# mindazhao/PWStableNet

Hardware: AMD Instinct MI355X
Metric: stabilized frames/sec at 256x256 (netG fp32 + grid_sample), whole job (higher is better)
Workload: dtype f32

## Files before the change

### pwstablenet_amd/csrc/abi.cpp

```cpp
#include <vector>

#include "common.h"

namespace pws {
bool g_two_queues = true;
int g_math = PWS_MATH_FP32;
int g_store = PWS_STORE_FP32;
int g_experiment = 0;
bool g_prof_on = false;
thread_local int g_prof_tag = -1;
thread_local bool t_deterministic = false;
namespace {
struct ProfEntry {
    hipEvent_t a, b;
    int kernel_id, tag;
    double flops, bytes;
};
std::vector<ProfEntry> g_prof_log;
std::vector<hipEvent_t> g_prof_pool;
hipEvent_t prof_event() {
    if (!g_prof_pool.empty()) {
        hipEvent_t e = g_prof_pool.back();
        g_prof_pool.pop_back();
        return e;
    }
    hipEvent_t e = nullptr;
    (void)hipEventCreate(&e);
    return e;
}
const char *const kKernelNames[KID_COUNT] = {
    "conv_mfma_kernel<k3s1,16x16>", "conv_mfma_kernel<k3s1,small>", "conv_mfma_kernel<k3s2,16x16>",
    "conv_mfma_kernel<k3s2,small>", "conv_mfma_kernel<k5s1,16x16>", "conv_mfma_kernel<convT4,16x16>",
    "conv_mfma_kernel<convT4,small>", "theta_head_kernel", "field_head_kernel", "grid_sample_fwd_kernel",
    "grid_sample_bwd_kernel", "upsample_grid_sample_fwd_kernel", "upsample_bilinear_ac_kernel", "affine_grid_kernel",
    "adam_kernel", "pack_weight_kernel", "conv_mfma_kernel<dgrad k4s2>", "conv_mfma_kernel<dgrad subpix k3s2>",
    "wgrad_mfma_kernel", "act_bwd_bias_kernel", "field_head_bwd_kernels", "theta_head_bwd_kernels",
    "wino_k3s1_kernel<F(2x2,3x3)>", "conv_bf16_kernel", "wgrad_bf16_kernel",
    "wino_ct4_kernel<F(3x3,2x2)>", "upsample_grid_sample_u8_kernel", "objective_kernels", "conv_ring_kernel", "conv_ringf_kernel",
    "wino_ring_kernel<F(2x2,3x3)>", "wino_ring_kernel<convT4,F(2x2,2x2)>", "conv_skinny_kernel", "wgrad_ring_kernel", "conv_skinny16_kernel", "conv_first_kernel", "wino5_first_kernel",
    "field_homography_kernel"};
}

bool prof_begin(int kernel_id, double flops, double bytes, hipStream_t st) {
    hipStreamCaptureStatus cs = hipStreamCaptureStatusNone;
    if (hipStreamIsCapturing(st, &cs) != hipSuccess || cs != hipStreamCaptureStatusNone) return false;
    ProfEntry e{prof_event(), prof_event(), kernel_id, g_prof_tag, flops, bytes};
    (void)hipEventRecord(e.a, st);
    g_prof_log.push_back(e);
    return true;
}
void prof_end(hipStream_t st) {
    if (!g_prof_log.empty()) (void)hipEventRecord(g_prof_log.back().b, st);
}
}

namespace pws {
static thread_local char g_err[512] = "";

void set_error(const char *fmt, ...) {
    va_list ap;
    va_start(ap, fmt);
    vsnprintf(g_err, sizeof(g_err), fmt, ap);
    va_end(ap);
}
}

extern "C" int pws_version(void) { return PWS_VERSION; }

extern "C" const char *pws_last_error(void) { return pws::g_err; }

extern "C" int pws_device_info(int *compute_units, int *arch_is_gfx950) {
    int dev = 0;
    hipError_t e = hipGetDevice(&dev);
    hipDeviceProp_t prop;
    if (e == hipSuccess) e = hipGetDeviceProperties(&prop, dev);
    if (e != hipSuccess) {
        pws::set_error("pws_device_info: %s", hipGetErrorString(e));
        return PWS_EHIP;
    }
    if (compute_units) *compute_units = prop.multiProcessorCount;
    if (arch_is_gfx950) {
        const char *a = prop.gcnArchName;
        *arch_is_gfx950 = (a[0] == 'g' && a[1] == 'f' && a[2] == 'x' && a[3] == '9' && a[4] == '5' && a[5] == '0') ? 1 : 0;
    }
    return PWS_OK;
}

extern "C" int pws_prof_enable(int on) {
    pws::g_prof_on = on != 0;
    return PWS_OK;
}

extern "C" int pws_prof_collect(pws_prof_record *out, int max_records) {
    const int n = (int)pws::g_prof_log.size();
    hipError_t bad = hipSuccess;
    for (int i = 0; i < n; ++i) {
        pws::ProfEntry &e = pws::g_prof_log[i];
        float ms = 0.f;
        hipError_t err = hipEventSynchronize(e.b);
        if (err == hipSuccess) err = hipEventElapsedTime(&ms, e.a, e.b);
        if (err != hipSuccess && bad == hipSuccess) bad = err;
        if (err == hipSuccess && out && i < max_records) out[i] = pws_prof_record{e.kernel_id, e.tag, e.flops, e.bytes, ms};
        pws::g_prof_pool.push_back(e.a);
        pws::g_prof_pool.push_back(e.b);
    }
    pws::g_prof_log.clear();
    if (bad != hipSuccess) {
        pws::set_error("pws_prof_collect: %s", hipGetErrorString(bad));
        return PWS_EHIP;
    }
    return n;
}

extern "C" const char *pws_prof_kernel_name(int kernel_id) {
    return (kernel_id >= 0 && kernel_id < pws::KID_COUNT) ? pws::kKernelNames[kernel_id] : "?";
}

extern "C" int pws_set_option(int key, int value) {
    if (key == PWS_OPT_TWO_QUEUES) {
        pws::g_two_queues = value != 0;
        return PWS_OK;
    }
    if (key == PWS_OPT_MATH) {
        if (value != PWS_MATH_FP32 && value != PWS_MATH_BF16) {
            pws::set_error("pws_set_option: PWS_OPT_MATH value %d is not PWS_MATH_FP32 / PWS_MATH_BF16", value);
            return PWS_EINVAL;
        }
        pws::g_math = value;
        return PWS_OK;
    }
    if (key == PWS_OPT_STORE) {
        if (value != PWS_STORE_FP32 && value != PWS_STORE_BF16) {
            pws::set_error("pws_set_option: PWS_OPT_STORE value %d is not PWS_STORE_FP32 / PWS_STORE_BF16", value);
            return PWS_EINVAL;
        }
        pws::g_store = value;
        return PWS_OK;
    }
    if (key == PWS_OPT_EXPERIMENT) {
        pws::g_experiment = value;
        return PWS_OK;
    }
    pws::set_error("pws_set_option: unknown key %d", key);
    return PWS_EINVAL;
}

extern "C" int pws_get_option(int key) {
    if (key == PWS_OPT_TWO_QUEUES) return pws::g_two_queues ? 1 : 0;
    if (key == PWS_OPT_MATH) return pws::g_math;
    if (key == PWS_OPT_STORE) return pws::g_store;
    if (key == PWS_OPT_EXPERIMENT) return pws::g_experiment;
    pws::set_error("pws_get_option: unknown key %d", key);
    return PWS_EINVAL;
}
```

### pwstablenet_amd/csrc/common.h

```cpp
#pragma once
#include <hip/hip_runtime.h>

#include <cstdarg>
#include <cstdio>

#include "../../include/pwstable.h"
#include "experiments.h"

namespace pws {

void set_error(const char *fmt, ...);

inline int check_launch(const char *what) {
    hipError_t e = hipGetLastError();
    if (e != hipSuccess) {
        set_error("%s: %s", what, hipGetErrorString(e));
        return PWS_EHIP;
    }
    return PWS_OK;
}

#define PWS_REQUIRE(cond, ...)          \
    do {                                \
        if (!(cond)) {                  \
            pws::set_error(__VA_ARGS__); \
            return PWS_EINVAL;          \
        }                               \
    } while (0)

inline hipStream_t as_stream(pws_stream_t s) { return reinterpret_cast<hipStream_t>(s); }

constexpr int kWave = 64;
constexpr int kXcds = 8;

__device__ __forceinline__ unsigned xcd_remap(unsigned bid, unsigned nblocks) {
    const unsigned q = nblocks / kXcds, r = nblocks % kXcds;
    const unsigned xcd = bid % kXcds, slot = bid / kXcds;
    const unsigned base = xcd < r ? xcd * (q + 1) : r * (q + 1) + (xcd - r) * q;
    return base + slot;
}

constexpr int kMaxDevices = 32;
inline int current_device_slot() {
    int d = 0;
    (void)hipGetDevice(&d);
    return (int)((unsigned)d % kMaxDevices);
}
struct PerDeviceFlag {
    bool v[kMaxDevices] = {};
    bool &cur() { return v[current_device_slot()]; }
};
struct PerDeviceInt {
    int v[kMaxDevices] = {};
    int &cur() { return v[current_device_slot()]; }
};

#if defined(__HIPCC__)
__device__ __forceinline__ float mul_rounded(float a, float b) {
    float p = a * b;
    asm volatile("" : "+v"(p));
    return p;
}
#endif

enum KernelId {
    KID_CONV_K3S1_BIG = 0, KID_CONV_K3S1_SMALL, KID_CONV_K3S2_BIG, KID_CONV_K3S2_SMALL, KID_CONV_K5S1, KID_CONVT4_BIG,
    KID_CONVT4_SMALL, KID_THETA_HEAD, KID_FIELD_HEAD, KID_GRID_SAMPLE_FWD, KID_GRID_SAMPLE_BWD, KID_UPSAMPLE_GRID_SAMPLE_FWD,
    KID_UPSAMPLE, KID_AFFINE_GRID, KID_ADAM, KID_PACK, KID_DGRAD_K4S2, KID_DGRAD_SP3, KID_WGRAD, KID_ACT_BWD, KID_FIELD_HEAD_BWD,
    KID_THETA_HEAD_BWD, KID_CONV_WINO, KID_CONV_BF16, KID_WGRAD_BF16, KID_CONV_WINO_CT4, KID_UPSAMPLE_GRID_SAMPLE_U8, KID_OBJECTIVE, KID_CONV_RING, KID_CONV_RINGF, KID_CONV_WRING, KID_CONV_WRING_CT4, KID_CONV_SKINNY, KID_WGRAD_RING, KID_CONV_SKINNY16, KID_CONV_FIRST, KID_CONV_FIRST_WINO, KID_FIELD_HOMOGRAPHY, KID_COUNT
};
extern thread_local bool t_deterministic;
struct DeterministicScope {
    bool prev;
    explicit DeterministicScope(bool on) : prev(t_deterministic) { t_deterministic = on || prev; }
    ~DeterministicScope() { t_deterministic = prev; }
};
extern bool g_two_queues;
extern int g_math;
extern int g_store;
extern bool g_prof_on;
extern thread_local int g_prof_tag;
bool prof_begin(int kernel_id, double flops, double bytes, hipStream_t st);
void prof_end(hipStream_t st);
struct ProfScope {
    hipStream_t st;
    bool on;
    ProfScope(int kernel_id, double flops, double bytes, hipStream_t s) : st(s), on(g_prof_on) {
        if (on) on = prof_begin(kernel_id, flops, bytes, st);
    }
    ~ProfScope() {
        if (on) prof_end(st);
    }
};

int nchw_to_nhwc_pad_strided(const float *x, size_t sample_stride, float *out, int n, int c, int h, int w, int cpad, int store, hipStream_t st);

struct ProfHint {
    double flops, bytes;
};
int theta_z1(const float *x, int n, int c, int hidden, const float *w_flat, const float *b_flat, float *ws, float *z1, hipStream_t st);
int theta_z2(const float *h, int n, int hidden, const float *w_lin, const float *b_lin, float *z2, hipStream_t st);
int field_head_raw(const float *x, int ld, int n, int h, int w, int c, const float *w_out, const float *b_out, float *z, hipStream_t st);
int field_bn_finish(const float *yhat, const float *theta, int n, int h, int w, int ac, float *resid, float *grid, hipStream_t st);
int field_bwd_gz(const float *resid, const float *g_grid, const float *g_resid, int n, int h, int w, int ac, float *gz, float *db_out,
                 float *dtheta, hipStream_t st);
int field_bwd_dx_dw(const float *x, int ld, const float *gz, int n, int h, int w, int c, const float *w_out, float *dx, int dx_ld,
                    int dx_accumulate, float *dw_out, int store, hipStream_t st, int dx_act = 0);
int theta_bwd_bn_lin(const float *dz2, const float *h, int n, int hidden, const float *w_lin, float *dw_lin, float *dh, hipStream_t st);
int theta_bwd_flat(const float *x, int n, int c, int hidden, const float *w_flat, const float *dz1, float *dw_flat, float *dx,
                   int dx_accumulate, hipStream_t st);
int wino_k3s1_launch(const pws_conv_args *a, const ProfHint &ph, hipStream_t st);
int wring_try(const pws_conv_args *a, const ProfHint &ph, hipStream_t st);
int wring_pack(const float *pk, float *ur, int cin_pad, int cout, int ct4, hipStream_t st);
__host__ __device__ inline size_t wring_index(int nc, int xi, int ci, int co, int nchunks) {
    const int cob = co >> 5, c32 = co & 31, co16 = c32 >> 1, nt = c32 & 1;
    const int chunk = ci >> 4, kq = (ci >> 2) & 3, st = ci & 3;
    return ((((((size_t)cob * nchunks + chunk) * nc + xi) * 2 + nt) * 4 + kq) * 16 + co16) * 4 + st;
}
#ifdef __HIPCC__
__device__ inline void wring_pack_element(const float *__restrict__ pk, float *__restrict__ ur, size_t plane, size_t i, int cin_pad, int cout,
                                          int ct4) {
    const int co = (int)(i % cout), ci = (int)(i / cout), nch = cin_pad / 16;
    if (!ct4) {
        float g[3][3];
#pragma unroll
        for (int r = 0; r < 3; ++r)
#pragma unroll
            for (int s = 0; s < 3; ++s) g[r][s] = pk[(size_t)(r * 3 + s) * plane + i];
        float u[4][3];
#pragma unroll
        for (int s = 0; s < 3; ++s) {
            u[0][s] = g[0][s], u[1][s] = 0.5f * (g[0][s] + g[1][s] + g[2][s]), u[2][s] = 0.5f * (g[0][s] - g[1][s] + g[2][s]);
            u[3][s] = g[2][s];
        }
#pragma unroll
        for (int r = 0; r < 4; ++r) {
            ur[wring_index(16, r * 4 + 0, ci, co, nch)] = u[r][0];
            ur[wring_index(16, r * 4 + 1, ci, co, nch)] = 0.5f * (u[r][0] + u[r][1] + u[r][2]);
            ur[wring_index(16, r * 4 + 2, ci, co, nch)] = 0.5f * (u[r][0] - u[r][1] + u[r][2]);
            ur[wring_index(16, r * 4 + 3, ci, co, nch)] = u[r][2];
        }
    } else if (ct4 == 2) {
        const double G[6][5] = {{1, 0, 0, 0, 0},
                                {-1.0 / 3, -1.0 / 3, -1.0 / 3, -1.0 / 3, -1.0 / 3},
                                {1.0 / 3, -1.0 / 3, 1.0 / 3, -1.0 / 3, 1.0 / 3},
                                {1.0 / 15, 2.0 / 15, 4.0 / 15, 8.0 / 15, 16.0 / 15},
                                {-16.0 / 15, 8.0 / 15, -4.0 / 15, 2.0 / 15, -1.0 / 15},
                                {0, 0, 0, 0, 1}};
        double t[6][5];
        for (int r = 0; r < 6; ++r)
            for (int v = 0; v < 5; ++v) {
                double a = 0;
                for (int q = 0; q < 5; ++q) a += G[r][q] * (double)pk[(size_t)(q * 5 + v) * plane + i];
                t[r][v] = a;
            }
        for (int r = 0; r < 6; ++r)
            for (int c = 0; c < 6; ++c) {
                double a = 0;
                for (int v = 0; v < 5; ++v) a += t[r][v] * G[c][v];
                ur[((((size_t)((ci >> 2) * 9 + ((r * 6 + c) >> 2)) * (cout / 16) + (co >> 4)) * 4 + (ci & 3)) * 16 + (co & 15)) * 4 + ((r * 6 + c) & 3)] = (float)a;
            }
    } else {
#pragma unroll
        for (int py = 0; py < 2; ++py)
#pragma unroll
            for (int px = 0; px < 2; ++px) {
                float g[2][2];
#pragma unroll
                for (int r = 0; r < 2; ++r)
#pragma unroll
                    for (int s = 0; s < 2; ++s) g[r][s] = pk[(size_t)((py * 2 + px) * 4 + r * 2 + s) * plane + i];
                float u[3][2];
#pragma unroll
                for (int s = 0; s < 2; ++s) u[0][s] = g[0][s], u[1][s] = g[0][s] + g[1][s], u[2][s] = g[1][s];
                float *o = ur + (size_t)py * 18 * plane;
#pragma unroll
                for (int r = 0; r < 3; ++r) {
                    o[wring_index(18, px * 9 + r * 3 + 0, ci, co, nch)] = u[r][0];
                    o[wring_index(18, px * 9 + r * 3 + 1, ci, co, nch)] = u[r][0] + u[r][1];
                    o[wring_index(18, px * 9 + r * 3 + 2, ci, co, nch)] = u[r][1];
                }
            }
    }
}
#endif

typedef __bf16 bf16x8 __attribute__((ext_vector_type(8)));
typedef __bf16 bf16x2 __attribute__((ext_vector_type(2)));
typedef float f32x2 __attribute__((ext_vector_type(2)));
typedef float f32x4 __attribute__((ext_vector_type(4)));
typedef unsigned u32x4 __attribute__((ext_vector_type(4)));
__device__ __forceinline__ unsigned cvt_pk_bf16(float a, float b) {
    return __builtin_bit_cast(unsigned, __builtin_convertvector((f32x2){a, b}, bf16x2));
}

template <bool IO16>
__device__ __forceinline__ float4 ld4(const float *base, size_t idx) {
    if constexpr (IO16) {
        const uint2 u = *reinterpret_cast<const uint2 *>(reinterpret_cast<const __bf16 *>(base) + idx);
        return make_float4(__builtin_bit_cast(float, u.x << 16), __builtin_bit_cast(float, u.x & 0xffff0000u),
                           __builtin_bit_cast(float, u.y << 16), __builtin_bit_cast(float, u.y & 0xffff0000u));
    } else {
        return *reinterpret_cast<const float4 *>(base + idx);
    }
}
template <bool IO16>
__device__ __forceinline__ void st4(float *base, size_t idx, const float4 &v) {
    if constexpr (IO16) {
        *reinterpret_cast<uint2 *>(reinterpret_cast<__bf16 *>(base) + idx) = make_uint2(cvt_pk_bf16(v.x, v.y), cvt_pk_bf16(v.z, v.w));
    } else {
        *reinterpret_cast<float4 *>(base + idx) = v;
    }
}

__device__ __forceinline__ float act_apply(float v, int act) {
    const float slope = act == PWS_ACT_LRELU ? 0.2f : 1.f;
    const unsigned keep = act == PWS_ACT_RELU ? 0u : 0xffffffffu;
    const float t = __builtin_bit_cast(float, __builtin_bit_cast(unsigned, slope * v) & keep);
    float r;
    asm("v_max_f32 %0, %1, %2" : "=v"(r) : "v"(v), "v"(t));
    return r;
}

}
```

### pwstablenet_amd/csrc/conv_common.h

```cpp
#pragma once
#include "common.h"

namespace pws {

typedef float f32x16 __attribute__((ext_vector_type(16)));

struct ConvKParams {
    const float *src_ptr[4];
    int src_c[4];
    int src_ld[4];
    int nsrc;
    int N, H, W;
    int LH, LW;
    int OH, OW;
    int cin_pad;
    int cout;
    const float *w;
    const float *bias;
    float *out;
    int out_ld;
    int act;
    int tiles_x, tiles_y;
    unsigned ntiles;
    int nclasses;
    int cls_inner;
    int ksplit;
    int chunks_per_split;
    size_t split_stride;
    const void *w_bf;
    int kpad_bf, npad_bf;
    int io_bf16;
    int epi16;
    int ndst;
    float *dst_ptr[4];
    int dst_c0[4], dst_c1[4], dst_ld[4], dst_acc[4];
    const void *dst_y[4];
    int dst_y_ld[4], dst_act[4];
    void *out_sign;
    int out_sign_ld;
    const void *dst_sign[4];
    int dst_sign_ld[4];
};

__device__ __forceinline__ void epi_store(const ConvKParams &p, size_t pix, int co, float v) {
    if (p.ndst == 0) {
        p.out[pix * p.out_ld + co] = act_apply(v + (p.bias ? p.bias[co] : 0.f), p.act);
    } else {
#pragma unroll
        for (int s = 0; s < 4; ++s) {
            if (s < p.ndst && co >= p.dst_c0[s] && co < p.dst_c1[s]) {
                float *d = p.dst_ptr[s] + pix * p.dst_ld[s] + (co - p.dst_c0[s]);
                *d = p.dst_acc[s] ? *d + v : v;
            }
        }
    }
}

__device__ __forceinline__ float bf16_lo(unsigned u) { return __builtin_bit_cast(float, u << 16); }
__device__ __forceinline__ float bf16_hi(unsigned u) { return __builtin_bit_cast(float, u & 0xffff0000u); }
__device__ __forceinline__ void epi_store_pair16(const ConvKParams &p, size_t pix, int co, float v0, float v1) {
    if (p.ndst == 0) {
        const float b0 = p.bias ? p.bias[co] : 0.f, b1 = p.bias ? p.bias[co + 1] : 0.f;
        unsigned *d = reinterpret_cast<unsigned *>(reinterpret_cast<__bf16 *>(p.out) + pix * p.out_ld + co);
        *d = cvt_pk_bf16(act_apply(v0 + b0, p.act), act_apply(v1 + b1, p.act));
    } else {
#pragma unroll
        for (int s = 0; s < 4; ++s) {
            if (s < p.ndst && co >= p.dst_c0[s] && co < p.dst_c1[s]) {
                unsigned *d = reinterpret_cast<unsigned *>(reinterpret_cast<__bf16 *>(p.dst_ptr[s]) + pix * p.dst_ld[s] + (co - p.dst_c0[s]));
                if (p.dst_acc[s]) {
                    const unsigned o = *d;
                    v0 += bf16_lo(o), v1 += bf16_hi(o);
                }
                if (p.dst_act[s] != PWS_ACT_NONE) {
                    const unsigned y = *reinterpret_cast<const unsigned *>(static_cast<const __bf16 *>(p.dst_y[s]) + pix * p.dst_y_ld[s] +
                                                                           (co - p.dst_c0[s]));
                    const float sl = p.dst_act[s] == PWS_ACT_LRELU ? 0.2f : 0.f;
                    v0 *= bf16_lo(y) > 0.f ? 1.f : sl, v1 *= bf16_hi(y) > 0.f ? 1.f : sl;
                }
                *d = cvt_pk_bf16(v0, v1);
            }
        }
    }
}

__device__ __forceinline__ void conv_block_coords(const ConvKParams &p, bool subpix, unsigned &tile, int &cls, int &split) {
    if (subpix && p.cls_inner) {
        const unsigned xcd = blockIdx.x & 7u, slot = blockIdx.x >> 3;
        cls = (int)(slot & 3u), split = (int)blockIdx.z;
        tile = xcd_remap(((slot >> 2) << 3) | xcd, p.ntiles);
    } else {
        tile = xcd_remap(blockIdx.x, p.ntiles);
        cls = subpix ? (int)(blockIdx.z & 3) : 0;
        split = subpix ? (int)(blockIdx.z >> 2) : (int)blockIdx.z;
    }
}
static inline dim3 conv_grid(ConvKParams &kp, int bn) {
    kp.cls_inner = kp.nclasses == 4 && kp.ntiles % 8 == 0 ? 1 : 0;
    const unsigned gy = (unsigned)((kp.cout + bn - 1) / bn);
    return kp.cls_inner ? dim3(kp.ntiles * 4, gy, (unsigned)kp.ksplit) : dim3(kp.ntiles, gy, (unsigned)(kp.nclasses * kp.ksplit));
}

struct ProfInfo {
    double flops, bytes;
};

struct TileChoice {
    int th, tw, tn, ck, bn;
    int kid;
    int (*launch)(ConvKParams &, hipStream_t, const ProfInfo &);
};

int launch_splitk_reduce(const ConvKParams &kp, const float *partial, size_t total4, hipStream_t st);

static inline long cdiv(long a, long b) { return (a + b - 1) / b; }

constexpr long kFillBlocks = 512;
constexpr long kFillBlocksBf16 = 256;

[[maybe_unused]] static int select_and_launch(const TileChoice *cands, int ncand, ConvKParams &kp, int cin_total, float *final_out,
                             float *ws, size_t ws_floats, hipStream_t st, const ProfInfo &pi, long kFill = kFillBlocks) {
    const TileChoice *best = nullptr;
    long best_blocks = -1;
    double best_score = -1.0;
    for (int i = 0; i < ncand; ++i) {
        const TileChoice &c = cands[i];
        const long tiles = cdiv(kp.LW, c.tw) * cdiv(kp.LH, c.th) * cdiv(kp.N, c.tn);
        const double useful = (double)kp.N * kp.LH * kp.LW / ((double)tiles * c.th * c.tw * c.tn);
        if (useful < 0.45 && i + 1 < ncand) continue;
        if (c.th < 8 && c.th < kp.LH && i > 0 && best) continue;
        const long blocks = tiles * cdiv(kp.cout, c.bn) * kp.nclasses;
        if (blocks >= kFill) {
            best = &c, best_blocks = blocks;
            break;
        }
        if (blocks * useful > best_score) best = &c, best_blocks = blocks, best_score = blocks * useful;
    }
    const TileChoice &c = *best;
    kp.tiles_x = (int)cdiv(kp.LW, c.tw), kp.tiles_y = (int)cdiv(kp.LH, c.th);
    kp.ntiles = (unsigned)(kp.tiles_x * kp.tiles_y * cdiv(kp.N, c.tn));
    const int total_chunks = cin_total / c.ck;
    int ksplit = 1;
    const size_t out_floats = (size_t)kp.N * kp.OH * kp.OW * kp.cout;
    if (best_blocks < kFill && ws && kp.cout % 4 == 0 && total_chunks >= 4) {
        long want = cdiv(kFill, best_blocks);
        if (want > 64) want = 64;
        if (want > total_chunks / 2) want = total_chunks / 2;
        while (want > 1 && (size_t)want * out_floats > ws_floats) --want;
        ksplit = (int)want;
    }
    kp.ksplit = ksplit < 1 ? 1 : ksplit;
    kp.chunks_per_split = (int)cdiv(total_chunks, kp.ksplit);
    kp.ksplit = (int)cdiv(total_chunks, kp.chunks_per_split);
    kp.split_stride = out_floats;
    kp.out = kp.ksplit > 1 ? ws : final_out;
    ProfScope prof(c.kid, pi.flops, pi.bytes, st);
    int rc = c.launch(kp, st, pi);
    if (rc != PWS_OK || kp.ksplit == 1) return rc;
    const size_t total4 = out_floats / 4;
    kp.out = final_out;
    return launch_splitk_reduce(kp, ws, total4, st);
}


}
```

### pwstablenet_amd/csrc/conv_mfma.hip

```cpp
#include "conv_common.h"

namespace pws {

template <int KS_, int STRIDE_, int PAD_, int SUBPIX_, int TH_, int TW_, int TN_, int CK_, int WM_, int WN_, int MT_,
          int NT_, bool NCHW_ = false>
struct ConvCfg {
    static constexpr int KS = KS_, STRIDE = STRIDE_, PAD = PAD_, TH = TH_, TW = TW_, TN = TN_, CK = CK_;
    static constexpr int SUBPIX = SUBPIX_;
    static constexpr bool CONVT = SUBPIX_ != 0, NCHW = NCHW_;
    static constexpr int WM = WM_, WN = WN_, MT = MT_, NT = NT_;
    static constexpr int THREADS = 64 * WM * WN;
    static constexpr int BM = TH * TW * TN, BN = 32 * NT * WN;
    static_assert(BM == 32 * MT * WM, "tile pixels must equal the M extent of the wave grid");
    static constexpr int IH = (TH - 1) * STRIDE + KS, IW = (TW - 1) * STRIDE + KS;
    static constexpr int PIX = TN * IH * IW;
    static constexpr int CKP = CK + 1;
    static constexpr int TAPS = KS * KS;
    static constexpr int LDS_IN = (PIX * CKP + 3) / 4 * 4;
    static constexpr int LDS_W = TAPS * CK * BN;
    static constexpr int LDS_BYTES = (LDS_IN + LDS_W) * 4;
    static constexpr int C4 = CK / 4;
    static constexpr int ITEMS_IN = (PIX * C4 + THREADS - 1) / THREADS;
    static constexpr int ITEMS_W = (TAPS * CK * (BN / 4) + THREADS - 1) / THREADS;
    static constexpr int ITEMS_NCHW = (PIX * CK + THREADS - 1) / THREADS;
};

template <class C>
__global__ void __launch_bounds__(C::THREADS, 2) conv_mfma_kernel(const ConvKParams p) {
    extern __shared__ float lds[];
    float *lds_in = lds;
    float *lds_w = lds + C::LDS_IN;

    const int tid = threadIdx.x;
    const int lane = tid & 63, wv = tid >> 6;
    const int l31 = lane & 31, hi = lane >> 5;
    const int wm = wv / C::WN, wn = wv % C::WN;

    unsigned tile;
    int cls, split;
    conv_block_coords(p, C::CONVT, tile, cls, split);
    const int tx_i = tile % p.tiles_x;
    const int ty_i = (tile / p.tiles_x) % p.tiles_y;
    const int tn_i = tile / (p.tiles_x * p.tiles_y);
    const int n0 = tn_i * C::TN, y0 = ty_i * C::TH, x0 = tx_i * C::TW;
    const int co0 = blockIdx.y * C::BN;
    const int py = cls >> 1, px = cls & 1;
    const int pad_y = C::SUBPIX == 1 ? 1 - py : (C::SUBPIX == 2 ? 0 : C::PAD);
    const int pad_x = C::SUBPIX == 1 ? 1 - px : (C::SUBPIX == 2 ? 0 : C::PAD);
    const int iy0 = y0 * C::STRIDE - pad_y, ix0 = x0 * C::STRIDE - pad_x;

    int g_pix[C::ITEMS_IN];
    int l_off[C::ITEMS_IN];
    int g_c4[C::ITEMS_IN];
    unsigned ok_mask = 0;
#pragma unroll
    for (int it = 0; it < C::ITEMS_IN; ++it) {
        const int item = tid + it * C::THREADS;
        const int pix = item / C::C4, c4 = item % C::C4;
        const int lx = pix % C::IW, ly = (pix / C::IW) % C::IH, tn = pix / (C::IW * C::IH);
        const int n = n0 + tn, iy = iy0 + ly, ix = ix0 + lx;
        const bool ok = item < C::PIX * C::C4 && n < p.N && iy >= 0 && iy < p.H && ix >= 0 && ix < p.W;
        g_pix[it] = ok ? (n * p.H + iy) * p.W + ix : 0;
        ok_mask |= ok ? (1u << it) : 0u;
        l_off[it] = item < C::PIX * C::C4 ? pix * C::CKP + c4 * 4 : -1;
        g_c4[it] = c4 * 4;
    }
    static_assert(C::ITEMS_IN <= 32 && C::ITEMS_W <= 32, "mask width");
    int w_off[C::ITEMS_W];
    unsigned w_mask = 0;
#pragma unroll
    for (int it = 0; it < C::ITEMS_W; ++it) {
        const int item = tid + it * C::THREADS;
        const int row = item / (C::BN / 4), q = item % (C::BN / 4);
        const int tap = row / C::CK, c = row % C::CK;
        const bool ok = item < C::TAPS * C::CK * (C::BN / 4) && (co0 + q * 4) < p.cout;
        w_off[it] = ok ? (tap * p.cin_pad + c) * p.cout + co0 + q * 4 : 0;
        w_mask |= ok ? (1u << it) : 0u;
    }
    const float *w_cls = p.w + (size_t)cls * C::TAPS * p.cin_pad * p.cout;
    float4 r_in[C::NCHW ? 1 : C::ITEMS_IN];
    float4 r_w[C::ITEMS_W];
    float r_nchw[C::NCHW ? C::ITEMS_NCHW : 1];

    auto load_chunk = [&](int s, int c0, int wrow) {
        if constexpr (C::NCHW) {
            const int Creal = p.src_c[0];
            const size_t sstride = p.src_ld[0] ? (size_t)p.src_ld[0] : (size_t)Creal * p.H * p.W;
#pragma unroll
            for (int it = 0; it < C::ITEMS_NCHW; ++it) {
                const int item = tid + it * C::THREADS;
                const int c = item / C::PIX, pix = item % C::PIX;
                const int lx = pix % C::IW, ly = (pix / C::IW) % C::IH, tn = pix / (C::IW * C::IH);
                const int n = n0 + tn, iy = iy0 + ly, ix = ix0 + lx;
                const bool ok = item < C::PIX * C::CK && (c0 + c) < Creal && n < p.N && iy >= 0 && iy < p.H && ix >= 0 &&
                                ix < p.W;
                const size_t off = ok ? (size_t)n * sstride + ((size_t)(c0 + c) * p.H + iy) * p.W + ix : 0;
                const float v = p.src_ptr[0][off];
                r_nchw[it] = ok ? v : 0.f;
            }
        } else {
            const float *sp = p.src_ptr[s] + c0;
            const size_t ld = p.src_ld[s];
#pragma unroll
            for (int it = 0; it < C::ITEMS_IN; ++it)
                r_in[it] = *reinterpret_cast<const float4 *>(sp + (size_t)g_pix[it] * ld + g_c4[it]);
        }
        const float *wp = w_cls + (size_t)wrow * p.cout;
#pragma unroll
        for (int it = 0; it < C::ITEMS_W; ++it) r_w[it] = *reinterpret_cast<const float4 *>(wp + w_off[it]);
    };
    auto store_chunk = [&]() {
        if constexpr (C::NCHW) {
#pragma unroll
            for (int it = 0; it < C::ITEMS_NCHW; ++it) {
                const int item = tid + it * C::THREADS;
                const int c = item / C::PIX, pix = item % C::PIX;
                if (item < C::PIX * C::CK) lds_in[pix * C::CKP + c] = r_nchw[it];
            }
        } else {
#pragma unroll
            for (int it = 0; it < C::ITEMS_IN; ++it) {
                if (l_off[it] >= 0) {
                    const bool ok = (ok_mask >> it) & 1u;
                    float *d = lds_in + l_off[it];
                    d[0] = ok ? r_in[it].x : 0.f, d[1] = ok ? r_in[it].y : 0.f, d[2] = ok ? r_in[it].z : 0.f,
                    d[3] = ok ? r_in[it].w : 0.f;
                }
            }
        }
#pragma unroll
        for (int it = 0; it < C::ITEMS_W; ++it) {
            const int item = tid + it * C::THREADS;
            if (item < C::TAPS * C::CK * (C::BN / 4)) {
                const bool ok = (w_mask >> it) & 1u;
                *reinterpret_cast<float4 *>(lds_w + item * 4) =
                    ok ? r_w[it] : make_float4(0.f, 0.f, 0.f, 0.f);
            }
        }
    };

    f32x16 acc[C::MT][C::NT];
#pragma unroll
    for (int mt = 0; mt < C::MT; ++mt)
#pragma unroll
        for (int nt = 0; nt < C::NT; ++nt)
#pragma unroll
            for (int r = 0; r < 16; ++r) acc[mt][nt][r] = 0.f;

    int a_base[C::MT];
#pragma unroll
    for (int mt = 0; mt < C::MT; ++mt) {
        const int m = (wm * C::MT + mt) * 32 + l31;
        const int tx = m % C::TW, ty = (m / C::TW) % C::TH, tn = m / (C::TW * C::TH);
        a_base[mt] = ((tn * C::IH + ty * C::STRIDE) * C::IW + tx * C::STRIDE) * C::CKP + hi;
    }
    const int b_base = hi * C::BN + wn * C::NT * 32 + l31;

    int total_chunks = 0;
    if constexpr (C::NCHW) {
        total_chunks = p.cin_pad / C::CK;
    } else {
        for (int s = 0; s < p.nsrc; ++s) total_chunks += p.src_c[s] / C::CK;
    }
    const int ch_begin = split * p.chunks_per_split;
    const int ch_end = min(total_chunks, ch_begin + p.chunks_per_split);
    int s = 0, c0 = ch_begin * C::CK, wrow = ch_begin * C::CK;
    if constexpr (!C::NCHW) {
        while (s < p.nsrc - 1 && c0 >= p.src_c[s]) c0 -= p.src_c[s], ++s;
    }
    if (ch_begin < ch_end) load_chunk(s, c0, wrow);
    for (int ch = ch_begin; ch < ch_end; ++ch) {
        __syncthreads();
        store_chunk();
        __syncthreads();
        c0 += C::CK, wrow += C::CK;
        if (!C::NCHW && c0 >= p.src_c[s]) ++s, c0 = 0;
        if (ch + 1 < ch_end) load_chunk(s, c0, wrow);

#pragma unroll
        for (int tap = 0; tap < C::TAPS; ++tap) {
            if (C::SUBPIX == 2 && ((!py && tap / C::KS) || (!px && tap % C::KS))) continue;
            const int toff = ((tap / C::KS) * C::IW + (tap % C::KS)) * C::CKP;
#pragma unroll
            for (int kk = 0; kk < C::CK / 2; ++kk) {
                float a[C::MT], b[C::NT];
#pragma unroll
                for (int mt = 0; mt < C::MT; ++mt) a[mt] = lds_in[a_base[mt] + toff + 2 * kk];
#pragma unroll
                for (int nt = 0; nt < C::NT; ++nt) b[nt] = lds_w[b_base + (tap * C::CK + 2 * kk) * C::BN + nt * 32];
#pragma unroll
                for (int mt = 0; mt < C::MT; ++mt)
#pragma unroll
                    for (int nt = 0; nt < C::NT; ++nt)
                        acc[mt][nt] = __builtin_amdgcn_mfma_f32_32x32x2f32(a[mt], b[nt], acc[mt][nt], 0, 0, 0);
            }
        }
    }

    const bool partial = p.ksplit > 1;
    float *part = p.out + (size_t)split * p.split_stride;
#pragma unroll
    for (int nt = 0; nt < C::NT; ++nt) {
        const int co = co0 + (wn * C::NT + nt) * 32 + l31;
        const bool co_ok = co < p.cout;
#pragma unroll
        for (int mt = 0; mt < C::MT; ++mt) {
#pragma unroll
            for (int r = 0; r < 16; ++r) {
                const int m = (wm * C::MT + mt) * 32 + (r & 3) + 8 * (r >> 2) + 4 * hi;
                const int tx = m % C::TW, ty = (m / C::TW) % C::TH, tn = m / (C::TW * C::TH);
                const int n = n0 + tn, y = y0 + ty, x = x0 + tx;
                const int oy = C::CONVT ? 2 * y + py : y, ox = C::CONVT ? 2 * x + px : x;
                if (co_ok && n < p.N && y < p.LH && x < p.LW && oy < p.OH && ox < p.OW) {
                    const size_t pix = (size_t)(n * p.OH + oy) * p.OW + ox;
                    if (partial)
                        part[pix * p.cout + co] = acc[mt][nt][r];
                    else
                        epi_store(p, pix, co, acc[mt][nt][r]);
                }
            }
        }
    }
}

__global__ void __launch_bounds__(256) splitk_reduce_kernel(const ConvKParams p, const float *__restrict__ partial,
                                                            size_t total4) {
    const size_t i = (size_t)blockIdx.x * 256 + threadIdx.x;
    if (i >= total4) return;
    float4 a = reinterpret_cast<const float4 *>(partial)[i];
    for (int s = 1; s < p.ksplit; ++s) {
        const float4 b = reinterpret_cast<const float4 *>(partial + (size_t)s * p.split_stride)[i];
        a.x += b.x, a.y += b.y, a.z += b.z, a.w += b.w;
    }
    const size_t pix = (i * 4) / p.cout;
    const int co = (int)((i * 4) % p.cout);
    if (p.io_bf16) {
        epi_store_pair16(p, pix, co, a.x, a.y), epi_store_pair16(p, pix, co + 2, a.z, a.w);
        return;
    }
    epi_store(p, pix, co, a.x), epi_store(p, pix, co + 1, a.y), epi_store(p, pix, co + 2, a.z), epi_store(p, pix, co + 3, a.w);
}

int launch_splitk_reduce(const ConvKParams &kp, const float *partial, size_t total4, hipStream_t st) {
    hipLaunchKernelGGL(splitk_reduce_kernel, dim3((unsigned)((total4 + 255) / 256)), dim3(256), 0, st, kp, partial, total4);
    return check_launch("splitk_reduce_kernel");
}

template <class C, int KID>
static int launch_cfg(ConvKParams &kp, hipStream_t st, const ProfInfo &pi) {
    static PerDeviceFlag attr_set_dev;
    bool &attr_set = attr_set_dev.cur();
    if (!attr_set) {
        hipError_t e = hipFuncSetAttribute(reinterpret_cast<const void *>(&conv_mfma_kernel<C>),
                                           hipFuncAttributeMaxDynamicSharedMemorySize, C::LDS_BYTES);
        if (e != hipSuccess) {
            set_error("hipFuncSetAttribute(conv_mfma_kernel, %d B LDS): %s", C::LDS_BYTES, hipGetErrorString(e));
            return PWS_EHIP;
        }
        attr_set = true;
    }
    const dim3 grid = conv_grid(kp, C::BN);
    hipLaunchKernelGGL(conv_mfma_kernel<C>, grid, dim3(C::THREADS), C::LDS_BYTES, st, kp);
    return check_launch("conv_mfma_kernel");
}

template <class C, int KID>
static constexpr TileChoice choice() {
    return TileChoice{C::TH, C::TW, C::TN, C::CK, C::BN, KID, &launch_cfg<C, KID>};
}

using K3S1_T256 = ConvCfg<3, 1, 1, 0, 16, 16, 1, 16, 4, 1, 2, 2>;
using K3S1_T128 = ConvCfg<3, 1, 1, 0, 8, 16, 1, 16, 4, 1, 1, 2>;
using K3S1_T64 = ConvCfg<3, 1, 1, 0, 8, 8, 1, 16, 2, 2, 1, 1>;
using K3S1_T64N4 = ConvCfg<3, 1, 1, 0, 4, 4, 4, 16, 2, 2, 1, 1>;
using K3S1_T64N16 = ConvCfg<3, 1, 1, 0, 2, 2, 16, 16, 2, 2, 1, 1>;
using K3S2_T256 = ConvCfg<3, 2, 1, 0, 16, 16, 1, 8, 4, 1, 2, 2>;
using K3S2_T128 = ConvCfg<3, 2, 1, 0, 8, 16, 1, 16, 4, 1, 1, 2>;
using K3S2_T64 = ConvCfg<3, 2, 1, 0, 8, 8, 1, 16, 2, 2, 1, 1>;
using K3S2_T64N4 = ConvCfg<3, 2, 1, 0, 4, 4, 4, 16, 2, 2, 1, 1>;
using K3S2_T64N16 = ConvCfg<3, 2, 1, 0, 2, 2, 16, 16, 2, 2, 1, 1>;
using K5S1_T256 = ConvCfg<5, 1, 2, 0, 16, 16, 1, 8, 4, 1, 2, 2>;
using K5S1_T256_NCHW = ConvCfg<5, 1, 2, 0, 16, 16, 1, 8, 4, 1, 2, 2, true>;
using CT4_T256 = ConvCfg<2, 1, 0, 1, 16, 16, 1, 16, 4, 1, 2, 2>;
using CT4_T128 = ConvCfg<2, 1, 0, 1, 8, 16, 1, 16, 4, 1, 1, 2>;
using CT4_T64 = ConvCfg<2, 1, 0, 1, 8, 8, 1, 16, 2, 2, 1, 1>;
using CT4_T64N4 = ConvCfg<2, 1, 0, 1, 4, 4, 4, 16, 2, 2, 1, 1>;
using CT4_T64N16 = ConvCfg<2, 1, 0, 1, 2, 2, 16, 16, 2, 2, 1, 1>;

using K4S2_T256 = ConvCfg<4, 2, 1, 0, 16, 16, 1, 8, 4, 1, 2, 2>;
using K4S2_T128 = ConvCfg<4, 2, 1, 0, 8, 16, 1, 8, 4, 1, 1, 2>;
using K4S2_T64 = ConvCfg<4, 2, 1, 0, 8, 8, 1, 8, 2, 2, 1, 1>;
using K4S2_T64N4 = ConvCfg<4, 2, 1, 0, 4, 4, 4, 8, 2, 2, 1, 1>;
using K4S2_T64N16 = ConvCfg<4, 2, 1, 0, 2, 2, 16, 8, 2, 2, 1, 1>;
using SP3_T256 = ConvCfg<2, 1, 0, 2, 16, 16, 1, 16, 4, 1, 2, 2>;
using SP3_T128 = ConvCfg<2, 1, 0, 2, 8, 16, 1, 16, 4, 1, 1, 2>;
using SP3_T64 = ConvCfg<2, 1, 0, 2, 8, 8, 1, 16, 2, 2, 1, 1>;
using SP3_T64N4 = ConvCfg<2, 1, 0, 2, 4, 4, 4, 16, 2, 2, 1, 1>;
using SP3_T64N16 = ConvCfg<2, 1, 0, 2, 2, 2, 16, 16, 2, 2, 1, 1>;

static const TileChoice kK3S1[] = {choice<K3S1_T256, KID_CONV_K3S1_BIG>(), choice<K3S1_T128, KID_CONV_K3S1_BIG>(),
                                   choice<K3S1_T64, KID_CONV_K3S1_SMALL>(), choice<K3S1_T64N4, KID_CONV_K3S1_SMALL>(),
                                   choice<K3S1_T64N16, KID_CONV_K3S1_SMALL>()};
static const TileChoice kK3S2[] = {choice<K3S2_T256, KID_CONV_K3S2_BIG>(), choice<K3S2_T128, KID_CONV_K3S2_BIG>(),
                                   choice<K3S2_T64, KID_CONV_K3S2_SMALL>(), choice<K3S2_T64N4, KID_CONV_K3S2_SMALL>(),
                                   choice<K3S2_T64N16, KID_CONV_K3S2_SMALL>()};
static const TileChoice kCT4[] = {choice<CT4_T256, KID_CONVT4_BIG>(), choice<CT4_T128, KID_CONVT4_BIG>(),
                                  choice<CT4_T64, KID_CONVT4_SMALL>(), choice<CT4_T64N4, KID_CONVT4_SMALL>(),
                                  choice<CT4_T64N16, KID_CONVT4_SMALL>()};
static const TileChoice kK4S2[] = {choice<K4S2_T256, KID_DGRAD_K4S2>(), choice<K4S2_T128, KID_DGRAD_K4S2>(),
                                   choice<K4S2_T64, KID_DGRAD_K4S2>(), choice<K4S2_T64N4, KID_DGRAD_K4S2>(),
                                   choice<K4S2_T64N16, KID_DGRAD_K4S2>()};
static const TileChoice kSP3[] = {choice<SP3_T256, KID_DGRAD_SP3>(), choice<SP3_T128, KID_DGRAD_SP3>(),
                                  choice<SP3_T64, KID_DGRAD_SP3>(), choice<SP3_T64N4, KID_DGRAD_SP3>(),
                                  choice<SP3_T64N16, KID_DGRAD_SP3>()};
static const TileChoice kK5[] = {choice<K5S1_T256, KID_CONV_K5S1>()};
static const TileChoice kK5N[] = {choice<K5S1_T256_NCHW, KID_CONV_K5S1>()};

int conv_bf16_fwd(int kind, ConvKParams &kp, int cin_total, float *out, float *ws, size_t ws_floats, hipStream_t st,
                  const ProfInfo &pi);
int conv_bf16_dgrad(int kind, ConvKParams &kp, int cout_f, float *ws, size_t ws_floats, hipStream_t st, const ProfInfo &pi);
static inline bool ledger_direct(int bit) { return (exp_mask(EXP_PARITY_LEDGER, 32) & bit) != 0; }
int conv_ringf_try(int kind, const ConvKParams &kp, hipStream_t st, const ProfInfo &pi);
int conv_first_try(const ConvKParams &kp, hipStream_t st, const ProfInfo &pi);
int wino5_first_try(const ConvKParams &kp, const float *u, hipStream_t st, const ProfInfo &pi);
int conv_skinny_try(int kind, ConvKParams &kp, float *final_out, float *ws, size_t ws_floats, hipStream_t st, const ProfInfo &pi);

int conv2d_fwd_impl(const pws_conv_args *a, hipStream_t st) {
    PWS_REQUIRE(a != nullptr, "pws_conv2d_fwd: args is NULL");
    PWS_REQUIRE(a->n >= 0 && a->h > 0 && a->w > 0, "pws_conv2d_fwd: bad n/h/w %d/%d/%d", a->n, a->h, a->w);
    PWS_REQUIRE(a->nsrc >= 1 && a->nsrc <= 4, "pws_conv2d_fwd: nsrc %d not in 1..4", a->nsrc);
    PWS_REQUIRE(a->cout > 0 && a->cout % 4 == 0, "pws_conv2d_fwd: cout %d must be a positive multiple of 4", a->cout);
    PWS_REQUIRE(a->out && a->w_packed, "pws_conv2d_fwd: NULL out / w_packed");
    PWS_REQUIRE(a->out_ld >= a->cout, "pws_conv2d_fwd: out_ld %d < cout %d", a->out_ld, a->cout);
    PWS_REQUIRE(a->act >= PWS_ACT_NONE && a->act <= PWS_ACT_RELU, "pws_conv2d_fwd: bad act %d", a->act);
    PWS_REQUIRE(a->ws == nullptr || (reinterpret_cast<size_t>(a->ws) & 15) == 0, "pws_conv2d_fwd: ws must be 16-B aligned");
    if (a->n == 0) return PWS_OK;

    ConvKParams kp{};
    int cin = 0;
    kp.nsrc = a->nsrc;
    const bool nchw = a->src_nchw != 0;
    if (nchw) {
        PWS_REQUIRE(a->kind == PWS_CONV_K5S1 && a->nsrc == 1, "pws_conv2d_fwd: NCHW source only for the k5 first layer");
        PWS_REQUIRE(a->src[0].ptr && a->src[0].channels > 0, "pws_conv2d_fwd: bad NCHW source");
        PWS_REQUIRE(a->src[0].ld >= 0, "pws_conv2d_fwd: NCHW source: ld is the sample stride in floats (0 = dense)");
        kp.src_ptr[0] = a->src[0].ptr, kp.src_c[0] = a->src[0].channels, kp.src_ld[0] = a->src[0].ld;
        cin = a->src[0].channels;
    } else {
        for (int s = 0; s < a->nsrc; ++s) {
            const pws_src &sr = a->src[s];
            PWS_REQUIRE(sr.ptr && sr.channels > 0 && sr.channels % 16 == 0 && sr.ld >= sr.channels && sr.ld % 4 == 0 &&
                            (reinterpret_cast<size_t>(sr.ptr) & 15) == 0,
                        "pws_conv2d_fwd: source %d (channels %d, ld %d) must be 16-B aligned, channels %% 16 == 0, ld %% 4 == 0",
                        s, sr.channels, sr.ld);
            kp.src_ptr[s] = sr.ptr, kp.src_c[s] = sr.channels, kp.src_ld[s] = sr.ld;
            cin += sr.channels;
        }
    }
    kp.cin_pad = (cin + 15) / 16 * 16;
    kp.N = a->n, kp.H = a->h, kp.W = a->w;
    kp.cout = a->cout, kp.w = a->w_packed, kp.bias = a->bias, kp.out_ld = a->out_ld, kp.act = a->act;
    kp.nclasses = 1;
    PWS_REQUIRE((size_t)a->n * a->h * a->w < (1u << 31), "pws_conv2d_fwd: n*h*w too large for 32-bit pixel indices");
    float *ws = static_cast<float *>(a->ws);
    const size_t ws_floats = a->ws_bytes / sizeof(float);
    const bool bf16 = a->math == PWS_MATH_BF16 && a->w_bf16 && !nchw;
    if (a->store == PWS_STORE_BF16) {
        PWS_REQUIRE(bf16, "pws_conv2d_fwd: bf16 storage needs math == PWS_MATH_BF16, w_bf16 and NHWC sources");
        PWS_REQUIRE(a->out_ld % 2 == 0 && a->cout % 2 == 0 && (reinterpret_cast<size_t>(a->out) & 3) == 0,
                    "pws_conv2d_fwd: bf16 storage needs an even cout / out_ld and a 4-byte aligned out");
        for (int s = 0; s < a->nsrc; ++s)
            PWS_REQUIRE(a->src[s].channels % 32 == 0 && a->src[s].ld % 8 == 0,
                        "pws_conv2d_fwd: bf16 storage needs channels %% 32 == 0 and ld %% 8 == 0 (source %d: %d, %d)", s,
                        a->src[s].channels, a->src[s].ld);
        kp.io_bf16 = 1;
        kp.epi16 = a->cout % 8 == 0 && a->out_ld % 8 == 0 && (reinterpret_cast<size_t>(a->out) & 15) == 0;
    }
    kp.w_bf = a->w_bf16, kp.kpad_bf = (kp.cin_pad + 31) / 32 * 32, kp.npad_bf = (a->cout + 63) / 64 * 64;
    if (a->out_sign) {
        PWS_REQUIRE(a->store == PWS_STORE_BF16 && a->cout % 8 == 0 && a->out_sign_ld >= a->cout / 8,
                    "pws_conv2d_fwd: out_sign needs bf16 storage, cout %% 8 == 0 and out_sign_ld >= cout / 8");
        kp.out_sign = a->out_sign, kp.out_sign_ld = a->out_sign_ld;
    }

    auto info = [&](int k2, double out_pix) {
        ProfInfo pi;
        pi.flops = 2.0 * out_pix * a->cout * (double)cin * k2;
        const double es = a->store == PWS_STORE_BF16 ? 2.0 : 4.0, ws_ = bf16 ? 2.0 : 4.0;
        pi.bytes = es * ((double)a->n * a->h * a->w * cin + out_pix * a->cout) + ws_ * (double)k2 * cin * a->cout;
        return pi;
    };
    switch (a->kind) {
    case PWS_CONV_K3S1:
    case PWS_CONVT_K3S1: {
        kp.OH = kp.LH = a->h, kp.OW = kp.LW = a->w;
        const ProfInfo pi = info(9, (double)a->n * a->h * a->w);
        if (bf16) {
            const int rc = conv_bf16_fwd(a->kind, kp, kp.cin_pad, a->out, ws, ws_floats, st, pi);
            if (rc != 1) return rc;
        }
        if (a->w_wring && !nchw && !bf16 && !ledger_direct(2)) {
            const int rc = wring_try(a, ProfHint{pi.flops, pi.bytes}, st);
            if (rc != 1) return rc;
        }
        const long wblocks = cdiv(a->w, 16) * cdiv(a->h, 16) * a->n * cdiv(a->cout, 64);
        if (a->w_wino && !nchw && a->h >= 16 && a->w >= 16 && wblocks >= 128 && (cin >= 128 || wblocks >= 2048) && !ledger_direct(2))
            return wino_k3s1_launch(a, ProfHint{pi.flops, pi.bytes}, st);
        if (!bf16 && !nchw) {
            kp.out = a->out;
            int rc = ledger_direct(8) ? 1 : conv_ringf_try(a->kind, kp, st, pi);
            if (rc != 1) return rc;
            rc = ledger_direct(16) ? 1 : conv_skinny_try(a->kind, kp, a->out, ws, ws_floats, st, pi);
            if (rc != 1) return rc;
        }
        return select_and_launch(kK3S1, 5, kp, kp.cin_pad, a->out, ws, ws_floats, st, pi);
    }
    case PWS_CONV_K3S2:
        kp.OH = kp.LH = (a->h + 2 - 3) / 2 + 1, kp.OW = kp.LW = (a->w + 2 - 3) / 2 + 1;
        if (bf16) {
            const int rc = conv_bf16_fwd(a->kind, kp, kp.cin_pad, a->out, ws, ws_floats, st, info(9, (double)a->n * kp.OH * kp.OW));
            if (rc != 1) return rc;
        }
        if (!bf16 && !nchw) {
            kp.out = a->out;
            int rc = ledger_direct(8) ? 1 : conv_ringf_try(a->kind, kp, st, info(9, (double)a->n * kp.OH * kp.OW));
            if (rc != 1) return rc;
            rc = ledger_direct(16) ? 1 : conv_skinny_try(a->kind, kp, a->out, ws, ws_floats, st, info(9, (double)a->n * kp.OH * kp.OW));
            if (rc != 1) return rc;
        }
        return select_and_launch(kK3S2, 5, kp, kp.cin_pad, a->out, ws, ws_floats, st, info(9, (double)a->n * kp.OH * kp.OW));
    case PWS_CONV_K5S1:
        kp.OH = kp.LH = a->h, kp.OW = kp.LW = a->w;
        if (bf16) {
            const int rc = conv_bf16_fwd(a->kind, kp, kp.cin_pad, a->out, nullptr, 0, st, info(25, (double)a->n * a->h * a->w));
            if (rc != 1) return rc;
        }
        if (nchw && !ledger_direct(1)) {
            kp.out = a->out;
            if (a->w_wring) {
                const int rcw = wino5_first_try(kp, static_cast<const float *>(a->w_wring), st, info(25, (double)a->n * a->h * a->w));
                if (rcw != 1) return rcw;
            }
            const int rc = conv_first_try(kp, st, info(25, (double)a->n * a->h * a->w));
            if (rc != 1) return rc;
        }
        return select_and_launch(nchw ? kK5N : kK5, 1, kp, kp.cin_pad, a->out, nullptr, 0, st,
                                 info(25, (double)a->n * a->h * a->w));
    case PWS_CONVT_K4S2: {
        kp.LH = a->h, kp.LW = a->w, kp.OH = 2 * a->h, kp.OW = 2 * a->w, kp.nclasses = 4;
        ProfInfo pi = info(4, (double)a->n * kp.OH * kp.OW);
        pi.bytes += (bf16 ? 2.0 : 4.0) * 12.0 * cin * a->cout;
        if (bf16) {
            const int rc = conv_bf16_fwd(a->kind, kp, kp.cin_pad, a->out, ws, ws_floats, st, pi);
            if (rc != 1) return rc;
        }
        if (a->w_wring && !nchw && !bf16 && !ledger_direct(4)) {
            const int rc = wring_try(a, ProfHint{pi.flops, pi.bytes}, st);
            if (rc != 1) return rc;
        }
        const long wb = cdiv(a->w, 24) * cdiv(a->h, 12) * a->n * cdiv(a->cout, 64) * 4;
        if (a->w_wino && a->h >= 24 && a->w >= 24 && wb >= 256 && !ledger_direct(4)) return wino_k3s1_launch(a, ProfHint{pi.flops, pi.bytes}, st);
        if (!bf16 && !nchw) {
            kp.out = a->out;
            int rc = ledger_direct(8) ? 1 : conv_ringf_try(a->kind, kp, st, pi);
            if (rc != 1) return rc;
            rc = ledger_direct(16) ? 1 : conv_skinny_try(a->kind, kp, a->out, ws, ws_floats, st, pi);
            if (rc != 1) return rc;
        }
        return select_and_launch(kCT4, 5, kp, kp.cin_pad, a->out, ws, ws_floats, st, pi);
    }
    default:
        set_error("pws_conv2d_fwd: kind %d is not a runnable conv kind", a->kind);
        return PWS_EINVAL;
    }
}

int conv2d_bwd_data_impl(const pws_conv_bwd_data_args *a, hipStream_t st) {
    PWS_REQUIRE(a != nullptr, "pws_conv2d_bwd_data: args is NULL");
    PWS_REQUIRE(a->n >= 0 && a->h > 0 && a->w > 0 && a->cout > 0 && a->cout % 16 == 0, "pws_conv2d_bwd_data: bad shape");
    PWS_REQUIRE(a->gout && a->w_dgrad && a->gout_ld >= a->cout && a->gout_ld % 4 == 0, "pws_conv2d_bwd_data: bad gout / weights");
    PWS_REQUIRE(a->ndst >= 1 && a->ndst <= 4, "pws_conv2d_bwd_data: ndst %d not in 1..4", a->ndst);
    if (a->n == 0) return PWS_OK;
    ConvKParams kp{};
    int oh = a->h, ow = a->w;
    if (a->kind == PWS_CONV_K3S2) oh = (a->h - 1) / 2 + 1, ow = (a->w - 1) / 2 + 1;
    if (a->kind == PWS_CONVT_K4S2) oh = 2 * a->h, ow = 2 * a->w;
    kp.nsrc = 1, kp.src_ptr[0] = a->gout, kp.src_c[0] = a->cout, kp.src_ld[0] = a->gout_ld;
    kp.N = a->n, kp.H = oh, kp.W = ow;
    kp.OH = a->h, kp.OW = a->w;
    kp.cin_pad = a->cout;
    int cin_f = 0;
    kp.ndst = a->ndst;
    for (int s = 0; s < a->ndst; ++s) {
        const pws_dst &d = a->dst[s];
        PWS_REQUIRE(d.ptr && d.channels > 0 && d.ld >= d.channels, "pws_conv2d_bwd_data: bad destination %d", s);
        kp.dst_ptr[s] = d.ptr, kp.dst_c0[s] = cin_f, kp.dst_c1[s] = cin_f + d.channels, kp.dst_ld[s] = d.ld;
        kp.dst_acc[s] = d.accumulate ? 1 : 0;
        if (d.act_y && d.act != PWS_ACT_NONE) {
            PWS_REQUIRE(a->store == PWS_STORE_BF16 && (d.act == PWS_ACT_LRELU || d.act == PWS_ACT_RELU),
                        "pws_conv2d_bwd_data: the fused act' (dst[%d].act_y) needs bf16 storage and PWS_ACT_LRELU / PWS_ACT_RELU", s);
            PWS_REQUIRE(d.act_y_ld >= d.channels && d.act_y_ld % 2 == 0 && (reinterpret_cast<size_t>(d.act_y) & 3) == 0,
                        "pws_conv2d_bwd_data: bad act_y / act_y_ld of destination %d", s);
            kp.dst_y[s] = d.act_y, kp.dst_y_ld[s] = d.act_y_ld, kp.dst_act[s] = d.act;
            if (d.act_sign) {
                PWS_REQUIRE(d.channels % 8 == 0 && d.act_sign_ld >= d.channels / 8, "pws_conv2d_bwd_data: bad act_sign / act_sign_ld of destination %d", s);
                kp.dst_sign[s] = d.act_sign, kp.dst_sign_ld[s] = d.act_sign_ld;
            }
        }
        cin_f += d.channels;
    }
    PWS_REQUIRE(cin_f % 4 == 0, "pws_conv2d_bwd_data: total destination channels %d must be a multiple of 4", cin_f);
    kp.cout = cin_f, kp.w = a->w_dgrad, kp.bias = nullptr, kp.act = PWS_ACT_NONE, kp.out_ld = cin_f, kp.nclasses = 1;
    PWS_REQUIRE((size_t)a->n * oh * ow < (1u << 31) && (size_t)a->n * a->h * a->w < (1u << 31), "pws_conv2d_bwd_data: too large");
    float *ws = static_cast<float *>(a->ws);
    const size_t ws_floats = a->ws_bytes / sizeof(float);
    ProfInfo pi;
    const double k2 = a->kind == PWS_CONVT_K4S2 ? 4.0 : 9.0;
    pi.flops = 2.0 * a->n * oh * ow * (double)a->cout * cin_f * k2;
    {
        const double es = a->store == PWS_STORE_BF16 ? 2.0 : 4.0, in_pix = (double)a->n * a->h * a->w;
        pi.bytes = es * ((double)a->n * oh * ow * a->cout + in_pix * cin_f);
        for (int s = 0; s < a->ndst; ++s)
            pi.bytes += es * in_pix * a->dst[s].channels * (a->dst[s].accumulate ? 1.0 : 0.0) +
                        (kp.dst_act[s] == PWS_ACT_NONE ? 0.0 : (kp.dst_sign[s] ? in_pix * a->dst[s].channels / 8.0 : es * in_pix * a->dst[s].channels));
    }
    if (a->kind == PWS_CONV_K3S2)
        kp.LH = oh, kp.LW = ow, kp.nclasses = 4;
    else
        kp.LH = a->h, kp.LW = a->w;
    if (a->store == PWS_STORE_BF16) {
        PWS_REQUIRE(a->math == PWS_MATH_BF16 && a->w_dgrad_bf16 && a->cout % 32 == 0 && a->gout_ld % 8 == 0,
                    "pws_conv2d_bwd_data: bf16 storage needs bf16 math, w_dgrad_bf16, cout %% 32 == 0 and gout_ld %% 8 == 0");
        for (int s = 0; s < a->ndst; ++s)
            PWS_REQUIRE(a->dst[s].channels % 2 == 0 && a->dst[s].ld % 2 == 0 && (reinterpret_cast<size_t>(a->dst[s].ptr) & 3) == 0,
                        "pws_conv2d_bwd_data: bf16 storage needs even channels / ld and 4-byte aligned destinations");
        kp.io_bf16 = 1;
        kp.epi16 = 1;
        for (int s = 0; s < a->ndst; ++s)
            if (a->dst[s].channels % 8 || a->dst[s].ld % 8 || (reinterpret_cast<size_t>(a->dst[s].ptr) & 15) ||
                (kp.dst_act[s] != PWS_ACT_NONE && (kp.dst_y_ld[s] % 8 || (reinterpret_cast<size_t>(kp.dst_y[s]) & 15))))
                kp.epi16 = 0;
    }
    if (a->math == PWS_MATH_BF16 && a->w_dgrad_bf16) {
        kp.w_bf = a->w_dgrad_bf16, kp.kpad_bf = (a->cout + 31) / 32 * 32, kp.npad_bf = (cin_f + 63) / 64 * 64;
        const int rc = conv_bf16_dgrad(a->kind, kp, a->cout, ws, ws_floats, st, pi);
        if (rc != 1) return rc;
    }
    switch (a->kind) {
    case PWS_CONV_K3S1:
    case PWS_CONVT_K3S1:
        return select_and_launch(kK3S1, 5, kp, a->cout, nullptr, ws, ws_floats, st, pi);
    case PWS_CONV_K3S2:
        return select_and_launch(kSP3, 5, kp, a->cout, nullptr, ws, ws_floats, st, pi);
    case PWS_CONVT_K4S2:
        return select_and_launch(kK4S2, 5, kp, a->cout, nullptr, ws, ws_floats, st, pi);
    default:
        set_error("pws_conv2d_bwd_data: kind %d has no data gradient here", a->kind);
        return PWS_EINVAL;
    }
}

}

extern "C" int pws_conv2d_fwd(const pws_conv_args *args, pws_stream_t stream) {
    return pws::conv2d_fwd_impl(args, pws::as_stream(stream));
}

extern "C" int pws_conv2d_bwd_data(const pws_conv_bwd_data_args *args, pws_stream_t stream) {
    return pws::conv2d_bwd_data_impl(args, pws::as_stream(stream));
}
```

### pwstablenet_amd/csrc/conv_skinny.hip

```cpp
#include "conv_common.h"

namespace pws {

enum SkinnyMode { SK_K3S1 = 0, SK_K3S2 = 1, SK_CT4 = 2 };

struct SkParams {
    const float *src_ptr[4];
    int src_c[4], src_ld[4];
    int nsrc;
    int N, H, W;
    int LH, LW;
    int OH, OW;
    int mode;
    int cin_pad, cout;
    const float *w;
    unsigned w_bytes;
    const float *bias;
    int act;
    float *out;
    int out_ld;
    size_t split_stride;
    int ksplit, cps, nchunks;
    int M;
    unsigned ncob;
};

constexpr unsigned kSkOob = 0x7ffffff0u;
__device__ __forceinline__ void sk_dma16(unsigned lds_addr, unsigned voff, __amdgpu_buffer_rsrc_t rsrc, unsigned soff) {
    unsigned keep;
    asm volatile("s_nop 4\n\ts_mov_b32 %0, m0\n\ts_mov_b32 m0, %1\n\ts_nop 0\n\tbuffer_load_dwordx4 %2, %3, %4 offen lds\n\ts_mov_b32 m0, %0"
                 : "=&s"(keep)
                 : "s"(lds_addr), "v"(voff), "s"(rsrc), "s"(soff));
}
template <class T>
__device__ __forceinline__ T sksel4(const T (&a)[4], int i) {
    return i == 0 ? a[0] : (i == 1 ? a[1] : (i == 2 ? a[2] : a[3]));
}

template <int MT_W, int NT_W, int WM>
__global__ void __launch_bounds__(256) conv_skinny_kernel(const SkParams p) {
    extern __shared__ __attribute__((aligned(16))) unsigned char lds[];
    constexpr int WN = 4 / WM;
    static_assert(NT_W * WN == 4, "4 N tiles of 16 output channels per workgroup");
    const int tid = threadIdx.x, lane = tid & 63;
    const int wv = __builtin_amdgcn_readfirstlane(tid >> 6);
    const int l15 = lane & 15, kq = lane >> 4;
    const int wm = wv % WM, wn = wv / WM;

    unsigned b = blockIdx.x;
    const int ks = (int)(b % (unsigned)p.ksplit);
    b /= (unsigned)p.ksplit;
    const int cob = (int)(b % p.ncob), cls = (int)(b / p.ncob);
    const int py = cls >> 1, px = cls & 1;
    const int co0 = cob * 64;
    const int c_begin = ks * p.cps;
    const int nck = min(p.nchunks - c_begin, p.cps);
    const int ntaps = p.mode == SK_CT4 ? 4 : 9;

    {
        const __amdgpu_buffer_rsrc_t rsrc_w = __builtin_amdgcn_make_buffer_rsrc(const_cast<float *>(p.w), 0, (int)p.w_bytes, 0x00020000);
        const int nt = lane >> 4 >> 0 & 3, kqd = (lane >> 2) & 3, c4 = lane & 3;
        const int col = co0 + nt * 16 + c4 * 4;
        const bool col_ok = col < p.cout;
        const size_t plane = (size_t)p.cin_pad * p.cout;
        const int npieces = nck * ntaps * 4;
        for (int q = wv; q < npieces; q += 4) {
            const int blk = q >> 2, st = q & 3;
            const int ck = blk / ntaps, tap = blk - ck * ntaps;
            const int wplane = p.mode == SK_CT4 ? cls * 4 + tap : tap;
            const unsigned row = (unsigned)((c_begin + ck) * 16 + kqd * 4 + st);
            const unsigned voff = col_ok ? (row * (unsigned)p.cout + (unsigned)col) * 4u : kSkOob;
            sk_dma16((unsigned)(blk * 4096 + st * 1024), voff, rsrc_w, (unsigned)__builtin_amdgcn_readfirstlane((unsigned)((size_t)wplane * plane * 4)));
        }
    }

    int pn[MT_W], piy[MT_W], pix_[MT_W];
    bool pok[MT_W];
#pragma unroll
    for (int i = 0; i < MT_W; ++i) {
        const int m = (wm + i * WM) * 16 + l15;
        pok[i] = m < p.M;
        const int mm = pok[i] ? m : 0;
        const int ox = mm % p.LW, t2 = mm / p.LW;
        const int oy = t2 % p.LH;
        pn[i] = t2 / p.LH;
        if (p.mode == SK_K3S2) piy[i] = 2 * oy - 1, pix_[i] = 2 * ox - 1;
        else if (p.mode == SK_CT4) piy[i] = oy + py - 1, pix_[i] = ox + px - 1;
        else piy[i] = oy - 1, pix_[i] = ox - 1;
    }
    int s = 0, c0 = c_begin * 16;
    while (s < p.nsrc - 1 && c0 >= sksel4(p.src_c, s)) c0 -= sksel4(p.src_c, s), ++s;

    constexpr int MAXT = 9;
    f32x4 a_cur[MAXT][MT_W], a_nxt[MAXT][MT_W];
    auto load_a = [&](f32x4 (&a)[MAXT][MT_W]) {
        const float *sp = sksel4(p.src_ptr, s) + c0 + kq * 4;
        const int ld = sksel4(p.src_ld, s);
        const int kw = p.mode == SK_CT4 ? 2 : 3;
#pragma unroll
        for (int t = 0; t < MAXT; ++t) {
            if (t < ntaps) {
                const int dy = t / kw, dx = t - dy * kw;
#pragma unroll
                for (int i = 0; i < MT_W; ++i) {
                    const int iy = piy[i] + dy, ix = pix_[i] + dx;
                    const bool ok = pok[i] && iy >= 0 && iy < p.H && ix >= 0 && ix < p.W;
                    a[t][i] = ok ? *reinterpret_cast<const f32x4 *>(sp + ((size_t)(pn[i] * p.H + iy) * p.W + ix) * ld) : (f32x4){0.f, 0.f, 0.f, 0.f};
                }
            }
        }
        c0 += 16;
        if (c0 >= sksel4(p.src_c, s) && s < p.nsrc - 1) ++s, c0 = 0;
    };

    f32x4 acc[MT_W][NT_W];
#pragma unroll
    for (int i = 0; i < MT_W; ++i)
#pragma unroll
        for (int j = 0; j < NT_W; ++j) acc[i][j] = (f32x4){0.f, 0.f, 0.f, 0.f};

    load_a(a_cur);
    asm volatile("s_waitcnt vmcnt(0)" ::: "memory");
    __syncthreads();
    const int b_lane = (kq * 16 + l15) * 4;
    for (int ck = 0; ck < nck; ++ck) {
        if (ck + 1 < nck) load_a(a_nxt);
#pragma unroll
        for (int t = 0; t < MAXT; ++t) {
            if (t < ntaps) {
                const unsigned char *bb = lds + (unsigned)((ck * ntaps + t) * 4096) + b_lane;
#pragma unroll
                for (int st = 0; st < 4; ++st) {
                    float bv[NT_W];
#pragma unroll
                    for (int j = 0; j < NT_W; ++j) bv[j] = *reinterpret_cast<const float *>(bb + (st * 4 + wn * NT_W + j) * 256);
#pragma unroll
                    for (int i = 0; i < MT_W; ++i)
#pragma unroll
                        for (int j = 0; j < NT_W; ++j) acc[i][j] = __builtin_amdgcn_mfma_f32_16x16x4f32(a_cur[t][i][st], bv[j], acc[i][j], 0, 0, 0);
                }
            }
        }
        if (ck + 1 < nck) {
#pragma unroll
            for (int t = 0; t < MAXT; ++t)
#pragma unroll
                for (int i = 0; i < MT_W; ++i) a_cur[t][i] = a_nxt[t][i];
        }
    }

    float *out = p.out + (size_t)ks * p.split_stride;
    const bool fin = p.ksplit == 1;
#pragma unroll
    for (int i = 0; i < MT_W; ++i) {
#pragma unroll
        for (int r = 0; r < 4; ++r) {
            const int m = (wm + i * WM) * 16 + 4 * kq + r;
            if (m >= p.M) continue;
            const int ox = m % p.LW, t2 = m / p.LW;
            const int oy = t2 % p.LH, n = t2 / p.LH;
            size_t opix;
            if (p.mode == SK_CT4) opix = ((size_t)n * p.OH + 2 * oy + py) * p.OW + 2 * ox + px;
            else opix = ((size_t)n * p.OH + oy) * p.OW + ox;
#pragma unroll
            for (int j = 0; j < NT_W; ++j) {
                const int co = co0 + (wn * NT_W + j) * 16 + l15;
                if (co < p.cout) {
                    if (fin) p.out[opix * p.out_ld + co] = act_apply(acc[i][j][r] + (p.bias ? p.bias[co] : 0.f), p.act);
                    else out[opix * p.cout + co] = acc[i][j][r];
                }
            }
        }
    }
}

template <int MT_W, int NT_W, int WM>
static int skinny_launch(const SkParams &p, unsigned grid, int lds_bytes, hipStream_t st) {
    static PerDeviceFlag attr_set_dev;
    bool &attr_set = attr_set_dev.cur();
    if (!attr_set) {
        hipError_t e = hipFuncSetAttribute(reinterpret_cast<const void *>(&conv_skinny_kernel<MT_W, NT_W, WM>), hipFuncAttributeMaxDynamicSharedMemorySize,
                                           160 * 1024);
        if (e != hipSuccess) {
            set_error("hipFuncSetAttribute(conv_skinny_kernel): %s", hipGetErrorString(e));
            return PWS_EHIP;
        }
        attr_set = true;
    }
    hipLaunchKernelGGL((conv_skinny_kernel<MT_W, NT_W, WM>), dim3(grid), dim3(256), lds_bytes, st, p);
    return check_launch("conv_skinny_kernel");
}

int conv_skinny_try(int kind, ConvKParams &kp, float *final_out, float *ws, size_t ws_floats, hipStream_t st, const ProfInfo &pi) {
    if (kp.io_bf16 || kp.ndst != 0 || exp_is(EXP_SKINNY_OFF)) return 1;
    int mode;
    if (kind == PWS_CONV_K3S1 || kind == PWS_CONVT_K3S1) mode = SK_K3S1;
    else if (kind == PWS_CONV_K3S2) mode = SK_K3S2;
    else if (kind == PWS_CONVT_K4S2) mode = SK_CT4;
    else return 1;
    const long M = (long)kp.N * kp.LH * kp.LW;
    if (M < 1 || M > 128 || kp.cout % 4 != 0) return 1;
    int cin = 0;
    for (int s = 0; s < kp.nsrc; ++s) {
        if (kp.src_ld[s] == 0 || kp.src_c[s] % 16 != 0 || kp.src_ld[s] % 4 != 0 || (reinterpret_cast<size_t>(kp.src_ptr[s]) & 15)) return 1;
        cin += kp.src_c[s];
    }
    if (cin != kp.cin_pad) return 1;
    const int ntaps = mode == SK_CT4 ? 4 : 9, ncls = mode == SK_CT4 ? 4 : 1;
    const size_t w_bytes = (size_t)(mode == SK_CT4 ? 16 : 9) * kp.cin_pad * kp.cout * 4;
    if (w_bytes >= (1u << 31)) return 1;
    SkParams p{};
    for (int s = 0; s < 4; ++s) p.src_ptr[s] = kp.src_ptr[s], p.src_c[s] = kp.src_c[s], p.src_ld[s] = kp.src_ld[s];
    p.nsrc = kp.nsrc, p.N = kp.N, p.H = kp.H, p.W = kp.W, p.LH = kp.LH, p.LW = kp.LW, p.OH = kp.OH, p.OW = kp.OW, p.mode = mode;
    p.cin_pad = kp.cin_pad, p.cout = kp.cout, p.w = kp.w, p.w_bytes = (unsigned)w_bytes, p.bias = kp.bias, p.act = kp.act, p.out_ld = kp.out_ld;
    p.M = (int)M, p.ncob = (unsigned)((kp.cout + 63) / 64);
    p.nchunks = cin / 16;
    const int maxc = 36 / ntaps;
    const long blocks1 = (long)p.ncob * ncls;
    int ksplit = (int)cdiv(512, blocks1);
    if (ksplit > p.nchunks) ksplit = p.nchunks;
    const int kmin = (int)cdiv(p.nchunks, maxc);
    if (ksplit < kmin) ksplit = kmin;
    const size_t out_floats = (size_t)kp.N * kp.OH * kp.OW * kp.cout;
    if (ksplit > 1 && (!ws || (size_t)ksplit * out_floats > ws_floats)) {
        if (!ws || (size_t)kmin * out_floats > ws_floats) return 1;
        ksplit = (int)(ws_floats / out_floats);
    }
    p.cps = (int)cdiv(p.nchunks, ksplit);
    p.ksplit = (int)cdiv(p.nchunks, p.cps);
    if (p.cps > maxc) return 1;
    p.split_stride = out_floats;
    p.out = p.ksplit > 1 ? ws : final_out;
    const unsigned grid = (unsigned)(blocks1 * p.ksplit);
    const int lds_bytes = p.cps * ntaps * 4096;
    if (exp_is(EXP_SKINNY_SKIP)) return PWS_OK;
    ProfScope prof(KID_CONV_SKINNY, pi.flops, pi.bytes, st);
    int rc;
    if (M <= 16) rc = skinny_launch<1, 1, 1>(p, grid, lds_bytes, st);
    else if (M <= 32) rc = skinny_launch<1, 2, 2>(p, grid, lds_bytes, st);
    else rc = skinny_launch<2, 4, 4>(p, grid, lds_bytes, st);
    if (rc != PWS_OK || p.ksplit == 1) return rc;
    kp.ksplit = p.ksplit, kp.split_stride = out_floats, kp.out = final_out;
    return launch_splitk_reduce(kp, ws, out_floats / 4, st);
}

}
```

### pwstablenet_amd/csrc/experiments.h

```cpp
#pragma once

namespace pws {

extern int g_experiment;

enum Exp : int {
    EXP_GS_BWD_GENERAL = 2,
    EXP_U8_CVT_SHIFT = 4,
    EXP_GS_ROWWIN = 5,
    EXP_NO_SIGN_BITS = 12,
    EXP_NETG_PER_STAGE = 15,
    EXP_RING_OFF = 20,
    EXP_RING_SMALL = 21,
    EXP_RINGF_OFF = 22,
    EXP_RINGF_8X32 = 23,
    EXP_RINGF_16X32 = 24,
    EXP_FIRST_MFMA = 25,
    EXP_FIRST_NO_WINO = 26,
    EXP_RINGF_32CH = 27,
    EXP_FIRST_SMALL = 29,
    EXP_WINO5_SMALL = 30,
    EXP_HEAD_V1 = 35,
    EXP_GS_U8_LANE_WINDOWS = 49,
    EXP_WRING_OFF = 50,
    EXP_WRING_FORCE = 58,
    EXP_WRING_MODE2 = 59,
    EXP_SKINNY_OFF = 70,
    EXP_SKINNY16_OFF = 71,
    EXP_SKINNY16_4096 = 72,
    EXP_SKINNY_SKIP = 73,
    EXP_WGRAD_RING_OFF = 80,
    EXP_WGRAD_RING_FORCE = 81,
    EXP_HEAD_VALU = 90,
    EXP_HEAD_BWD_VALU = 91,
    EXP_HEAD_ONE_TILE = 92,
    EXP_DEEP_TILE_ALWAYS = 96,
    EXP_SHAPE_GENERAL = 97,
    EXP_TL1_TILED = 98,
    EXP_RING_8WAVE = 105,
    EXP_SMOOTH_ONE_PIXEL = 110,
    EXP_NO_PACK_ONE_PASS = 120,
    EXP_RING_UNIT256 = 186,
    EXP_RING_UNIT128 = 187,
    EXP_WGRAD_NO_MERGE = 188,
    EXP_WGRAD_MIN_TILES = 190,
    EXP_FIRST_ABLATE = 1100,
    EXP_FIRST_CLOCK = 1200,
    EXP_WINO5_ABLATE = 1300,
    EXP_WGRAD_WIDE_ABLATE = 1400,
    EXP_RING_ABLATE = 1500,
    EXP_WINO_ABLATE = 1600,
    EXP_BF16_PROBE = 2100,
    EXP_RINGF_VARIANT = 2200,
    EXP_PARITY_LEDGER = 3000,
    EXP_WRING_ABLATE = 4000,
};

inline bool exp_is(Exp e) { return g_experiment == e; }
inline bool exp_in(Exp base, int n) { return g_experiment >= base && g_experiment < base + n; }
inline int exp_mask(Exp base, int n) { return exp_in(base, n) ? g_experiment - base : 0; }

}
```

### pwstablenet_amd/csrc/netg.cpp

```cpp
#include <mutex>
#include <unordered_map>
#include <vector>

#include "common.h"
#include <cstdlib>
#include <cstdio>
#include "netg_pack.h"

namespace pws {

struct Layer {
    int kind, cin, cout;
    size_t w_off, b_off;
    size_t gw_off, gb_off;
    size_t dg_off;
    size_t ww_off;
    size_t wr_off;
    size_t wb_off;
    size_t dgb_off;
};

static int bf16_planes(int kind) {
    switch (kind) {
    case PWS_CONV_K3S1:
    case PWS_CONV_K3S2:
    case PWS_CONVT_K3S1: return 9;
    case PWS_CONVT_K4S2: return 16;
    case PWS_CONV_K5S1: return 25;
    default: return 0;
    }
}
static int bf16_dgrad_planes(int kind) { return kind == PWS_CONV_K3S1 || kind == PWS_CONVT_K3S1 ? 9 : 16; }

enum {
    L_TRANSFER = 0,
    L_DOWN1 = 1,
    L_UP7 = 8,
    L_OUT = 15,
    L_DB1_CS = 16,
    L_UB7_MP = 30,
    L_FLATTEN = 44,
    L_LINEAR = 45,
    L_COUNT = 46
};

static size_t align_up(size_t v, size_t a) { return (v + a - 1) / a * a; }

static std::vector<Layer> build_layers(int input_nc, int g, size_t *total_floats, size_t *total_dgrad = nullptr, size_t *total_grad = nullptr) {
    std::vector<Layer> L;
    size_t off = 0, dg = 0, gr = 0;
    auto add = [&](int kind, int cin, int cout, bool ring = false) {
        Layer l{kind, cin, cout, 0, 0, 0, 0, (size_t)-1, (size_t)-1, (size_t)-1, (size_t)-1, (size_t)-1};
        l.w_off = off;
        off = align_up(off + pws_packed_weight_floats(kind, cin, cout), 64);
        l.b_off = off;
        off = align_up(off + (size_t)cout, 64);
        l.gw_off = gr;
        gr = align_up(gr + pws_packed_weight_floats(kind, cin, cout), 64);
        l.gb_off = gr;
        gr = align_up(gr + (size_t)cout, 64);
        if (kind == PWS_CONV_K3S1 || kind == PWS_CONVT_K3S1) {
            l.ww_off = off;
            off = align_up(off + pws_packed_wino_floats(cin, cout), 64);
        }
        if (ring && pws_packed_wring_floats(kind, cin, cout)) {
            l.wr_off = off;
            off = align_up(off + pws_packed_wring_floats(kind, cin, cout), 64);
        }
        if (bf16_planes(kind) && ((cin + 15) / 16 * 16) % 32 == 0) {
            l.wb_off = off;
            off = align_up(off + pws_packed_bf16_floats(bf16_planes(kind), (cin + 15) / 16 * 16, cout), 64);
        }
        const size_t d = pws_packed_dgrad_floats(kind, cin, cout);
        if (d) l.dg_off = dg, dg = align_up(dg + d, 64);
        if (d && bf16_planes(kind) && cout % 32 == 0) {
            l.dgb_off = dg;
            dg = align_up(dg + pws_packed_bf16_floats(bf16_dgrad_planes(kind), cout, cin), 64);
        }
        L.push_back(l);
    };
    const int enc[7][2] = {{g, g}, {g, 2 * g}, {2 * g, 4 * g}, {4 * g, 4 * g}, {4 * g, 4 * g}, {4 * g, 4 * g}, {4 * g, 4 * g}};
    add(PWS_CONV_K5S1, input_nc, g, true);
    for (int i = 0; i < 7; ++i) add(PWS_CONV_K3S2, enc[i][0], enc[i][1]);
    const int dec[7][2] = {{4 * g, 4 * g}, {8 * g, 4 * g}, {8 * g, 4 * g}, {8 * g, 4 * g}, {8 * g, 2 * g}, {4 * g, g}, {2 * g, g}};
    for (int j = 0; j < 7; ++j) add(PWS_CONVT_K4S2, dec[j][0], dec[j][1], j >= 3);
    add(PWS_CONV_K3S1_OUT, g, 2);
    for (int i = 0; i < 7; ++i) {
        add(PWS_CONV_K3S1, enc[i][0], enc[i][0], i < 4);
        add(PWS_CONV_K3S2, i == 0 ? enc[i][0] : 2 * enc[i][0], enc[i][1]);
    }
    const int ub[7][3] = {{4 * g, 4 * g, 8 * g}, {8 * g, 4 * g, 16 * g}, {8 * g, 4 * g, 16 * g}, {8 * g, 4 * g, 16 * g},
                          {8 * g, 2 * g, 16 * g}, {4 * g, g, 8 * g}, {2 * g, g, 4 * g}};
    for (int j = 0; j < 7; ++j) {
        add(PWS_CONVT_K4S2, ub[j][2], ub[j][1], j >= 3);
        add(PWS_CONVT_K3S1, ub[j][0], ub[j][0], j >= 3);
    }
    add(PWS_CONV_K2S1P0, 4 * g, 8 * g);
    add(PWS_CONV_K1, 8 * g, 6);
    if (total_floats) *total_floats = off;
    if (total_dgrad) *total_dgrad = dg;
    if (total_grad) *total_grad = gr;
    return L;
}

static int kind_ksize(int kind) {
    switch (kind) {
    case PWS_CONV_K5S1: return 5;
    case PWS_CONVT_K4S2: return 4;
    case PWS_CONV_K2S1P0: return 2;
    case PWS_CONV_K1: return 1;
    default: return 3;
    }
}
static unsigned off32(size_t off) { return off == (size_t)-1 ? kNoOff : (unsigned)off; }

static void fill_pack_layers(const std::vector<Layer> &L, PackLayer *out) {
    for (int i = 0; i < L_COUNT; ++i) {
        const Layer &l = L[i];
        PackLayer &p = out[i];
        p.kind = l.kind, p.cin = l.cin, p.cin_pad = (l.cin + 15) / 16 * 16, p.cout = l.cout, p.k = kind_ksize(l.kind);
        p.planes = l.kind == PWS_CONVT_K4S2 ? 16 : p.k * p.k;
        p.dg_taps = l.dg_off == (size_t)-1 ? 0 : (l.kind == PWS_CONV_K3S1 || l.kind == PWS_CONVT_K3S1 ? 9 : 16);
        p.w_off = off32(l.w_off), p.b_off = off32(l.b_off), p.ww_off = off32(l.ww_off), p.dg_off = off32(l.dg_off), p.wr_off = off32(l.wr_off);
    }
}

struct NetgOpts {
    int math, store;
    bool two_queues;
    bool deterministic = false;
    size_t x_sample_stride = 0;
    bool prune_dead = false;
};
static NetgOpts opts_defaults() { return NetgOpts{g_math, g_store, g_two_queues}; }
static int opts_from(const pws_netg_opts *o, NetgOpts *out) {
    if (!o) {
        *out = opts_defaults();
        return PWS_OK;
    }
    PWS_REQUIRE(o->math == PWS_MATH_FP32 || o->math == PWS_MATH_BF16, "pws_netg_opts: math %d", o->math);
    PWS_REQUIRE(o->store == PWS_STORE_FP32 || o->store == PWS_STORE_BF16, "pws_netg_opts: store %d", o->store);
    PWS_REQUIRE(o->store == PWS_STORE_FP32 || o->math == PWS_MATH_BF16, "pws_netg_opts: PWS_STORE_BF16 needs PWS_MATH_BF16");
    PWS_REQUIRE(o->two_queues >= -1 && o->two_queues <= 1 && (o->flags & ~(PWS_NETG_DETERMINISTIC | PWS_NETG_PRUNE_DEAD)) == 0, "pws_netg_opts: two_queues %d / flags %d",
                o->two_queues, o->flags);
    *out = NetgOpts{o->math, o->store, o->two_queues < 0 ? g_two_queues : o->two_queues != 0, (o->flags & PWS_NETG_DETERMINISTIC) != 0,
                    o->x_sample_stride, (o->flags & PWS_NETG_PRUNE_DEAD) != 0};
    return PWS_OK;
}

struct Seg {
    float *ptr;
    int c, ld;
    unsigned char *sign = nullptr;
};
struct Tn {
    Seg seg[4];
    int nseg, h, w;
};

enum { OP_CONV = 0, OP_THETA = 1, OP_FIELD = 2 };
struct Op {
    int type, layer, act, stage;
    bool nchw;
    Tn in, out;
    float *aux[4] = {nullptr, nullptr, nullptr, nullptr};
};

struct BnCfg {
    const float *params = nullptr;
    float *running = nullptr;
    float momentum = 0.1f, eps = 1e-5f;
};

static hipStream_t shared_side_queue(int dev) {
    static std::mutex m;
    static std::unordered_map<int, hipStream_t> per_device;
    std::lock_guard<std::mutex> lock(m);
    auto it = per_device.find(dev);
    if (it != per_device.end()) return it->second;
    hipStream_t s = nullptr;
    if (hipStreamCreateWithFlags(&s, hipStreamNonBlocking) != hipSuccess) s = nullptr;
    per_device[dev] = s;
    return s;
}
struct SideStream {
    hipStream_t stream = nullptr;
    hipStream_t own = nullptr;
    struct Pool {
        std::vector<hipEvent_t> events;
        size_t next = 0;
    };
    std::unordered_map<hipStream_t, Pool> pools;
    Pool *cur = nullptr;
    int dev = 0;
    void begin(hipStream_t st) { cur = &pools[st], cur->next = 0; }
    hipStream_t pick(hipStream_t st) {
        hipStreamCaptureStatus cm = hipStreamCaptureStatusNone;
        if (hipStreamIsCapturing(st, &cm) != hipSuccess) return nullptr;
        if (cm == hipStreamCaptureStatusNone) {
            if (!stream) stream = shared_side_queue(dev);
            if (!own && hipStreamCreateWithFlags(&own, hipStreamNonBlocking) != hipSuccess) own = nullptr;
            return stream;
        }
        if (cm != hipStreamCaptureStatusActive) return nullptr;
        return own;
    }
    hipEvent_t event() {
        if (!cur) return nullptr;
        if (cur->next == cur->events.size()) {
            hipEvent_t e = nullptr;
            if (hipEventCreateWithFlags(&e, hipEventDisableTiming) != hipSuccess) return nullptr;
            cur->events.push_back(e);
        }
        return cur->events[cur->next++];
    }
};
static SideStream &side_stream() {
    static thread_local std::unordered_map<int, SideStream> per_device;
    int dev = 0;
    (void)hipGetDevice(&dev);
    SideStream &s = per_device[dev];
    s.dev = dev;
    return s;
}

class Exec {
  public:
    Exec(const float *packed, const std::vector<Layer> &layers, int n, char *ws, size_t ws_bytes, hipStream_t st, bool dry,
         bool launch, const NetgOpts &o, const BnCfg *bn = nullptr)
        : math_(o.math), x_sstride_(o.x_sample_stride), prune_dead_(o.prune_dead), packed_(packed), L_(layers), n_(n), ws_(ws), cap_(ws_bytes), dry_(dry), launch_(launch && !dry) {
        if (bn) {
            bn_on_ = true, bn_ = *bn;
            size_t off = 0;
            for (int i = 0; i < L_COUNT; ++i) bn_off_[i] = off, off += 2 * (size_t)layers[i].cout;
            bn_total_ = off;
        }
        io16_ = o.math == PWS_MATH_BF16 && o.store == PWS_STORE_BF16 && layers[L_DOWN1].cin % 32 == 0;
        streams_[0] = st, streams_[1] = st;
        if (launch_ && o.two_queues) {
            side_ = &side_stream();
            if (hipStream_t q = side_->pick(st)) streams_[1] = q, side_->begin(st);
        }
    }

    void use(int q) { q_ = q; }
    bool two_queues() const { return streams_[1] != streams_[0]; }
    hipEvent_t mark(int from) {
        if (!launch_ || !two_queues()) return nullptr;
        hipEvent_t e = side_->event();
        if (!e || hipEventRecord(e, streams_[from]) != hipSuccess) {
            if (rc_ == PWS_OK) set_error("pws_netg_forward: hipEventRecord failed"), rc_ = PWS_EHIP;
            return nullptr;
        }
        return e;
    }
    void wait(int to, hipEvent_t e) {
        if (!e) return;
        if (hipStreamWaitEvent(streams_[to], e, 0) != hipSuccess && rc_ == PWS_OK)
            set_error("pws_netg_forward: hipStreamWaitEvent failed"), rc_ = PWS_EHIP;
    }
    void order(int from, int to) { wait(to, mark(from)); }

    size_t used() const { return off_; }
    int rc() const { return rc_; }
    const std::vector<Op> &tape() const { return tape_; }
    float *splitk_ws() const { return splitk_ws_; }
    float *x_nhwc() const { return x_nhwc_; }
    bool io16() const { return io16_; }
    bool prune_dead() const { return prune_dead_; }
    int math() const { return math_; }
    int store() const { return io16_ ? PWS_STORE_BF16 : PWS_STORE_FP32; }
    float *theta_x32(int q) const { return theta_x32_[q]; }
    size_t splitk_bytes() const { return splitk_bytes_; }
    float *h_saved(int stage) const { return h_saved_[stage]; }
    bool bn_on() const { return bn_on_; }
    size_t bn_off(int layer) const { return bn_off_[layer]; }
    size_t bn_total() const { return bn_total_; }
    float *bn_ws(int q) const { return bn_ws_[q]; }
    size_t bn_ws_bytes() const { return bn_ws_bytes_; }
    const float *gamma(int layer) const { return bn_.params + bn_off_[layer]; }
    const float *beta(int layer) const { return bn_.params + bn_off_[layer] + L_[layer].cout; }
    int bn_forward(int layer, const float *z, size_t pixels, int act, float *y, float *stats, int repeat) {
        const int c = L_[layer].cout;
        float *rm = bn_.running ? bn_.running + bn_off_[layer] : nullptr;
        return pws_bn_train_fwd(z, pixels, c, gamma(layer), beta(layer), act, y, stats, rm, rm ? rm + c : nullptr, bn_.momentum, bn_.eps,
                                repeat, bn_ws_[q_], bn_ws_bytes_, streams_[q_]);
    }

    float *alloc(size_t floats) {
        const size_t bytes = align_up(floats * sizeof(float), 256);
        const size_t at = off_;
        off_ += bytes;
        if (dry_) return nullptr;
        if (off_ > cap_) {
            if (rc_ == PWS_OK) {
                set_error("pws_netg: workspace too small (%zu B needed so far, %zu B given)", off_, cap_);
                rc_ = PWS_ENOMEM;
            }
            return nullptr;
        }
        return reinterpret_cast<float *>(ws_ + at);
    }

    static Tn cat(const Tn &a, const Tn &b) {
        Tn o = a;
        for (int i = 0; i < b.nseg && o.nseg < 4; ++i) o.seg[o.nseg++] = b.seg[i];
        return o;
    }

    static void out_extent(int kind, const Tn &x, int *oh, int *ow) {
        *oh = x.h, *ow = x.w;
        if (kind == PWS_CONV_K3S2) *oh = (x.h - 1) / 2 + 1, *ow = (x.w - 1) / 2 + 1;
        if (kind == PWS_CONVT_K4S2) *oh = 2 * x.h, *ow = 2 * x.w;
    }
    Tn conv(int layer, const Tn &x, int act, const float *nchw_src = nullptr, int nchw_c = 0) {
        const Layer &l = L_[layer];
        int oh, ow;
        out_extent(l.kind, x, &oh, &ow);
        Tn o{};
        o.nseg = 1, o.h = oh, o.w = ow;
        o.seg[0] = Seg{alloc((size_t)n_ * oh * ow * l.cout), l.cout, l.cout};
        if (wants_sign(act, l.cout, ow)) {
            unsigned char *sg = reinterpret_cast<unsigned char *>(alloc(((size_t)n_ * oh * ow * (l.cout / 8) + 3) / 4));
            if (io16_ && !exp_is(EXP_NO_SIGN_BITS)) o.seg[0].sign = sg;
        }
        return run_conv(layer, x, act, o, 1, nchw_src, nchw_c);
    }
    bool wants_sign(int act, int cout, int ow) const { return training_ && !bn_on_ && act != PWS_ACT_NONE && cout % 8 == 0 && ow >= 32; }

    struct Groups {
        float *ptr = nullptr;
        unsigned char *sign = nullptr;
        int c = 0, h = 0, w = 0;
    };
    size_t esz() const { return io16_ ? 2 : 4; }
    Groups alloc_groups(int ngroups, int h, int w, int c, int act) {
        Groups t;
        t.c = c, t.h = h, t.w = w;
        t.ptr = alloc((size_t)ngroups * n_ * h * w * c);
        if (wants_sign(act, c, w)) {
            unsigned char *sg = reinterpret_cast<unsigned char *>(alloc(((size_t)ngroups * n_ * h * w * (c / 8) + 3) / 4));
            if (io16_ && !exp_is(EXP_NO_SIGN_BITS)) t.sign = sg;
        }
        return t;
    }
    Tn group(const Groups &t, int g0) const {
        Tn o{};
        o.nseg = 1, o.h = t.h, o.w = t.w;
        float *p = t.ptr ? reinterpret_cast<float *>(reinterpret_cast<char *>(t.ptr) + (size_t)g0 * n_ * t.h * t.w * t.c * esz()) : nullptr;
        o.seg[0] = Seg{p, t.c, t.c, t.sign ? t.sign + (size_t)g0 * n_ * t.h * t.w * (t.c / 8) : nullptr};
        return o;
    }
    Tn shifted(const Tn &x, int k) const {
        Tn o = x;
        for (int i = 0; i < o.nseg; ++i) {
            Seg &sg = o.seg[i];
            if (sg.ptr) sg.ptr = reinterpret_cast<float *>(reinterpret_cast<char *>(sg.ptr) + (size_t)k * n_ * x.h * x.w * sg.ld * esz());
            if (sg.sign) sg.sign += (size_t)k * n_ * x.h * x.w * (sg.c / 8);
        }
        return o;
    }
    Tn conv_groups(int layer, const Tn &x, int act, int ngroups, const Groups &dst, int g0) {
        return run_conv(layer, x, act, group(dst, g0), ngroups, nullptr, 0);
    }

    Tn run_conv(int layer, const Tn &x, int act, const Tn &o, int ngroups, const float *nchw_src, int nchw_c) {
        const Layer &l = L_[layer];
        const int oh = o.h, ow = o.w;
        Op op{OP_CONV, layer, act, 0, nchw_c > 0, x, o};
        if (bn_on_) op.aux[0] = alloc((size_t)n_ * oh * ow * l.cout), op.aux[1] = alloc(2 * (size_t)l.cout);
        tape_.push_back(op);
        for (int k = 1; k < ngroups; ++k) tape_.push_back(Op{OP_CONV, layer, act, 0, false, shifted(x, k), shifted(o, k)});
        if (!launch_ || rc_ != PWS_OK) return o;
        pws_conv_args a{};
        a.kind = l.kind, a.n = ngroups * n_, a.h = x.h, a.w = x.w;
        if (nchw_c > 0 && math_ == PWS_MATH_BF16 && l.wb_off != (size_t)-1 && x_nhwc_ && nchw_c <= 32) {
            rc_ = nchw_to_nhwc_pad_strided(nchw_src, x_sstride_, x_nhwc_, n_, nchw_c, x.h, x.w, 32, store(), streams_[q_]);
            if (rc_ != PWS_OK) return o;
            a.nsrc = 1, a.src[0] = pws_src{x_nhwc_, 32, 32};
        } else if (nchw_c > 0) {
            a.nsrc = 1, a.src_nchw = 1, a.src[0] = pws_src{nchw_src, nchw_c, (int)x_sstride_};
        } else {
            a.nsrc = x.nseg;
            for (int i = 0; i < x.nseg; ++i) a.src[i] = pws_src{x.seg[i].ptr, x.seg[i].c, x.seg[i].ld};
        }
        a.cout = l.cout, a.w_packed = packed_ + l.w_off, a.bias = packed_ + l.b_off, a.act = bn_on_ ? PWS_ACT_NONE : act;
        a.w_wino = l.ww_off != (size_t)-1 ? packed_ + l.ww_off : nullptr;
        a.w_wring = l.wr_off != (size_t)-1 ? packed_ + l.wr_off : nullptr;
        a.out = bn_on_ ? op.aux[0] : o.seg[0].ptr, a.out_ld = l.cout;
        a.ws = q_ ? splitk_ws2_ : splitk_ws_, a.ws_bytes = math_ == PWS_MATH_FP32 ? splitk_big_ : splitk_bytes_;
        if (math_ == PWS_MATH_BF16 && l.wb_off != (size_t)-1) {
            a.math = PWS_MATH_BF16, a.w_bf16 = packed_ + l.wb_off;
            a.w_wino = a.w_wring = nullptr;
        }
        a.store = store();
        a.out_sign = o.seg[0].sign, a.out_sign_ld = l.cout / 8;
        g_prof_tag = layer;
        rc_ = pws_conv2d_fwd(&a, streams_[q_]);
        g_prof_tag = -1;
        if (bn_on_ && rc_ == PWS_OK) {
            const int repeat = (layer == L_DB1_CS || layer == L_DB1_CS + 1) ? 2 : 1;
            rc_ = bn_forward(layer, op.aux[0], (size_t)n_ * oh * ow, act, o.seg[0].ptr, op.aux[1], repeat);
        }
        return o;
    }

    Tn down(int i, const Tn &x) { return conv(L_DOWN1 + (i - 1), x, PWS_ACT_LRELU); }
    Tn down_bottom(int k, const Tn *x_left, const Tn &x_up) {
        Tn c = conv(L_DB1_CS + 2 * (k - 1), x_up, PWS_ACT_LRELU);
        return conv(L_DB1_CS + 2 * (k - 1) + 1, x_left ? cat(*x_left, c) : c, PWS_ACT_LRELU);
    }
    Tn up(int level, const Tn &x1, const Tn *x2) {
        Tn u = conv(L_UP7 + (7 - level), x1, PWS_ACT_RELU);
        return x2 ? cat(u, *x2) : u;
    }
    Tn up_bottom(int level, const Tn &x_up, const Tn &x_left, const Tn *x_before) {
        Tn e = conv(L_UB7_MP + 2 * (7 - level) + 1, x_up, PWS_ACT_RELU);
        Tn v = conv(L_UB7_MP + 2 * (7 - level), cat(e, x_left), PWS_ACT_RELU);
        return x_before ? cat(v, *x_before) : v;
    }
    void theta(const Tn &x_s8, int stage, float *theta_out) {
        Op op{OP_THETA, L_FLATTEN, 0, stage, false, x_s8, Tn{}};
        if (bn_on_) {
            const int hidden = L_[L_FLATTEN].cout;
            op.aux[0] = alloc((size_t)n_ * hidden), op.aux[1] = alloc(2 * (size_t)hidden);
            op.aux[2] = alloc((size_t)n_ * 6), op.aux[3] = alloc(12);
        }
        tape_.push_back(op);
        if (!launch_ || rc_ != PWS_OK) return;
        const Layer &f = L_[L_FLATTEN], &l = L_[L_LINEAR];
        const float *xin = x_s8.seg[0].ptr;
        if (bn_on_) {
            rc_ = theta_z1(xin, n_, x_s8.seg[0].c, f.cout, packed_ + f.w_off, packed_ + f.b_off, q_ ? theta_ws2_ : theta_ws_, op.aux[0],
                           streams_[q_]);
            if (rc_ == PWS_OK) rc_ = bn_forward(L_FLATTEN, op.aux[0], (size_t)n_, PWS_ACT_LRELU, h_saved_[stage], op.aux[1], 1);
            if (rc_ == PWS_OK) rc_ = theta_z2(h_saved_[stage], n_, f.cout, packed_ + l.w_off, packed_ + l.b_off, op.aux[2], streams_[q_]);
            if (rc_ == PWS_OK) rc_ = bn_forward(L_LINEAR, op.aux[2], (size_t)n_, PWS_ACT_LRELU, theta_out, op.aux[3], 1);
            return;
        }
        if (io16_) {
            rc_ = pws_cvt_bf16_to_f32(xin, theta_x32_[q_], (size_t)n_ * 4 * x_s8.seg[0].c, streams_[q_]);
            if (rc_ != PWS_OK) return;
            xin = theta_x32_[q_];
        }
        rc_ = pws_theta_head_fwd_save(xin, n_, x_s8.seg[0].c, f.cout, packed_ + f.w_off, packed_ + f.b_off,
                                      packed_ + l.w_off, packed_ + l.b_off, q_ ? theta_ws2_ : theta_ws_, theta_out,
                                      h_saved_[stage], streams_[q_]);
    }
    void field(const Tn &x, int stage, const float *theta_k, int ac, float *resid, float *grid) {
        Op op{OP_FIELD, L_OUT, 0, stage, false, x, Tn{}};
        if (bn_on_) {
            const size_t e = (size_t)n_ * x.h * x.w * 2;
            op.aux[0] = alloc(e), op.aux[1] = alloc(4), op.aux[2] = alloc(e);
        }
        tape_.push_back(op);
        if (!launch_ || rc_ != PWS_OK) return;
        const Layer &o = L_[L_OUT];
        if (bn_on_) {
            rc_ = field_head_raw(x.seg[0].ptr, x.seg[0].ld, n_, x.h, x.w, x.seg[0].c, packed_ + o.w_off, packed_ + o.b_off, op.aux[0],
                                 streams_[q_]);
            if (rc_ == PWS_OK) rc_ = bn_forward(L_OUT, op.aux[0], (size_t)n_ * x.h * x.w, PWS_ACT_NONE, op.aux[2], op.aux[1], 1);
            if (rc_ == PWS_OK) rc_ = field_bn_finish(op.aux[2], theta_k, n_, x.h, x.w, ac, resid, grid, streams_[q_]);
            return;
        }
        rc_ = pws_field_head_fwd_s(x.seg[0].ptr, x.seg[0].ld, n_, x.h, x.w, x.seg[0].c, packed_ + o.w_off, packed_ + o.b_off,
                                   theta_k, ac, resid, grid, store(), streams_[q_]);
    }

    void reserve_scratch(int ngf, bool training) {
        training_ = training;
        splitk_bytes_ = (size_t)(2 * n_ > 8 ? 2 * n_ : 8) * (2u << 20);
        splitk_big_ = splitk_bytes_ + ((size_t)48 << 20) < 4 * splitk_bytes_ ? splitk_bytes_ + ((size_t)48 << 20) : 4 * splitk_bytes_;
        splitk_ws_ = alloc(splitk_big_ / sizeof(float));
        splitk_ws2_ = alloc(splitk_big_ / sizeof(float));
        theta_ws_ = alloc(pws_theta_head_ws_floats(n_, 4 * ngf, 8 * ngf));
        theta_ws2_ = alloc(pws_theta_head_ws_floats(n_, 4 * ngf, 8 * ngf));
        if (!splitk_ws_ || !splitk_ws2_) splitk_bytes_ = 0, splitk_big_ = 0;
        for (int s = 0; s < 3; ++s) h_saved_[s] = training ? alloc((size_t)n_ * 8 * ngf) : nullptr;
        x_nhwc_ = alloc((size_t)n_ * 256 * 256 * 32);
        theta_x32_[0] = alloc((size_t)n_ * 16 * ngf), theta_x32_[1] = alloc((size_t)n_ * 16 * ngf);
        if (bn_on_) {
            bn_ws_bytes_ = pws_bn_ws_bytes(16 * ngf);
            bn_ws_[0] = alloc(bn_ws_bytes_ / sizeof(float)), bn_ws_[1] = alloc(bn_ws_bytes_ / sizeof(float));
        }
    }

  private:
    float *splitk_ws_ = nullptr, *splitk_ws2_ = nullptr, *theta_ws_ = nullptr, *theta_ws2_ = nullptr;
    float *h_saved_[3] = {nullptr, nullptr, nullptr};
    float *x_nhwc_ = nullptr;
    float *theta_x32_[2] = {nullptr, nullptr};
    bool bn_on_ = false;
    BnCfg bn_;
    size_t bn_off_[L_COUNT] = {}, bn_total_ = 0, bn_ws_bytes_ = 0;
    float *bn_ws_[2] = {nullptr, nullptr};
    bool io16_ = false, training_ = false;
    int math_ = PWS_MATH_FP32;
    size_t x_sstride_ = 0;
    bool prune_dead_ = false;
    SideStream *side_ = nullptr;
    hipStream_t streams_[2];
    int q_ = 0;
    size_t splitk_bytes_ = 0, splitk_big_ = 0;
    const float *packed_;
    const std::vector<Layer> &L_;
    int n_;
    char *ws_;
    size_t cap_, off_ = 0;
    bool dry_, launch_;
    int rc_ = PWS_OK;
    std::vector<Op> tape_;
};

static void forward_lockstep(Exec &E, const Tn &in, const float *x, int n, int input_nc, int g, int is_training, int ac, float *grids, float *resid,
                             float *th1, float *th2, float *th3) {
    const int S = 256;
    const size_t gsz = (size_t)n * S * S * 2;
    const int enc_c[9] = {0, g, g, 2 * g, 4 * g, 4 * g, 4 * g, 4 * g, 4 * g};
    const int dec_c[8] = {0, g, g, 2 * g, 4 * g, 4 * g, 4 * g, 4 * g};
    auto side = [&](int k) { return S >> (k - 1); };
    Exec::Groups Ek[9], Ck[9], Vl[8], Gl[8];
    for (int k = 2; k <= 8; ++k) Ek[k] = E.alloc_groups(k == 2 ? 2 : 3, side(k), side(k), enc_c[k], PWS_ACT_LRELU);
    for (int k = 3; k <= 8; ++k) Ck[k] = E.alloc_groups(2, side(k - 1), side(k - 1), enc_c[k - 1], PWS_ACT_LRELU);
    for (int l = 7; l >= 2; --l) {
        Vl[l] = E.alloc_groups(3, side(l), side(l), dec_c[l], PWS_ACT_RELU);
        const int cin = l == 7 ? enc_c[8] : dec_c[l + 1] + enc_c[l + 1];
        Gl[l] = E.alloc_groups(2, side(l + 1), side(l + 1), cin, PWS_ACT_RELU);
    }
    auto enc = [&](int k, int s) { return E.group(Ek[k], s - 1); };
    auto dec = [&](int l, int s) {
        if (l == 8) return enc(8, s);
        Tn skip = s == 3 && l == 2 ? enc(2, 2) : enc(l, s);
        return Exec::cat(E.group(Vl[l], s - 1), skip);
    };
    auto db1 = [&](const Tn &x11) {
        Tn c = E.conv(L_DB1_CS, x11, PWS_ACT_LRELU);
        E.conv_groups(L_DB1_CS + 1, c, PWS_ACT_LRELU, 1, Ek[2], 1);
    };
    auto level3 = [&]() {
        E.conv_groups(L_DB1_CS + 2, enc(2, 1), PWS_ACT_LRELU, 2, Ck[3], 0);
        E.conv_groups(L_DB1_CS + 3, Exec::cat(enc(2, 2), E.group(Ck[3], 0)), PWS_ACT_LRELU, 1, Ek[3], 1);
        E.conv_groups(L_DB1_CS + 3, Exec::cat(enc(2, 2), E.group(Ck[3], 1)), PWS_ACT_LRELU, 1, Ek[3], 2);
    };
    auto enc1 = [&](int k, const Tn &x11) { E.conv_groups(L_DOWN1 + (k - 2), k == 2 ? x11 : enc(k - 1, 1), PWS_ACT_LRELU, 1, Ek[k], 0); };
    E.use(0);
    Tn x11 = E.conv(L_TRANSFER, in, PWS_ACT_LRELU, x, input_nc);
    for (int k = 2; k <= 4; ++k) enc1(k, x11);
    E.order(0, 1);
    E.use(1);
    db1(x11);
    level3();
    E.use(0);
    for (int k = 5; k <= 8; ++k) enc1(k, x11);
    E.order(0, 1);
    E.use(1);
    if (is_training) {
        E.use(0);
        E.theta(enc(8, 1), 0, th1);
        E.use(1);
    }
    for (int k = 4; k <= 8; ++k) {
        const int db = k - 1;
        E.conv_groups(L_DB1_CS + 2 * (db - 1), enc(k - 1, 1), PWS_ACT_LRELU, 2, Ck[k], 0);
        E.conv_groups(L_DB1_CS + 2 * (db - 1) + 1, Exec::cat(enc(k - 1, 2), E.group(Ck[k], 0)), PWS_ACT_LRELU, 2, Ek[k], 1);
    }
    E.use(0);
    const int l_last = (!is_training && E.prune_dead()) ? 3 : 2;
    for (int l = 7; l >= l_last; --l) {
        E.conv_groups(L_UP7 + (7 - l), dec(l + 1, 1), PWS_ACT_RELU, 1, Vl[l], 0);
        if (l == 6) E.order(0, 1);
    }
    if (is_training) {
        Tn x111 = E.up(1, dec(2, 1), nullptr);
        E.field(x111, 0, th1, ac, resid, grids);
    }
    auto merged_level = [&](int l) {
        E.conv_groups(L_UB7_MP + 2 * (7 - l) + 1, dec(l + 1, 1), PWS_ACT_RELU, 2, Gl[l], 0);
        E.conv_groups(L_UB7_MP + 2 * (7 - l), Exec::cat(E.group(Gl[l], 0), dec(l + 1, 2)), PWS_ACT_RELU, 2, Vl[l], 1);
    };
    E.use(1);
    for (int l = 7; l >= 5; --l) merged_level(l);
    E.order(1, 0);
    E.use(1);
    if (is_training) E.theta(enc(8, 2), 1, th2);
    E.theta(enc(8, 3), 2, th3);
    hipEvent_t th_done = E.mark(1);
    E.use(0);
    for (int l = 4; l >= 2; --l) merged_level(l);
    E.wait(0, th_done);
    if (is_training) {
        Tn x211 = E.up_bottom(1, dec(2, 1), dec(2, 2), nullptr);
        E.field(x211, 1, th2, ac, resid ? resid + gsz : nullptr, grids ? grids + gsz : nullptr);
    }
    Tn x311 = E.up_bottom(1, dec(2, 2), dec(2, 3), nullptr);
    if (is_training)
        E.field(x311, 2, th3, ac, resid ? resid + 2 * gsz : nullptr, grids ? grids + 2 * gsz : nullptr);
    else
        E.field(x311, 2, th3, ac, nullptr, grids);
}

static void forward_graph(Exec &E, const float *x, int n, int input_nc, int g, int is_training, int ac, float *grids,
                          float *resid, float *thetas, bool caller_thetas = false) {
    const int S = 256;
    E.reserve_scratch(g, is_training != 0);
    const size_t gsz = (size_t)n * S * S * 2;
    float *th = (thetas || caller_thetas) ? thetas : E.alloc((size_t)3 * n * 6);
    float *th1 = th, *th2 = th ? th + (size_t)n * 6 : nullptr, *th3 = th ? th + (size_t)2 * n * 6 : nullptr;

    Tn in{};
    in.nseg = 1, in.h = S, in.w = S, in.seg[0] = Seg{nullptr, input_nc, 0};
    if (!E.bn_on() && !exp_is(EXP_NETG_PER_STAGE)) {
        forward_lockstep(E, in, x, n, input_nc, g, is_training, ac, grids, resid, th1, th2, th3);
        return;
    }
    E.use(0);
    Tn x11 = E.conv(L_TRANSFER, in, PWS_ACT_LRELU, x, input_nc);
    Tn x12 = E.down(1, x11), x13 = E.down(2, x12), x14 = E.down(3, x13), x15 = E.down(4, x14);
    E.order(0, 1);
    E.use(1);
    Tn x22 = E.down_bottom(1, nullptr, x11);
    Tn x23 = E.down_bottom(2, &x22, x12), x24 = E.down_bottom(3, &x23, x13), x25 = E.down_bottom(4, &x24, x14);
    E.use(0);
    Tn x16 = E.down(5, x15), x17 = E.down(6, x16), x18 = E.down(7, x17);
    E.order(0, 1);
    if (is_training) E.theta(x18, 0, th1);
    E.use(1);
    Tn x26 = E.down_bottom(5, &x25, x15), x27 = E.down_bottom(6, &x26, x16), x28 = E.down_bottom(7, &x27, x17);
    hipEvent_t enc2_done = E.mark(1);
    if (is_training) E.theta(x28, 1, th2);
    hipEvent_t th2_done = is_training ? E.mark(1) : nullptr;
    E.use(0);
    Tn x177 = E.up(7, x18, &x17), x166 = E.up(6, x177, &x16), x155 = E.up(5, x166, &x15);
    Tn x144 = E.up(4, x155, &x14), x133 = E.up(3, x144, &x13), x122 = E.up(2, x133, &x12);
    if (is_training) {
        Tn x111 = E.up(1, x122, nullptr);
        E.field(x111, 0, th1, ac, resid, grids);
    }
    E.use(1);
    const Tn &x32 = x22;
    Tn x33 = E.down_bottom(2, &x32, x22), x34 = E.down_bottom(3, &x33, x23), x35 = E.down_bottom(4, &x34, x24);
    Tn x36 = E.down_bottom(5, &x35, x25), x37 = E.down_bottom(6, &x36, x26), x38 = E.down_bottom(7, &x37, x27);
    hipEvent_t enc3_done = E.mark(1);
    E.wait(0, enc2_done);
    E.use(0);
    Tn x277 = E.up_bottom(7, x18, x28, &x27), x266 = E.up_bottom(6, x177, x277, &x26);
    Tn x255 = E.up_bottom(5, x166, x266, &x25);
    hipEvent_t dec2_deep = E.mark(0);
    const bool deep_on_q1 = !E.bn_on();
    Tn x377{}, x366{}, x355{};
    hipEvent_t dec3_deep = nullptr;
    if (deep_on_q1) {
        E.use(1);
        E.wait(1, dec2_deep);
        x377 = E.up_bottom(7, x28, x38, &x37), x366 = E.up_bottom(6, x277, x377, &x36), x355 = E.up_bottom(5, x266, x366, &x35);
        dec3_deep = E.mark(1);
        E.use(0);
    }
    Tn x244 = E.up_bottom(4, x155, x255, &x24);
    Tn x233 = E.up_bottom(3, x144, x244, &x23), x222 = E.up_bottom(2, x133, x233, &x22);
    if (is_training) {
        Tn x211 = E.up_bottom(1, x122, x222, nullptr);
        E.wait(0, th2_done);
        E.field(x211, 1, th2, ac, resid ? resid + gsz : nullptr, grids ? grids + gsz : nullptr);
    }
    E.use(1);
    E.theta(x38, 2, th3);
    hipEvent_t th3_done = E.mark(1);
    E.use(0);
    E.wait(0, enc3_done);
    if (deep_on_q1) E.wait(0, dec3_deep);
    else x377 = E.up_bottom(7, x28, x38, &x37), x366 = E.up_bottom(6, x277, x377, &x36), x355 = E.up_bottom(5, x266, x366, &x35);
    Tn x344 = E.up_bottom(4, x255, x355, &x34);
    Tn x333 = E.up_bottom(3, x244, x344, &x33), x322 = E.up_bottom(2, x233, x333, &x32);
    Tn x311 = E.up_bottom(1, x222, x322, nullptr);
    E.wait(0, th3_done);
    if (is_training)
        E.field(x311, 2, th3, ac, resid ? resid + 2 * gsz : nullptr, grids ? grids + 2 * gsz : nullptr);
    else
        E.field(x311, 2, th3, ac, nullptr, grids);
}

struct GradBuf {
    float *g;
    bool written;
    bool preact;
};

struct UpGrads {
    const float *grids[3] = {nullptr, nullptr, nullptr}, *resid[3] = {nullptr, nullptr, nullptr};
    UpGrads() = default;
    UpGrads(const float *g_grids, const float *g_resid, size_t gsz) {
        for (int k = 0; k < 3; ++k) grids[k] = g_grids ? g_grids + k * gsz : nullptr, resid[k] = g_resid ? g_resid + k * gsz : nullptr;
    }
    UpGrads(const float *const *g_grids, const float *const *g_resid) {
        for (int k = 0; k < 3; ++k) grids[k] = g_grids ? g_grids[k] : nullptr, resid[k] = g_resid ? g_resid[k] : nullptr;
    }
    bool any() const {
        for (int k = 0; k < 3; ++k)
            if (grids[k] || resid[k]) return true;
        return false;
    }
};

static int run_backward(const float *packed, const float *packed_dgrad, const float *x, int n, int input_nc, int g, int ac,
                        char *ws, size_t ws_bytes, const float *resid, const float *thetas, const UpGrads &up, float *dpacked,
                        hipStream_t st, bool dry, size_t *used, int part = 0,
                        int nparts = 1, unsigned char *final_mask = nullptr, const BnCfg *bn = nullptr, float *dbn = nullptr,
                        const NetgOpts *opts = nullptr) {
    const int S = 256;
    size_t total = 0, total_grad = 0;
    const std::vector<Layer> L = build_layers(input_nc, g, &total, nullptr, &total_grad);
    const NetgOpts mode = opts ? *opts : opts_defaults();
    DeterministicScope det_scope(mode.deterministic);
    Exec E(packed, L, n, ws, ws_bytes, st, dry, false, mode, bn);
    forward_graph(E, x, n, input_nc, g, 1, ac, nullptr, nullptr, nullptr, true);
    std::unordered_map<const float *, GradBuf> G;
    for (size_t i = 0; i < E.tape().size(); ++i) {
        const Op &op = E.tape()[i];
        if (op.type != OP_CONV) continue;
        const Seg &o = op.out.seg[0];
        float *gp = E.alloc((size_t)n * op.out.h * op.out.w * o.c);
        if (!dry) G[o.ptr] = GradBuf{gp, false, false};
    }
    float *gz_ws = E.alloc((size_t)n * S * S * 2);
    float *th_bwd_ws = E.alloc((size_t)n * 8 * g);
    float *dtheta = E.alloc((size_t)3 * n * 6);
    float *th_dx32 = E.alloc((size_t)n * 16 * g);
    const size_t abb_bytes = pws_act_bwd_bias_ws_bytes(16 * g);
    float *abb_ws = E.alloc(abb_bytes / sizeof(float));
    if (used) *used = E.used();
    if (dry) return PWS_OK;
    if (E.rc() != PWS_OK) return E.rc();

    if (part == 0 && bn && dbn) {
        hipError_t e = hipMemsetAsync(dbn, 0, E.bn_total() * sizeof(float), st);
        if (e != hipSuccess) {
            set_error("pws_netg_backward: hipMemsetAsync: %s", hipGetErrorString(e));
            return PWS_EHIP;
        }
    }
    auto bn_backward = [&](int layer, float *dy, const float *y, const float *z, const float *stats, int act, size_t pixels) {
        const int c = L[layer].cout;
        float *dg = dbn + E.bn_off(layer);
        return pws_bn_train_bwd(dy, y, z, stats, E.gamma(layer), act, pixels, c, dg, dg + c, E.bn_ws(0), E.bn_ws_bytes(), st);
    };
    if (part == 0) {
        hipError_t e = hipMemsetAsync(dpacked, 0, total_grad * sizeof(float), st);
        if (e != hipSuccess) {
            set_error("pws_netg_backward: hipMemsetAsync: %s", hipGetErrorString(e));
            return PWS_EHIP;
        }
    }
    const size_t T = E.tape().size();
    const size_t r_begin = T * (size_t)part / nparts, r_end = T * (size_t)(part + 1) / nparts;
    hipStream_t wst = st;
    SideStream *wside = nullptr;
    if (mode.two_queues) {
        wside = &side_stream();
        if (hipStream_t q = wside->pick(st)) wst = q, wside->begin(st);
        else wside = nullptr;
    }
    auto wgrad_fork = [&]() -> int {
        if (wst == st) return PWS_OK;
        hipEvent_t e = wside->event();
        if (!e || hipEventRecord(e, st) != hipSuccess || hipStreamWaitEvent(wst, e, 0) != hipSuccess) {
            set_error("pws_netg_backward: event record / wait on the weight-gradient queue failed");
            return PWS_EHIP;
        }
        return PWS_OK;
    };
    if (final_mask) {
        for (int i = 0; i < L_COUNT; ++i) final_mask[i] = 1;
        for (size_t ii = 0; ii < T; ++ii) {
            if (T - 1 - ii < r_end) continue;
            const Op &op = E.tape()[ii];
            if (op.type == OP_FIELD) final_mask[L_OUT] = 0;
            else if (op.type == OP_THETA) final_mask[L_FLATTEN] = 0, final_mask[L_LINEAR] = 0;
            else final_mask[op.layer] = 0;
        }
    }
    const size_t gsz = (size_t)n * S * S * 2;
    std::unordered_map<const float *, size_t> last_writer, producer;
    const bool fuse_act = E.io16() && !bn && mode.math == PWS_MATH_BF16;
    if (fuse_act) {
        std::unordered_map<const float *, bool> wr;
        bool hd[3] = {false, false, false};
        for (size_t ii = T; ii-- > 0;) {
            const Op &op = E.tape()[ii];
            if (op.type == OP_FIELD) {
                const float *gg = up.grids[op.stage], *gr = up.resid[op.stage];
                if (!gg && !gr) continue;
                wr[op.in.seg[0].ptr] = true, last_writer[op.in.seg[0].ptr] = ii, hd[op.stage] = gg != nullptr;
            } else if (op.type == OP_THETA) {
                if (!hd[op.stage]) continue;
                wr[op.in.seg[0].ptr] = true, last_writer[op.in.seg[0].ptr] = ii;
            } else {
                producer[op.out.seg[0].ptr] = ii;
                if (!wr[op.out.seg[0].ptr] || op.nchw) continue;
                for (int i = 0; i < op.in.nseg; ++i) wr[op.in.seg[i].ptr] = true, last_writer[op.in.seg[i].ptr] = ii;
            }
        }
    }
    auto fused_act = [&](size_t ii, const float *t) -> int {
        if (!fuse_act) return PWS_ACT_NONE;
        const auto lw = last_writer.find(t);
        const auto pr = producer.find(t);
        if (lw == last_writer.end() || lw->second != ii || pr == producer.end()) return PWS_ACT_NONE;
        const Op &pop = E.tape()[pr->second];
        if (E.tape()[ii].type == OP_THETA) return PWS_ACT_NONE;
        if (E.tape()[ii].type == OP_CONV && L[E.tape()[ii].layer].dgb_off == (size_t)-1) return PWS_ACT_NONE;
        return pop.act == PWS_ACT_LRELU || pop.act == PWS_ACT_RELU ? pop.act : PWS_ACT_NONE;
    };
    bool have_dtheta[3] = {false, false, false};
    int rc = PWS_OK;
    int layer_uses[L_COUNT] = {};
    for (size_t ii = 0; ii < T; ++ii)
        if (E.tape()[ii].type == OP_CONV) ++layer_uses[E.tape()[ii].layer];
    std::unordered_map<int, pws_conv_bwd_weight_args> pending;
    for (size_t ii = T; ii-- > 0 && rc == PWS_OK;) {
        const Op &op = E.tape()[ii];
        const size_t r = T - 1 - ii;
        if (r >= r_end) break;
        const bool run = r >= r_begin;
        if (op.type == OP_FIELD) {
            const int k = op.stage;
            const float *gg = up.grids[k], *gr = up.resid[k];
            if (!gg && !gr) continue;
            const Seg &xs = op.in.seg[0];
            GradBuf &gb = G[xs.ptr];
            const Layer &o = L[L_OUT];
            if (run && bn) {
                rc = field_bwd_gz(resid + k * gsz, gg, gr, n, op.in.h, op.in.w, ac, gz_ws, nullptr, gg ? dtheta + (size_t)k * n * 6 : nullptr, st);
                if (rc == PWS_OK) rc = bn_backward(L_OUT, gz_ws, nullptr, op.aux[0], op.aux[1], PWS_ACT_NONE, (size_t)n * op.in.h * op.in.w);
                if (rc == PWS_OK)
                    rc = field_bwd_dx_dw(xs.ptr, xs.ld, gz_ws, n, op.in.h, op.in.w, xs.c, packed + o.w_off, gb.g, xs.c, gb.written ? 1 : 0,
                                         dpacked + o.gw_off, E.store(), st);
            } else if (run)
                rc = pws_field_head_bwd_act(xs.ptr, xs.ld, n, op.in.h, op.in.w, xs.c, packed + o.w_off, resid + k * gsz, gg, gr, ac, gb.g,
                                            xs.c, gb.written ? 1 : 0, dpacked + o.gw_off, dpacked + o.gb_off,
                                            gg ? dtheta + (size_t)k * n * 6 : nullptr, gz_ws, E.store(), fused_act(ii, xs.ptr), st);
            gb.written = true;
            if (fused_act(ii, xs.ptr) != PWS_ACT_NONE) gb.preact = true;
            have_dtheta[k] = gg != nullptr;
        } else if (op.type == OP_THETA) {
            const int k = op.stage;
            if (!have_dtheta[k]) continue;
            const Seg &xs = op.in.seg[0];
            GradBuf &gb = G[xs.ptr];
            const Layer &f = L[L_FLATTEN], &l = L[L_LINEAR];
            if (!run) {
                gb.written = true;
                continue;
            }
            if (bn) {
                float *dz2 = dtheta + (size_t)k * n * 6;
                rc = bn_backward(L_LINEAR, dz2, thetas + (size_t)k * n * 6, op.aux[2], op.aux[3], PWS_ACT_LRELU, (size_t)n);
                if (rc == PWS_OK) rc = theta_bwd_bn_lin(dz2, E.h_saved(k), n, f.cout, packed + l.w_off, dpacked + l.gw_off, th_bwd_ws, st);
                if (rc == PWS_OK) rc = bn_backward(L_FLATTEN, th_bwd_ws, E.h_saved(k), op.aux[0], op.aux[1], PWS_ACT_LRELU, (size_t)n);
                if (rc == PWS_OK)
                    rc = theta_bwd_flat(xs.ptr, n, xs.c, f.cout, packed + f.w_off, th_bwd_ws, dpacked + f.gw_off, gb.g, gb.written ? 1 : 0, st);
                gb.written = true;
                continue;
            }
            if (E.io16()) {
                const size_t cnt = (size_t)n * 4 * xs.c;
                rc = pws_cvt_bf16_to_f32(xs.ptr, E.theta_x32(0), cnt, st);
                if (rc == PWS_OK)
                    rc = pws_theta_head_bwd(E.theta_x32(0), n, xs.c, f.cout, packed + f.w_off, packed + l.w_off, E.h_saved(k),
                                            thetas + (size_t)k * n * 6, dtheta + (size_t)k * n * 6, dpacked + f.gw_off,
                                            dpacked + f.gb_off, dpacked + l.gw_off, dpacked + l.gb_off, th_dx32, 0, th_bwd_ws, st);
                if (rc == PWS_OK) rc = pws_cvt_f32_to_bf16(th_dx32, gb.g, cnt, gb.written ? 1 : 0, st);
            } else {
                rc = pws_theta_head_bwd(xs.ptr, n, xs.c, f.cout, packed + f.w_off, packed + l.w_off, E.h_saved(k),
                                        thetas + (size_t)k * n * 6, dtheta + (size_t)k * n * 6, dpacked + f.gw_off, dpacked + f.gb_off,
                                        dpacked + l.gw_off, dpacked + l.gb_off, gb.g, gb.written ? 1 : 0, th_bwd_ws, st);
            }
            gb.written = true;
        } else {
            const Layer &l = L[op.layer];
            const Seg &o = op.out.seg[0];
            GradBuf &go = G[o.ptr];
            if (!go.written) continue;
            const size_t pixels = (size_t)n * op.out.h * op.out.w;
            auto make_wa = [&]() {
                pws_conv_bwd_weight_args wa{};
                wa.kind = l.kind, wa.n = n, wa.h = op.in.h, wa.w = op.in.w, wa.nsrc = op.in.nseg, wa.src_nchw = op.nchw ? 1 : 0;
                for (int i = 0; i < op.in.nseg; ++i) wa.src[i] = pws_src{op.in.seg[i].ptr, op.in.seg[i].c, op.in.seg[i].ld};
                if (op.nchw) wa.src[0] = pws_src{x, input_nc, 0};
                if (op.nchw && mode.math == PWS_MATH_BF16 && l.wb_off != (size_t)-1 && E.x_nhwc() && input_nc <= 32)
                    wa.src_nchw = 0, wa.src[0] = pws_src{E.x_nhwc(), 32, 32};
                wa.cout = l.cout, wa.gout = go.g, wa.gout_ld = l.cout, wa.dw_packed = dpacked + l.gw_off;
                wa.math = mode.math, wa.store = E.store();
                wa.dbias = !bn && go.preact && !mode.deterministic ? dpacked + l.gb_off : nullptr;
                return wa;
            };
            const bool shared = !bn && !op.nchw && layer_uses[op.layer] == 2;
            pws_conv_bwd_weight_args extra{};
            auto pair_up = [&](pws_conv_bwd_weight_args wa) {
                if (!shared) return wa;
                auto mine = pending.find(op.layer);
                if (mine == pending.end()) {
                    pending.emplace(op.layer, wa);
                    wa.nsrc = 0;
                    return wa;
                }
                const pws_conv_bwd_weight_args first = mine->second;
                pending.erase(mine);
                if ((first.dbias != nullptr) != (wa.dbias != nullptr)) {
                    extra = first;
                    return wa;
                }
                for (int i = 0; i < wa.nsrc; ++i) wa.src2_ptr[i] = first.src[i].ptr;
                wa.gout2 = first.gout;
                return wa;
            };
            if (!run) {
                if (!op.nchw)
                    for (int i = 0; i < op.in.nseg; ++i) {
                        GradBuf &gi = G[op.in.seg[i].ptr];
                        gi.written = true;
                        if (fused_act(ii, op.in.seg[i].ptr) != PWS_ACT_NONE) gi.preact = true;
                    }
                (void)pair_up(make_wa());
                continue;
            }
            g_prof_tag = op.layer;
            if (bn)
                rc = bn_backward(op.layer, go.g, o.ptr, op.aux[0], op.aux[1], op.act, pixels);
            else if (!go.preact)
                rc = pws_act_bwd_bias_s(go.g, o.ptr, pixels, l.cout, op.act, dpacked + l.gb_off, E.store(), abb_ws, abb_bytes, st);
            else if (mode.deterministic)
                rc = pws_act_bwd_bias_s(go.g, go.g, pixels, l.cout, PWS_ACT_NONE, dpacked + l.gb_off, E.store(), abb_ws, abb_bytes, st);
            if (rc != PWS_OK) break;
            const pws_conv_bwd_weight_args wa = pair_up(make_wa());
            if (wa.nsrc > 0 || extra.nsrc > 0) {
                rc = wgrad_fork();
                if (rc == PWS_OK && extra.nsrc > 0) rc = pws_conv2d_bwd_weight(&extra, wst);
                if (rc == PWS_OK && wa.nsrc > 0) rc = pws_conv2d_bwd_weight(&wa, wst);
            }
            if (rc != PWS_OK || op.nchw) {
                g_prof_tag = -1;
                continue;
            }
            pws_conv_bwd_data_args da{};
            da.kind = l.kind, da.n = n, da.h = op.in.h, da.w = op.in.w, da.cout = l.cout, da.gout = go.g, da.gout_ld = l.cout;
            da.w_dgrad = packed_dgrad + l.dg_off, da.ndst = op.in.nseg;
            for (int i = 0; i < op.in.nseg; ++i) {
                GradBuf &gi = G[op.in.seg[i].ptr];
                da.dst[i] = pws_dst{gi.g, op.in.seg[i].c, op.in.seg[i].c, gi.written ? 1 : 0, nullptr, 0, PWS_ACT_NONE, nullptr, 0};
                gi.written = true;
                const int fa = fused_act(ii, op.in.seg[i].ptr);
                if (fa != PWS_ACT_NONE)
                    da.dst[i].act_y = op.in.seg[i].ptr, da.dst[i].act_y_ld = op.in.seg[i].ld, da.dst[i].act = fa, gi.preact = true,
                    da.dst[i].act_sign = op.in.seg[i].sign, da.dst[i].act_sign_ld = op.in.seg[i].c / 8;
            }
            da.ws = E.splitk_ws(), da.ws_bytes = E.splitk_bytes();
            if (mode.math == PWS_MATH_BF16 && l.dgb_off != (size_t)-1) da.math = PWS_MATH_BF16, da.w_dgrad_bf16 = packed_dgrad + l.dgb_off;
            da.store = E.store();
            rc = pws_conv2d_bwd_data(&da, st);
            g_prof_tag = -1;
        }
    }
    if (rc == PWS_OK && !pending.empty()) {
        for (auto &kv : pending) {
            size_t last_r = 0;
            for (size_t ii = 0; ii < T; ++ii)
                if (E.tape()[ii].type == OP_CONV && E.tape()[ii].layer == kv.first) { last_r = T - 1 - ii; break; }
            if (last_r < r_begin || last_r >= r_end) continue;
            rc = wgrad_fork();
            if (rc == PWS_OK) rc = pws_conv2d_bwd_weight(&kv.second, wst);
            if (rc != PWS_OK) break;
        }
    }
    if (wst != st) {
        hipEvent_t e = wside->event();
        if (!e || hipEventRecord(e, wst) != hipSuccess || hipStreamWaitEvent(st, e, 0) != hipSuccess) {
            if (rc == PWS_OK) set_error("pws_netg_backward: joining the weight-gradient queue failed"), rc = PWS_EHIP;
        }
    }
    return rc;
}

}

using namespace pws;

extern "C" size_t pws_netg_packed_floats(int input_nc, int ngf) {
    if (input_nc <= 0 || ngf <= 0 || ngf % 16 != 0) return 0;
    size_t total = 0;
    build_layers(input_nc, ngf, &total);
    return total;
}

extern "C" size_t pws_netg_packed_dgrad_floats(int input_nc, int ngf) {
    if (input_nc <= 0 || ngf <= 0 || ngf % 16 != 0) return 0;
    size_t total = 0, dg = 0;
    build_layers(input_nc, ngf, &total, &dg);
    return dg;
}

extern "C" int pws_netg_pack_weights(const float *const *params, float *packed, int input_nc, int ngf, pws_stream_t stream) {
    return pws_netg_pack_weights_for(params, packed, input_nc, ngf, -1, stream);
}

static int pack_weights_impl(const float *const *params, float *packed, int input_nc, int ngf, int math, pws_stream_t stream, const bool *skip) {
    PWS_REQUIRE(params && packed, "pws_netg_pack_weights: NULL pointer");
    PWS_REQUIRE(input_nc > 0 && ngf > 0 && ngf % 16 == 0, "pws_netg_pack_weights: ngf must be a positive multiple of 16 (got %d)",
                ngf);
    size_t total = 0;
    const std::vector<Layer> L = build_layers(input_nc, ngf, &total);
    PWS_REQUIRE(total < 0xffffffffu, "pws_netg_pack_weights: packed buffer too large for 32-bit offsets");
    PackAllArgs a{};
    Bf16AllArgs b{};
    a.nlayers = b.nlayers = L_COUNT;
    fill_pack_layers(L, a.layer);
    unsigned nb = 0, nbw = 0, nbb = 0;
    for (int i = 0; i < L_COUNT; ++i) {
        PWS_REQUIRE(params[2 * i] && params[2 * i + 1], "pws_netg_pack_weights: params[%d] is NULL", 2 * i);
        a.params[2 * i] = params[2 * i], a.params[2 * i + 1] = params[2 * i + 1];
        const PackLayer &p = a.layer[i];
        const bool sk = skip && skip[i];
        a.first_block[i] = nb;
        if (sk) ;
        else if (pack_tiled(p.kind)) nb += pack_tiles(p.kind, p.cin_pad, p.cout, p.k) + (unsigned)((p.cout + 255) / 256);
        else nb += (unsigned)(((size_t)p.planes * p.cin_pad * p.cout + p.cout + 255) / 256);
        a.first_block_wino[i] = nbw;
        const bool skip_wino = sk || (math == PWS_MATH_BF16 && L[i].wb_off != (size_t)-1);
        if ((p.ww_off != kNoOff || p.wr_off != kNoOff) && !skip_wino) nbw += (unsigned)(((size_t)p.cin_pad * p.cout + 255) / 256);
        Bf16Layer &q = b.layer[i];
        q.planes = p.planes, q.krows = p.cin_pad, q.ncols = p.cout, q.kpad = (p.cin_pad + 31) / 32 * 32, q.npad = (p.cout + 63) / 64 * 64;
        q.src_off = p.w_off, q.dst_off = sk ? kNoOff : off32(L[i].wb_off);
        b.first_block[i] = nbb;
        if (q.dst_off != kNoOff && math != PWS_MATH_FP32) nbb += (unsigned)(q.planes * (q.kpad / 32) * (q.npad / 64));
    }
    a.total_blocks = nb, a.total_blocks_wino = nbw, b.total_blocks = nbb;
    int rc = launch_pack_all(a, packed, as_stream(stream));
    if (rc == PWS_OK && nbb) rc = launch_bf16_all(b, packed, packed, as_stream(stream));
    return rc;
}

extern "C" int pws_netg_pack_weights_for(const float *const *params, float *packed, int input_nc, int ngf, int math, pws_stream_t stream) {
    return pack_weights_impl(params, packed, input_nc, ngf, math, stream, nullptr);
}

static int pack_weights_dgrad_impl(const float *const *params, float *packed_dgrad, int input_nc, int ngf, pws_stream_t stream, const bool *skip) {
    PWS_REQUIRE(params && packed_dgrad, "pws_netg_pack_weights_dgrad: NULL pointer");
    PWS_REQUIRE(input_nc > 0 && ngf > 0 && ngf % 16 == 0, "pws_netg_pack_weights_dgrad: bad ngf %d", ngf);
    size_t total = 0, dg = 0;
    const std::vector<Layer> L = build_layers(input_nc, ngf, &total, &dg);
    PWS_REQUIRE(dg < 0xffffffffu, "pws_netg_pack_weights_dgrad: buffer too large for 32-bit offsets");
    PackAllArgs a{};
    Bf16AllArgs b{};
    a.nlayers = b.nlayers = L_COUNT;
    fill_pack_layers(L, a.layer);
    unsigned nb = 0, nbb = 0;
    for (int i = 0; i < L_COUNT; ++i) {
        a.params[2 * i] = params[2 * i], a.params[2 * i + 1] = nullptr;
        const PackLayer &p = a.layer[i];
        a.first_block_dgrad[i] = nb;
        Bf16Layer &q = b.layer[i];
        q = Bf16Layer{};
        q.dst_off = kNoOff;
        b.first_block[i] = nbb;
        if (p.dg_off == kNoOff || (skip && skip[i])) continue;
        PWS_REQUIRE(params[2 * i], "pws_netg_pack_weights_dgrad: params[%d] is NULL", 2 * i);
        if (pack_tiled(p.kind)) nb += pack_tiles(p.kind, p.cin, p.cout, p.k);
        else nb += (unsigned)(((size_t)p.dg_taps * p.cin * p.cout + 255) / 256);
        q.planes = p.dg_taps, q.krows = p.cout, q.ncols = p.cin, q.kpad = (p.cout + 31) / 32 * 32, q.npad = (p.cin + 63) / 64 * 64;
        q.src_off = p.dg_off, q.dst_off = off32(L[i].dgb_off);
        if (q.dst_off != kNoOff) nbb += (unsigned)(q.planes * (q.kpad / 32) * (q.npad / 64));
    }
    a.total_blocks_dgrad = nb, b.total_blocks = nbb;
    int rc = nb ? launch_dgrad_all(a, packed_dgrad, as_stream(stream)) : PWS_OK;
    if (rc == PWS_OK) rc = launch_bf16_all(b, packed_dgrad, packed_dgrad, as_stream(stream));
    return rc;
}

extern "C" int pws_netg_pack_weights_dgrad(const float *const *params, float *packed_dgrad, int input_nc, int ngf,
                                           pws_stream_t stream) {
    return pack_weights_dgrad_impl(params, packed_dgrad, input_nc, ngf, stream, nullptr);
}

extern "C" int pws_netg_pack_weights_train(const float *const *params, float *packed, float *packed_dgrad, int input_nc, int ngf, int math,
                                           pws_stream_t stream) {
    PWS_REQUIRE(params && packed && packed_dgrad, "pws_netg_pack_weights_train: NULL pointer");
    PWS_REQUIRE(input_nc > 0 && ngf > 0 && ngf % 16 == 0, "pws_netg_pack_weights_train: ngf must be a positive multiple of 16 (got %d)", ngf);
    bool fused[L_COUNT] = {};
    int nfused = 0;
    size_t total = 0, dg = 0;
    const std::vector<Layer> L = build_layers(input_nc, ngf, &total, &dg);
    PWS_REQUIRE(total < 0xffffffffu && dg < 0xffffffffu, "pws_netg_pack_weights_train: buffers too large for 32-bit offsets");
    Pack16Args f{};
    f.nlayers = L_COUNT;
    fill_pack_layers(L, f.layer);
    unsigned nb = 0;
    for (int i = 0; i < L_COUNT; ++i) {
        PWS_REQUIRE(params[2 * i] && params[2 * i + 1], "pws_netg_pack_weights_train: params[%d] is NULL", 2 * i);
        f.params[2 * i] = params[2 * i], f.params[2 * i + 1] = params[2 * i + 1];
        const PackLayer &p = f.layer[i];
        const Layer &l = L[i];
        const bool has_dg = l.dg_off != (size_t)-1;
        bool ok = math == PWS_MATH_BF16 && !exp_is(EXP_NO_PACK_ONE_PASS) && pack_tiled(p.kind) && l.wb_off != (size_t)-1 && p.cout % 64 == 0 && p.cin_pad % 32 == 0;
        if (ok && has_dg) ok = l.dgb_off != (size_t)-1 && p.cin % 64 == 0;
        ok = ok && ngf % 32 == 0;
        if (i == L_TRANSFER) ok = ok && input_nc <= 32;
        fused[i] = ok, nfused += ok ? 1 : 0;
        f.first_block[i] = nb;
        f.wb_off[i] = ok ? off32(l.wb_off) : kNoOff;
        f.dgb_off[i] = ok && has_dg ? off32(l.dgb_off) : kNoOff;
        if (ok) nb += pack_tiles(p.kind, p.cin_pad, p.cout, p.k) + (unsigned)((p.cout + 255) / 256);
    }
    f.total_blocks = nb;
    int rc = nfused ? launch_pack16_all(f, packed, packed_dgrad, as_stream(stream)) : PWS_OK;
    if (rc == PWS_OK) rc = pack_weights_impl(params, packed, input_nc, ngf, math, stream, nfused ? fused : nullptr);
    if (rc == PWS_OK) rc = pack_weights_dgrad_impl(params, packed_dgrad, input_nc, ngf, stream, nfused ? fused : nullptr);
    return rc;
}

extern "C" int pws_netg_backward_part(const float *packed, const float *packed_dgrad, const float *x, int n, int input_nc, int ngf,
                                      int align_corners, void *ws, size_t ws_bytes, const float *resid, const float *thetas,
                                      const float *g_grids, const float *g_resid, float *dpacked, int part, int nparts,
                                      unsigned char *final_mask, pws_stream_t stream) {
    return pws_netg_backward_opts(packed, packed_dgrad, x, n, input_nc, ngf, align_corners, ws, ws_bytes, resid, thetas, g_grids, g_resid,
                                  dpacked, part, nparts, final_mask, nullptr, stream);
}

extern "C" size_t pws_netg_bn_floats(int input_nc, int ngf) {
    if (input_nc <= 0 || ngf <= 0 || ngf % 16 != 0) return 0;
    size_t total = 0, bn = 0;
    for (const Layer &l : build_layers(input_nc, ngf, &total)) bn += 2 * (size_t)l.cout;
    return bn;
}

extern "C" size_t pws_netg_train_workspace_bytes_bn(int n, int input_nc, int ngf) {
    if (n <= 0 || input_nc <= 0 || ngf <= 0 || ngf % 16 != 0) return 0;
    size_t used = 0;
    BnCfg bn;
    const NetgOpts o{PWS_MATH_FP32, PWS_STORE_FP32, false};
    run_backward(nullptr, nullptr, nullptr, n, input_nc, ngf, 0, nullptr, 0, nullptr, nullptr, UpGrads(), nullptr, nullptr, true,
                 &used, 0, 1, nullptr, &bn, nullptr, &o);
    return used;
}

static int bn_opts_from(const pws_netg_opts *opts, NetgOpts *o) {
    *o = NetgOpts{PWS_MATH_FP32, PWS_STORE_FP32, g_two_queues};
    if (!opts) return PWS_OK;
    NetgOpts u;
    if (int rc = opts_from(opts, &u)) return rc;
    PWS_REQUIRE(u.store == PWS_STORE_FP32 && u.x_sample_stride == 0,
                "pws_netg_*_bn_opts: the BatchNorm training path stores fp32 activations (store must be PWS_STORE_FP32) and reads a dense window");
    o->math = u.math, o->two_queues = u.two_queues, o->deterministic = u.deterministic;
    return PWS_OK;
}

extern "C" int pws_netg_forward_bn(const float *packed, const float *bn_params, float *bn_running, float momentum, float eps,
                                   const float *x, int n, int input_nc, int ngf, int align_corners, void *ws, size_t ws_bytes,
                                   float *grids, float *resid, float *thetas, pws_stream_t stream) {
    return pws_netg_forward_bn_opts(packed, bn_params, bn_running, momentum, eps, x, n, input_nc, ngf, align_corners, ws, ws_bytes, grids, resid,
                                    thetas, nullptr, stream);
}

extern "C" int pws_netg_forward_bn_opts(const float *packed, const float *bn_params, float *bn_running, float momentum, float eps,
                                        const float *x, int n, int input_nc, int ngf, int align_corners, void *ws, size_t ws_bytes,
                                        float *grids, float *resid, float *thetas, const pws_netg_opts *opts, pws_stream_t stream) {
    PWS_REQUIRE(n >= 0 && input_nc > 0 && ngf > 0 && ngf % 16 == 0, "pws_netg_forward_bn: bad n/input_nc/ngf %d/%d/%d", n, input_nc, ngf);
    if (n == 0) return PWS_OK;
    PWS_REQUIRE(n >= 2, "pws_netg_forward_bn: training-mode BatchNorm needs more than 1 value per channel (the theta head has one per "
                        "sample): n >= 2, as torch");
    PWS_REQUIRE(packed && bn_params && x && ws && grids && resid && thetas, "pws_netg_forward_bn: NULL pointer");
    PWS_REQUIRE((reinterpret_cast<size_t>(ws) & 255) == 0, "pws_netg_forward_bn: workspace must be 256-byte aligned");
    size_t total = 0;
    const std::vector<Layer> L = build_layers(input_nc, ngf, &total);
    BnCfg bn;
    bn.params = bn_params, bn.running = bn_running, bn.momentum = momentum, bn.eps = eps;
    NetgOpts o;
    if (int rc = bn_opts_from(opts, &o)) return rc;
    Exec E(packed, L, n, static_cast<char *>(ws), ws_bytes, as_stream(stream), false, true, o, &bn);
    forward_graph(E, x, n, input_nc, ngf, 1, align_corners, grids, resid, thetas);
    return E.rc();
}

extern "C" int pws_netg_backward_bn(const float *packed, const float *packed_dgrad, const float *bn_params, float eps, const float *x,
                                    int n, int input_nc, int ngf, int align_corners, void *ws, size_t ws_bytes, const float *resid,
                                    const float *thetas, const float *g_grids, const float *g_resid, float *dpacked, float *dbn,
                                    pws_stream_t stream) {
    return pws_netg_backward_bn_opts(packed, packed_dgrad, bn_params, eps, x, n, input_nc, ngf, align_corners, ws, ws_bytes, resid, thetas, g_grids,
                                     g_resid, dpacked, dbn, nullptr, stream);
}

extern "C" int pws_netg_backward_bn_opts(const float *packed, const float *packed_dgrad, const float *bn_params, float eps, const float *x,
                                         int n, int input_nc, int ngf, int align_corners, void *ws, size_t ws_bytes, const float *resid,
                                         const float *thetas, const float *g_grids, const float *g_resid, float *dpacked, float *dbn,
                                         const pws_netg_opts *opts, pws_stream_t stream) {
    PWS_REQUIRE(n >= 2 && input_nc > 0 && ngf > 0 && ngf % 16 == 0, "pws_netg_backward_bn: bad n/input_nc/ngf");
    PWS_REQUIRE(packed && packed_dgrad && bn_params && x && ws && resid && thetas && dpacked && dbn, "pws_netg_backward_bn: NULL pointer");
    PWS_REQUIRE(g_grids || g_resid, "pws_netg_backward_bn: no output gradient given");
    PWS_REQUIRE((reinterpret_cast<size_t>(ws) & 255) == 0, "pws_netg_backward_bn: workspace must be 256-byte aligned");
    BnCfg bn;
    bn.params = bn_params, bn.eps = eps;
    NetgOpts o;
    if (int rc = bn_opts_from(opts, &o)) return rc;
    return run_backward(packed, packed_dgrad, x, n, input_nc, ngf, align_corners, static_cast<char *>(ws), ws_bytes, resid, thetas,
                        UpGrads(g_grids, g_resid, (size_t)n * 256 * 256 * 2), dpacked, as_stream(stream), false, nullptr, 0, 1, nullptr, &bn, dbn, &o);
}

extern "C" int pws_netg_unpack_grads(const float *dpacked, float *const *grads, int input_nc, int ngf, pws_stream_t stream) {
    PWS_REQUIRE(dpacked && grads, "pws_netg_unpack_grads: NULL pointer");
    PWS_REQUIRE(input_nc > 0 && ngf > 0 && ngf % 16 == 0, "pws_netg_unpack_grads: bad ngf %d", ngf);
    size_t total = 0;
    const std::vector<Layer> L = build_layers(input_nc, ngf, &total);
    UnpackAllArgs a{};
    a.nlayers = L_COUNT;
    fill_pack_layers(L, a.layer);
    for (int i = 0; i < L_COUNT; ++i) a.layer[i].w_off = off32(L[i].gw_off), a.layer[i].b_off = off32(L[i].gb_off);
    unsigned nb = 0;
    for (int i = 0; i < L_COUNT; ++i) {
        PWS_REQUIRE((grads[2 * i] != nullptr) == (grads[2 * i + 1] != nullptr), "pws_netg_unpack_grads: grads[%d], grads[%d]: one is NULL",
                    2 * i, 2 * i + 1);
        a.grads[2 * i] = grads[2 * i], a.grads[2 * i + 1] = grads[2 * i + 1];
        const PackLayer &p = a.layer[i];
        a.first_block[i] = nb;
        if (grads[2 * i] && pack_tiled(p.kind)) nb += pack_tiles(p.kind, p.cin, p.cout, p.k) + (unsigned)((p.cout + 255) / 256);
        else if (grads[2 * i]) nb += (unsigned)(((size_t)p.k * p.k * p.cin * p.cout + p.cout + 255) / 256);
    }
    a.total_blocks = nb;
    if (nb == 0) return PWS_OK;
    return launch_unpack_all(a, dpacked, as_stream(stream));
}

extern "C" size_t pws_netg_workspace_bytes(int n, int input_nc, int ngf, int is_training) {
    if (n <= 0 || input_nc <= 0 || ngf <= 0 || ngf % 16 != 0) return 0;
    size_t total = 0;
    const std::vector<Layer> L = build_layers(input_nc, ngf, &total);
    Exec E(nullptr, L, n, nullptr, 0, nullptr, true, false, NetgOpts{PWS_MATH_FP32, PWS_STORE_FP32, false});
    forward_graph(E, nullptr, n, input_nc, ngf, is_training, 0, nullptr, nullptr, nullptr);
    return E.used();
}

extern "C" int pws_netg_backward_plan(int input_nc, int ngf, int nparts, unsigned char *final_part) {
    PWS_REQUIRE(input_nc > 0 && ngf > 0 && ngf % 16 == 0, "pws_netg_backward_plan: bad input_nc / ngf %d / %d", input_nc, ngf);
    PWS_REQUIRE(nparts >= 1 && nparts <= 255 && final_part, "pws_netg_backward_plan: nparts %d (1..255) / NULL pointer", nparts);
    size_t total = 0;
    const std::vector<Layer> L = build_layers(input_nc, ngf, &total);
    Exec E(nullptr, L, 1, nullptr, 0, nullptr, true, false, NetgOpts{PWS_MATH_FP32, PWS_STORE_FP32, false});
    forward_graph(E, nullptr, 1, input_nc, ngf, 1, 0, nullptr, nullptr, nullptr, true);
    const size_t T = E.tape().size();
    size_t last[L_COUNT];
    bool used[L_COUNT];
    for (int i = 0; i < L_COUNT; ++i) last[i] = 0, used[i] = false;
    auto touch = [&](int layer, size_t rpos) { last[layer] = used[layer] ? std::max(last[layer], rpos) : rpos, used[layer] = true; };
    for (size_t ii = 0; ii < T; ++ii) {
        const Op &op = E.tape()[ii];
        const size_t rpos = T - 1 - ii;
        if (op.type == OP_FIELD) touch(L_OUT, rpos);
        else if (op.type == OP_THETA) touch(L_FLATTEN, rpos), touch(L_LINEAR, rpos);
        else touch(op.layer, rpos);
    }
    for (int i = 0; i < L_COUNT; ++i) {
        int part = 0;
        while (used[i] && part < nparts - 1 && !(last[i] < T * (size_t)(part + 1) / nparts)) ++part;
        final_part[i] = (unsigned char)part;
    }
    return PWS_OK;
}

extern "C" size_t pws_netg_train_workspace_bytes(int n, int input_nc, int ngf) {
    if (n <= 0 || input_nc <= 0 || ngf <= 0 || ngf % 16 != 0) return 0;
    size_t used = 0;
    const NetgOpts o{PWS_MATH_FP32, PWS_STORE_FP32, false};
    run_backward(nullptr, nullptr, nullptr, n, input_nc, ngf, 0, nullptr, 0, nullptr, nullptr, UpGrads(), nullptr, nullptr,
                 true, &used, 0, 1, nullptr, nullptr, nullptr, &o);
    return used;
}

extern "C" int pws_netg_forward_opts(const float *packed, const float *x, int n, int input_nc, int ngf, int is_training,
                                     int align_corners, void *ws, size_t ws_bytes, float *grids, float *resid, float *thetas,
                                     const pws_netg_opts *opts, pws_stream_t stream) {
    PWS_REQUIRE(n >= 0 && input_nc > 0 && ngf > 0 && ngf % 16 == 0, "pws_netg_forward: bad n/input_nc/ngf %d/%d/%d", n, input_nc,
                ngf);
    NetgOpts o;
    if (int rc = opts_from(opts, &o)) return rc;
    if (n == 0) return PWS_OK;
    PWS_REQUIRE(packed && x && ws && grids, "pws_netg_forward: NULL pointer");
    PWS_REQUIRE(!is_training || (resid && thetas), "pws_netg_forward: resid and thetas must be given when is_training");
    PWS_REQUIRE(o.x_sample_stride == 0 || (!is_training && o.x_sample_stride % 4 == 0 && o.x_sample_stride < (1u << 30)),
                "pws_netg_opts: x_sample_stride %zu: inference forward only, a multiple of 4 floats", o.x_sample_stride);
    PWS_REQUIRE((reinterpret_cast<size_t>(ws) & 255) == 0, "pws_netg_forward: workspace must be 256-byte aligned");
    size_t total = 0;
    const std::vector<Layer> L = build_layers(input_nc, ngf, &total);
    Exec E(packed, L, n, static_cast<char *>(ws), ws_bytes, as_stream(stream), false, true, o);
    forward_graph(E, x, n, input_nc, ngf, is_training, align_corners, grids, resid, thetas);
    return E.rc();
}

extern "C" int pws_netg_forward(const float *packed, const float *x, int n, int input_nc, int ngf, int is_training,
                                int align_corners, void *ws, size_t ws_bytes, float *grids, float *resid, float *thetas,
                                pws_stream_t stream) {
    return pws_netg_forward_opts(packed, x, n, input_nc, ngf, is_training, align_corners, ws, ws_bytes, grids, resid, thetas, nullptr,
                                 stream);
}

static int backward_entry(const float *packed, const float *packed_dgrad, const float *x, int n, int input_nc, int ngf, int align_corners,
                          void *ws, size_t ws_bytes, const float *resid, const float *thetas, const UpGrads &up, float *dpacked, int part,
                          int nparts, unsigned char *final_mask, const pws_netg_opts *opts, pws_stream_t stream) {
    PWS_REQUIRE(n >= 0 && input_nc > 0 && ngf > 0 && ngf % 16 == 0, "pws_netg_backward: bad n/input_nc/ngf");
    PWS_REQUIRE(nparts >= 1 && part >= 0 && part < nparts, "pws_netg_backward: part %d of %d", part, nparts);
    NetgOpts o;
    if (int rc = opts_from(opts, &o)) return rc;
    PWS_REQUIRE(o.x_sample_stride == 0, "pws_netg_backward: x_sample_stride is an option of the inference forward (the backward reads a dense window)");
    if (n == 0) {
        if (final_mask)
            for (int i = 0; i < L_COUNT; ++i) final_mask[i] = 1;
        return PWS_OK;
    }
    PWS_REQUIRE(packed && packed_dgrad && x && ws && resid && thetas && dpacked, "pws_netg_backward: NULL pointer");
    PWS_REQUIRE(up.any(), "pws_netg_backward: no output gradient given");
    PWS_REQUIRE((reinterpret_cast<size_t>(ws) & 255) == 0, "pws_netg_backward: workspace must be 256-byte aligned");
    return run_backward(packed, packed_dgrad, x, n, input_nc, ngf, align_corners, static_cast<char *>(ws), ws_bytes, resid, thetas, up,
                        dpacked, as_stream(stream), false, nullptr, part, nparts, final_mask, nullptr, nullptr, &o);
}

extern "C" int pws_netg_backward_opts(const float *packed, const float *packed_dgrad, const float *x, int n, int input_nc, int ngf,
                                      int align_corners, void *ws, size_t ws_bytes, const float *resid, const float *thetas,
                                      const float *g_grids, const float *g_resid, float *dpacked, int part, int nparts,
                                      unsigned char *final_mask, const pws_netg_opts *opts, pws_stream_t stream) {
    return backward_entry(packed, packed_dgrad, x, n, input_nc, ngf, align_corners, ws, ws_bytes, resid, thetas,
                          UpGrads(g_grids, g_resid, (size_t)(n > 0 ? n : 0) * 256 * 256 * 2), dpacked, part, nparts, final_mask, opts, stream);
}

extern "C" int pws_netg_backward_lists(const float *packed, const float *packed_dgrad, const float *x, int n, int input_nc, int ngf,
                                       int align_corners, void *ws, size_t ws_bytes, const float *resid, const float *thetas,
                                       const float *const *g_grids, const float *const *g_resid, float *dpacked, int part, int nparts,
                                       unsigned char *final_mask, const pws_netg_opts *opts, pws_stream_t stream) {
    return backward_entry(packed, packed_dgrad, x, n, input_nc, ngf, align_corners, ws, ws_bytes, resid, thetas, UpGrads(g_grids, g_resid),
                          dpacked, part, nparts, final_mask, opts, stream);
}

extern "C" size_t pws_netg_grad_floats(int input_nc, int ngf) {
    if (input_nc <= 0 || ngf <= 0 || ngf % 16 != 0) return 0;
    size_t total = 0, total_grad = 0;
    build_layers(input_nc, ngf, &total, nullptr, &total_grad);
    return total_grad;
}

extern "C" int pws_netg_grad_layout(int input_nc, int ngf, size_t *first_float, size_t *floats) {
    PWS_REQUIRE(input_nc > 0 && ngf > 0 && ngf % 16 == 0, "pws_netg_grad_layout: bad ngf %d", ngf);
    PWS_REQUIRE(first_float && floats, "pws_netg_grad_layout: NULL pointer");
    size_t total = 0, total_grad = 0;
    const std::vector<Layer> L = build_layers(input_nc, ngf, &total, nullptr, &total_grad);
    for (int i = 0; i < L_COUNT; ++i) {
        first_float[i] = L[i].gw_off;
        floats[i] = (i + 1 < L_COUNT ? L[i + 1].gw_off : total_grad) - L[i].gw_off;
    }
    return PWS_OK;
}

extern "C" int pws_netg_backward(const float *packed, const float *packed_dgrad, const float *x, int n, int input_nc, int ngf,
                                 int align_corners, void *ws, size_t ws_bytes, const float *resid, const float *thetas,
                                 const float *g_grids, const float *g_resid, float *dpacked, pws_stream_t stream) {
    return pws_netg_backward_opts(packed, packed_dgrad, x, n, input_nc, ngf, align_corners, ws, ws_bytes, resid, thetas, g_grids, g_resid,
                                  dpacked, 0, 1, nullptr, nullptr, stream);
}
```

### pwstablenet_amd/hipabi.py

```python
import contextlib
import ctypes
import os

_HERE = os.path.dirname(os.path.abspath(__file__))
LIB_PATH = os.environ.get("PWS_LIB_PATH") or os.path.join(_HERE, "libpwstable_hip.so")

c_f32p = ctypes.c_void_p
c_stream = ctypes.c_void_p

ACT_NONE, ACT_LRELU, ACT_RELU = 0, 1, 2
OPT_TWO_QUEUES = 1
OPT_MATH, MATH_FP32, MATH_BF16 = 2, 0, 1
OPT_STORE, STORE_FP32, STORE_BF16 = 3, 0, 1
ABI_VERSION = 5
NETG_DETERMINISTIC = 1
NETG_PRUNE_DEAD = 2
OPT_EXPERIMENT = 100


class Exp:
    GS_BWD_GENERAL = 2
    U8_CVT_SHIFT = 4
    GS_ROWWIN = 5
    NO_SIGN_BITS = 12
    NETG_PER_STAGE = 15
    RING_OFF = 20
    RING_SMALL = 21
    RINGF_OFF = 22
    RINGF_8X32 = 23
    RINGF_16X32 = 24
    FIRST_MFMA = 25
    FIRST_NO_WINO = 26
    RINGF_32CH = 27
    FIRST_SMALL = 29
    WINO5_SMALL = 30
    HEAD_V1 = 35
    GS_U8_LANE_WINDOWS = 49
    WRING_OFF = 50
    WRING_FORCE = 58
    WRING_MODE2 = 59
    SKINNY_OFF = 70
    SKINNY16_OFF = 71
    SKINNY16_4096 = 72
    SKINNY_SKIP = 73
    WGRAD_RING_OFF = 80
    WGRAD_RING_FORCE = 81
    HEAD_VALU = 90
    HEAD_BWD_VALU = 91
    HEAD_ONE_TILE = 92
    DEEP_TILE_ALWAYS = 96
    SHAPE_GENERAL = 97
    TL1_TILED = 98
    RING_8WAVE = 105
    SMOOTH_ONE_PIXEL = 110
    NO_PACK_ONE_PASS = 120
    RING_UNIT256 = 186
    RING_UNIT128 = 187
    WGRAD_NO_MERGE = 188
    WGRAD_MIN_TILES = 190
    FIRST_ABLATE = 1100
    FIRST_CLOCK = 1200
    WINO5_ABLATE = 1300
    WGRAD_WIDE_ABLATE = 1400
    RING_ABLATE = 1500
    WINO_ABLATE = 1600
    BF16_PROBE = 2100
    RINGF_VARIANT = 2200
    PARITY_LEDGER = 3000
    WRING_ABLATE = 4000
OBJ_SLOTS = 64
CONV_K3S1, CONV_K3S2, CONV_K5S1, CONVT_K3S1, CONVT_K4S2, CONV_K2S1P0, CONV_K1, CONV_K3S1_OUT = range(8)


class PwsSrc(ctypes.Structure):
    _fields_ = [("ptr", ctypes.c_void_p), ("channels", ctypes.c_int), ("ld", ctypes.c_int)]


class PwsConvArgs(ctypes.Structure):
    _fields_ = [("kind", ctypes.c_int), ("n", ctypes.c_int), ("h", ctypes.c_int), ("w", ctypes.c_int),
                ("nsrc", ctypes.c_int), ("src", PwsSrc * 4), ("src_nchw", ctypes.c_int), ("cout", ctypes.c_int),
                ("w_packed", ctypes.c_void_p), ("bias", ctypes.c_void_p), ("act", ctypes.c_int),
                ("out", ctypes.c_void_p), ("out_ld", ctypes.c_int), ("w_wino", ctypes.c_void_p), ("ws", ctypes.c_void_p),
                ("ws_bytes", ctypes.c_size_t), ("math", ctypes.c_int), ("w_bf16", ctypes.c_void_p), ("store", ctypes.c_int),
                ("w_wring", ctypes.c_void_p), ("out_sign", ctypes.c_void_p), ("out_sign_ld", ctypes.c_int)]


class PwsDst(ctypes.Structure):
    _fields_ = [("ptr", ctypes.c_void_p), ("channels", ctypes.c_int), ("ld", ctypes.c_int), ("accumulate", ctypes.c_int),
                ("act_y", ctypes.c_void_p), ("act_y_ld", ctypes.c_int), ("act", ctypes.c_int),
                ("act_sign", ctypes.c_void_p), ("act_sign_ld", ctypes.c_int)]


class PwsConvBwdDataArgs(ctypes.Structure):
    _fields_ = [("kind", ctypes.c_int), ("n", ctypes.c_int), ("h", ctypes.c_int), ("w", ctypes.c_int), ("cout", ctypes.c_int),
                ("gout", ctypes.c_void_p), ("gout_ld", ctypes.c_int), ("w_dgrad", ctypes.c_void_p), ("ndst", ctypes.c_int),
                ("dst", PwsDst * 4), ("ws", ctypes.c_void_p), ("ws_bytes", ctypes.c_size_t), ("math", ctypes.c_int),
                ("w_dgrad_bf16", ctypes.c_void_p), ("store", ctypes.c_int)]


class PwsConvBwdWeightArgs(ctypes.Structure):
    _fields_ = [("kind", ctypes.c_int), ("n", ctypes.c_int), ("h", ctypes.c_int), ("w", ctypes.c_int), ("nsrc", ctypes.c_int),
                ("src", PwsSrc * 4), ("src_nchw", ctypes.c_int), ("cout", ctypes.c_int), ("gout", ctypes.c_void_p),
                ("gout_ld", ctypes.c_int), ("dw_packed", ctypes.c_void_p), ("math", ctypes.c_int), ("store", ctypes.c_int),
                ("dbias", ctypes.c_void_p), ("deterministic", ctypes.c_int), ("src2_ptr", ctypes.c_void_p * 4), ("gout2", ctypes.c_void_p)]


class PwsNetgOpts(ctypes.Structure):
    _fields_ = [("math", ctypes.c_int), ("store", ctypes.c_int), ("two_queues", ctypes.c_int), ("flags", ctypes.c_int),
                ("x_sample_stride", ctypes.c_size_t)]


class PwsProfRecord(ctypes.Structure):
    _fields_ = [("kernel_id", ctypes.c_int), ("tag", ctypes.c_int), ("flops", ctypes.c_double),
                ("bytes", ctypes.c_double), ("ms", ctypes.c_float)]


_I, _S, _P = ctypes.c_int, ctypes.c_size_t, ctypes.c_void_p
_F = ctypes.c_float
SIGNATURES = {
    "pws_version": (_I, []),
    "pws_last_error": (ctypes.c_char_p, []),
    "pws_set_option": (_I, [_I, _I]),
    "pws_get_option": (_I, [_I]),
    "pws_packed_bf16_floats": (_S, [_I, _I, _I]),
    "pws_pack_weight_bf16": (_I, [_P, _P, _I, _I, _I, _P]),
    "pws_nchw_to_nhwc_pad": (_I, [_P, _P, _I, _I, _I, _I, _I, _P]),
    "pws_nchw_to_nhwc_pad_s": (_I, [_P, _P, _I, _I, _I, _I, _I, _I, _P]),
    "pws_cvt_bf16_to_f32": (_I, [_P, _P, _S, _P]),
    "pws_cvt_f32_to_bf16": (_I, [_P, _P, _S, _I, _P]),
    "pws_device_info": (_I, [ctypes.POINTER(_I), ctypes.POINTER(_I)]),
    "pws_packed_weight_floats": (_S, [_I, _I, _I]),
    "pws_pack_conv_weight": (_I, [_P, _P, _I, _I, _I, _P]),
    "pws_packed_wino_floats": (_S, [_I, _I]),
    "pws_pack_conv_weight_wino": (_I, [_P, _P, _I, _I, _P]),
    "pws_packed_wring_floats": (_S, [_I, _I, _I]),
    "pws_pack_conv_weight_wring": (_I, [_P, _P, _I, _I, _I, _P]),
    "pws_packed_wino_ct4_floats": (_S, [_I, _I]),
    "pws_pack_conv_weight_wino_ct4": (_I, [_P, _P, _I, _I, _P]),
    "pws_conv2d_fwd": (_I, [ctypes.POINTER(PwsConvArgs), _P]),
    "pws_act_bwd_bias": (_I, [_P, _P, _S, _I, _I, _P, _P]),
    "pws_act_bwd_bias_s": (_I, [_P, _P, _S, _I, _I, _P, _I, _P, _S, _P]),
    "pws_act_bwd_bias_ws_bytes": (_S, [_I]),
    "pws_packed_dgrad_floats": (_S, [_I, _I, _I]),
    "pws_pack_conv_weight_dgrad": (_I, [_P, _P, _I, _I, _I, _P]),
    "pws_conv2d_bwd_data": (_I, [ctypes.POINTER(PwsConvBwdDataArgs), _P]),
    "pws_conv2d_bwd_weight": (_I, [ctypes.POINTER(PwsConvBwdWeightArgs), _P]),
    "pws_unpack_conv_weight": (_I, [_P, _P, _I, _I, _I, _P]),
    "pws_theta_head_fwd_save": (_I, [_P, _I, _I, _I, _P, _P, _P, _P, _P, _P, _P, _P]),
    "pws_theta_head_bwd": (_I, [_P, _I, _I, _I, _P, _P, _P, _P, _P, _P, _P, _P, _P, _P, _I, _P, _P]),
    "pws_field_head_bwd": (_I, [_P, _I, _I, _I, _I, _I, _P, _P, _P, _P, _I, _P, _I, _I, _P, _P, _P, _P, _P]),
    "pws_field_head_bwd_s": (_I, [_P, _I, _I, _I, _I, _I, _P, _P, _P, _P, _I, _P, _I, _I, _P, _P, _P, _P, _I, _P]),
    "pws_field_head_bwd_act": (_I, [_P, _I, _I, _I, _I, _I, _P, _P, _P, _P, _I, _P, _I, _I, _P, _P, _P, _P, _I, _I, _P]),
    "pws_netg_packed_dgrad_floats": (_S, [_I, _I]),
    "pws_netg_pack_weights_dgrad": (_I, [ctypes.POINTER(_P), _P, _I, _I, _P]),
    "pws_netg_train_workspace_bytes": (_S, [_I, _I, _I]),
    "pws_netg_backward": (_I, [_P, _P, _P, _I, _I, _I, _I, _P, _S, _P, _P, _P, _P, _P, _P]),
    "pws_netg_backward_part": (_I, [_P, _P, _P, _I, _I, _I, _I, _P, _S, _P, _P, _P, _P, _P, _I, _I, _P, _P]),
    "pws_netg_bn_floats": (_S, [_I, _I]),
    "pws_netg_train_workspace_bytes_bn": (_S, [_I, _I, _I]),
    "pws_netg_forward_bn": (_I, [_P, _P, _P, _F, _F, _P, _I, _I, _I, _I, _P, _S, _P, _P, _P, _P]),
    "pws_netg_backward_bn": (_I, [_P, _P, _P, _F, _P, _I, _I, _I, _I, _P, _S, _P, _P, _P, _P, _P, _P, _P]),
    "pws_netg_forward_bn_opts": (_I, [_P, _P, _P, _F, _F, _P, _I, _I, _I, _I, _P, _S, _P, _P, _P, ctypes.POINTER(PwsNetgOpts), _P]),
    "pws_netg_backward_bn_opts": (_I, [_P, _P, _P, _F, _P, _I, _I, _I, _I, _P, _S, _P, _P, _P, _P, _P, _P, ctypes.POINTER(PwsNetgOpts), _P]),
    "pws_netg_unpack_grads": (_I, [_P, ctypes.POINTER(_P), _I, _I, _P]),
    "pws_theta_head_ws_floats": (_S, [_I, _I, _I]),
    "pws_theta_head_fwd": (_I, [_P, _I, _I, _I, _P, _P, _P, _P, _P, _P, _P]),
    "pws_field_head_fwd": (_I, [_P, _I, _I, _I, _I, _I, _P, _P, _P, _I, _P, _P, _P]),
    "pws_field_head_fwd_s": (_I, [_P, _I, _I, _I, _I, _I, _P, _P, _P, _I, _P, _P, _I, _P]),
    "pws_affine_grid": (_I, [_P, _P, _I, _I, _I, _I, _P]),
    "pws_grid_sample_fwd": (_I, [_P, _P, _P, _I, _I, _I, _I, _I, _I, _I, _P]),
    "pws_grid_sample_bwd": (_I, [_P, _P, _P, _P, _P, _I, _I, _I, _I, _I, _I, _I, _P]),
    "pws_upsample_bilinear_ac": (_I, [_P, _P, _I, _I, _I, _I, _I, _I, _P]),
    "pws_upsample_bilinear_ac_bwd": (_I, [_P, _P, _I, _I, _I, _I, _I, _I, _P]),
    "pws_affine_grid_bwd": (_I, [_P, _P, _I, _I, _I, _I, _P]),
    "pws_upsample_grid_sample_fwd": (_I, [_P, _P, _P, _I, _I, _I, _I, _I, _I, _I, _P]),
    "pws_upsample_grid_sample_u8": (_I, [_P, _P, _P, _I, _I, _I, _I, _I, _I, _I, _P]),
    "pws_adam_step": (_I, [_P, _P, _P, _P, _S, _F, _F, _F, _F, _I, _P]),
    "pws_adam_step_multi": (_I, [_P, _P, _P, _P, _P, _I, _F, _F, _F, _F, _I, _P]),
    "pws_netg_packed_floats": (_S, [_I, _I]),
    "pws_netg_pack_weights": (_I, [ctypes.POINTER(_P), _P, _I, _I, _P]),
    "pws_netg_pack_weights_for": (_I, [ctypes.POINTER(_P), _P, _I, _I, _I, _P]),
    "pws_netg_pack_weights_train": (_I, [ctypes.POINTER(_P), _P, _P, _I, _I, _I, _P]),
    "pws_netg_workspace_bytes": (_S, [_I, _I, _I, _I]),
    "pws_netg_forward": (_I, [_P, _P, _I, _I, _I, _I, _I, _P, _S, _P, _P, _P, _P]),
    "pws_netg_forward_opts": (_I, [_P, _P, _I, _I, _I, _I, _I, _P, _S, _P, _P, _P, ctypes.POINTER(PwsNetgOpts), _P]),
    "pws_netg_backward_opts": (_I, [_P, _P, _P, _I, _I, _I, _I, _P, _S, _P, _P, _P, _P, _P, _I, _I, _P, ctypes.POINTER(PwsNetgOpts), _P]),
    "pws_netg_backward_lists": (_I, [_P, _P, _P, _I, _I, _I, _I, _P, _S, _P, _P, ctypes.POINTER(_P), ctypes.POINTER(_P), _P, _I, _I, _P,
                                     ctypes.POINTER(PwsNetgOpts), _P]),
    "pws_netg_grad_floats": (_S, [_I, _I]),
    "pws_netg_grad_layout": (_I, [_I, _I, ctypes.POINTER(_S), ctypes.POINTER(_S)]),
    "pws_netg_backward_plan": (_I, [_I, _I, _I, ctypes.POINTER(ctypes.c_ubyte)]),
    "pws_u8_normalize": (_I, [_P, _S, _P, _S, _I, _S, _P]),
    "pws_warp_norm_fwd": (_I, [_P, _S, _P, _P, _P, _S, _P, _I, _I, _I, _P]),
    "pws_warp_norm_bwd": (_I, [_P, _S, _P, _P, _S, _F, _P, _P, _P, _I, _I, _I, _I, _P]),
    "pws_temporal_l1_fwd": (_I, [_P, _P, _P, _P, _I, _I, _I, _P]),
    "pws_temporal_l1_bwd": (_I, [_P, _P, _P, _F, _P, _P, _P, _I, _I, _I, _P]),
    "pws_temporal_l1_bwd_det": (_I, [_P, _P, _P, _F, _P, _P, _P, _P, _I, _I, _I, _P]),
    "pws_feature_loss_fwd": (_I, [_P, _P, _P, _I, _I, _I, _I, _P]),
    "pws_feature_loss_bwd": (_I, [_P, _P, _F, _P, _P, _I, _I, _I, _I, _P]),
    "pws_feature_loss_bwd_det": (_I, [_P, _P, _F, _P, _P, _I, _I, _I, _I, _P]),
    "pws_field_smoothness": (_I, [_P, _P, _P, _I, _I, _I, _P]),
    "pws_shape_loss_fwd": (_I, [_P, _P, _I, _I, _I, _P]),
    "pws_shape_loss_bwd": (_I, [_P, ctypes.c_double, _P, _P, _I, _I, _I, _P]),
    "pws_objective_finalize": (_I, [_P, _I, _P, _I, _P, _P]),
    "pws_maxpool2x2_fwd": (_I, [_P, _P, _I, _I, _I, _I, _P]),
    "pws_maxpool2x2_bwd": (_I, [_P, _P, _P, _I, _I, _I, _I, _P]),
    "pws_maxpool2x2_fwd_s": (_I, [_P, _P, _I, _I, _I, _I, _I, _P]),
    "pws_maxpool2x2_bwd_s": (_I, [_P, _P, _P, _I, _I, _I, _I, _I, _I, _P]),
    "pws_sqdiff_sum": (_I, [_P, _P, _S, _P, _P]),
    "pws_sqdiff_bwd": (_I, [_P, _P, _S, _F, _P, _P, _P]),
    "pws_gray_area_u8": (_I, [_P, _P, _I, _I, _I, _I, _I, _I, _I, _P]),
    "pws_area_half_u8": (_I, [_P, _P, _I, _I, _I, _I, _P]),
    "pws_area_resize_u8": (_I, [_P, _P, _I, _I, _I, _I, _I, _I, _P]),
    "pws_gray_area_yuv420_u8": (_I, [_P, _P, _I, _I, _I, _I, _I, _I, _I, _P]),
    "pws_area_resize_plane_u8": (_I, [_P, _S, _P, _S, _I, _I, _I, _I, _I, _I, _P]),
    "pws_upsample_grid_sample_yuv420_u8": (_I, [_P, _P, _P, _I, _I, _I, _I, _I, _I, _I, _P]),
    "pws_field_homography": (_I, [_P, _I, _I, _I, _I, _I, _P, _P, _P, _P]),
    "pws_bn_ws_bytes": (_S, [_I]),
    "pws_bn_train_fwd": (_I, [_P, _S, _I, _P, _P, _I, _P, _P, _P, _P, _F, _F, _I, _P, _S, _P]),
    "pws_bn_train_bwd": (_I, [_P, _P, _P, _P, _P, _I, _S, _I, _P, _P, _P, _S, _P]),
    "pws_prof_enable": (_I, [_I]),
    "pws_prof_collect": (_I, [ctypes.POINTER(PwsProfRecord), _I]),
    "pws_prof_kernel_name": (ctypes.c_char_p, [_I]),
}

_lib = None


def lib():
    global _lib
    if _lib is None:
        if not os.path.exists(LIB_PATH):
            raise RuntimeError(
                "pwstablenet_amd: %s is missing -- build it with `python -m pwstablenet_amd.build` "
                "(there is no CPU fallback for the HIP hot path)" % LIB_PATH)
        import torch
        L = ctypes.CDLL(LIB_PATH)
        for name, (res, args) in SIGNATURES.items():
            fn = getattr(L, name)
            fn.restype, fn.argtypes = res, args
        if L.pws_version() != ABI_VERSION:
            raise RuntimeError("pwstablenet_amd: ABI version mismatch (%d)" % L.pws_version())
        _lib = L
    return _lib


@contextlib.contextmanager
def experiment(exp):
    L = lib()
    prev = L.pws_get_option(OPT_EXPERIMENT)
    check(L.pws_set_option(OPT_EXPERIMENT, exp), "pws_set_option(PWS_OPT_EXPERIMENT, %d)" % exp)
    try:
        yield
    finally:
        L.pws_set_option(OPT_EXPERIMENT, prev)


def check(rc, what=""):
    if rc != 0:
        raise RuntimeError("pwstable HIP call %s failed (rc=%d): %s" % (what, rc, lib().pws_last_error().decode()))


def current_stream():
    import torch
    return ctypes.c_void_p(torch.cuda.current_stream().cuda_stream)


def cu_masked_streams(shares, device=None):
    import torch
    dev = torch.cuda.current_device() if device is None else torch.device(device).index
    key = (dev, tuple(int(n) for n in shares))
    if key in _cu_streams:
        return list(_cu_streams[key])
    ncu = torch.cuda.get_device_properties(dev).multi_processor_count
    if sum(shares) > ncu or min(shares) < 1:
        raise ValueError("cu_masked_streams: %r does not fit %d compute units" % (list(shares), ncu))
    hip = ctypes.CDLL("libamdhip64.so")
    words = (ncu + 31) // 32
    out, first = [], 0
    with torch.cuda.device(dev):
        for n in shares:
            bits = ((1 << n) - 1) << first
            mask = (ctypes.c_uint32 * words)(*[(bits >> (32 * w)) & 0xffffffff for w in range(words)])
            st = ctypes.c_void_p()
            rc = hip.hipExtStreamCreateWithCUMask(ctypes.byref(st), ctypes.c_uint32(words), mask)
            if rc != 0 or not st.value:
                raise RuntimeError("hipExtStreamCreateWithCUMask failed (rc=%d)" % rc)
            out.append(torch.cuda.ExternalStream(st.value, device=dev))
            first += n
    _cu_streams[key] = tuple(out)
    return out


_cu_streams = {}


def require_cuda(*tensors, dtype=None):
    import torch
    want = dtype or torch.float32
    for t in tensors:
        if t is None:
            continue
        if not isinstance(t, torch.Tensor) or not t.is_cuda:
            raise RuntimeError("pwstablenet_amd: the HIP hot path needs CUDA/HIP tensors (got %s); there is no CPU "
                               "fallback -- move the model and inputs to the GPU" %
                               (t.device if isinstance(t, torch.Tensor) else type(t)))
        if t.dtype != want:
            raise RuntimeError("pwstablenet_amd: %s tensors expected, got %s" % (want, t.dtype))


def ptr(t):
    return ctypes.c_void_p(t.data_ptr()) if t is not None else None


def prof_collect(max_records=4096):
    buf = (PwsProfRecord * max_records)()
    n = lib().pws_prof_collect(buf, max_records)
    if n < 0:
        check(n, "pws_prof_collect")
    L = lib()
    return [(L.pws_prof_kernel_name(r.kernel_id).decode(), r.tag, r.flops, r.bytes, r.ms) for r in buf[:min(n, max_records)]]
```

Measured before the change: 2022.

## Defer split-K reduction into the consuming convolution's input load

When a split-K convolution's output is read only by the next convolution, the partial sums are kept in a dedicated hold buffer and no separate reduce kernel is launched. The consumer's input loader sums the partials and applies bias and activation as it reads them. This removes one reduce kernel launch and a write and re-read of the dense output for the eligible layers, currently one encoder layer. In exchange the consumer reads ksplit times more input data, and the change adds template variants, extra buffers and bookkeeping state in the executor.

```diff
diff --git a/pwstablenet_amd/csrc/abi.cpp b/pwstablenet_amd/csrc/abi.cpp
--- a/pwstablenet_amd/csrc/abi.cpp
+++ b/pwstablenet_amd/csrc/abi.cpp
@@ -38,7 +38,7 @@
     "wino_k3s1_kernel<F(2x2,3x3)>", "conv_bf16_kernel", "wgrad_bf16_kernel",
     "wino_ct4_kernel<F(3x3,2x2)>", "upsample_grid_sample_u8_kernel", "objective_kernels", "conv_ring_kernel", "conv_ringf_kernel",
     "wino_ring_kernel<F(2x2,3x3)>", "wino_ring_kernel<convT4,F(2x2,2x2)>", "conv_skinny_kernel", "wgrad_ring_kernel", "conv_skinny16_kernel", "conv_first_kernel", "wino5_first_kernel",
-    "field_homography_kernel"};
+    "field_homography_kernel", "splitk_reduce_kernel"};
 }
 
 bool prof_begin(int kernel_id, double flops, double bytes, hipStream_t st) {
diff --git a/pwstablenet_amd/csrc/common.h b/pwstablenet_amd/csrc/common.h
--- a/pwstablenet_amd/csrc/common.h
+++ b/pwstablenet_amd/csrc/common.h
@@ -67,7 +67,7 @@
     KID_CONV_K3S1_BIG = 0, KID_CONV_K3S1_SMALL, KID_CONV_K3S2_BIG, KID_CONV_K3S2_SMALL, KID_CONV_K5S1, KID_CONVT4_BIG,
     KID_CONVT4_SMALL, KID_THETA_HEAD, KID_FIELD_HEAD, KID_GRID_SAMPLE_FWD, KID_GRID_SAMPLE_BWD, KID_UPSAMPLE_GRID_SAMPLE_FWD,
     KID_UPSAMPLE, KID_AFFINE_GRID, KID_ADAM, KID_PACK, KID_DGRAD_K4S2, KID_DGRAD_SP3, KID_WGRAD, KID_ACT_BWD, KID_FIELD_HEAD_BWD,
-    KID_THETA_HEAD_BWD, KID_CONV_WINO, KID_CONV_BF16, KID_WGRAD_BF16, KID_CONV_WINO_CT4, KID_UPSAMPLE_GRID_SAMPLE_U8, KID_OBJECTIVE, KID_CONV_RING, KID_CONV_RINGF, KID_CONV_WRING, KID_CONV_WRING_CT4, KID_CONV_SKINNY, KID_WGRAD_RING, KID_CONV_SKINNY16, KID_CONV_FIRST, KID_CONV_FIRST_WINO, KID_FIELD_HOMOGRAPHY, KID_COUNT
+    KID_THETA_HEAD_BWD, KID_CONV_WINO, KID_CONV_BF16, KID_WGRAD_BF16, KID_CONV_WINO_CT4, KID_UPSAMPLE_GRID_SAMPLE_U8, KID_OBJECTIVE, KID_CONV_RING, KID_CONV_RINGF, KID_CONV_WRING, KID_CONV_WRING_CT4, KID_CONV_SKINNY, KID_WGRAD_RING, KID_CONV_SKINNY16, KID_CONV_FIRST, KID_CONV_FIRST_WINO, KID_FIELD_HOMOGRAPHY, KID_SPLITK_REDUCE, KID_COUNT
 };
 extern thread_local bool t_deterministic;
 struct DeterministicScope {
@@ -98,6 +98,21 @@
 struct ProfHint {
     double flops, bytes;
 };
+struct SplitkOut {
+    float *hold = nullptr;
+    size_t hold_floats = 0;
+    int ksplit = 1;
+    size_t split_stride = 0;
+};
+struct SplitkSrc {
+    int src = -1;
+    int ksplit = 1;
+    size_t split_stride = 0;
+    const float *partial = nullptr, *bias = nullptr;
+    int act = 0;
+    size_t pixels = 0;
+};
+int conv2d_fwd_impl(const pws_conv_args *a, hipStream_t st, const SplitkSrc *din = nullptr, SplitkOut *dout = nullptr);
 int theta_z1(const float *x, int n, int c, int hidden, const float *w_flat, const float *b_flat, float *ws, float *z1, hipStream_t st);
 int theta_z2(const float *h, int n, int hidden, const float *w_lin, const float *b_lin, float *z2, hipStream_t st);
 int field_head_raw(const float *x, int ld, int n, int h, int w, int c, const float *w_out, const float *b_out, float *z, hipStream_t st);
diff --git a/pwstablenet_amd/csrc/conv_common.h b/pwstablenet_amd/csrc/conv_common.h
--- a/pwstablenet_amd/csrc/conv_common.h
+++ b/pwstablenet_amd/csrc/conv_common.h
@@ -40,7 +40,43 @@
     int out_sign_ld;
     const void *dst_sign[4];
     int dst_sign_ld[4];
+    int dsrc, dsrc_ksplit, dsrc_act;
+    size_t dsrc_stride;
+    const float *dsrc_bias;
 };
+
+template <int N, int SPR, class V>
+__device__ __forceinline__ void splitk_deferred_load(V (&a)[N], const float *p0, const unsigned (&off)[N], const int (&c)[N], int n_used, int ksplit,
+                                                     size_t stride, const float *bias, int act) {
+#pragma unroll
+    for (int i = 0; i < N; ++i)
+        if (i < n_used) a[i] = *reinterpret_cast<const V *>(p0 + off[i]);
+    for (int s = 1; s < ksplit; s += SPR) {
+        V b[SPR][N];
+#pragma unroll
+        for (int j = 0; j < SPR; ++j) {
+            const float *ps = p0 + (size_t)min(s + j, ksplit - 1) * stride;
+#pragma unroll
+            for (int i = 0; i < N; ++i)
+                if (i < n_used) b[j][i] = *reinterpret_cast<const V *>(ps + off[i]);
+        }
+#pragma unroll
+        for (int j = 0; j < SPR; ++j) {
+            if (s + j < ksplit) {
+#pragma unroll
+                for (int i = 0; i < N; ++i)
+                    if (i < n_used) a[i].x += b[j][i].x, a[i].y += b[j][i].y, a[i].z += b[j][i].z, a[i].w += b[j][i].w;
+            }
+        }
+    }
+#pragma unroll
+    for (int i = 0; i < N; ++i) {
+        if (i < n_used) {
+            a[i].x = act_apply(a[i].x + (bias ? bias[c[i]] : 0.f), act), a[i].y = act_apply(a[i].y + (bias ? bias[c[i] + 1] : 0.f), act);
+            a[i].z = act_apply(a[i].z + (bias ? bias[c[i] + 2] : 0.f), act), a[i].w = act_apply(a[i].w + (bias ? bias[c[i] + 3] : 0.f), act);
+        }
+    }
+}
 
 __device__ __forceinline__ void epi_store(const ConvKParams &p, size_t pix, int co, float v) {
     if (p.ndst == 0) {
@@ -109,9 +145,17 @@
     int th, tw, tn, ck, bn;
     int kid;
     int (*launch)(ConvKParams &, hipStream_t, const ProfInfo &);
+    bool defer = false;
 };
 
 int launch_splitk_reduce(const ConvKParams &kp, const float *partial, size_t total4, hipStream_t st);
+int splitk_resolve(const pws_conv_args *a, const SplitkSrc &d, hipStream_t st);
+int splitk_finish(ConvKParams &kp, float *final_out, const float *ws, size_t out_floats, hipStream_t st, SplitkOut *dout);
+static inline float *splitk_partial_dst(const ConvKParams &kp, int ksplit, size_t out_floats, float *ws, const SplitkOut *dout) {
+    const bool hold = dout && dout->hold && ksplit > 1 && (size_t)ksplit * out_floats <= dout->hold_floats && kp.ndst == 0 && !kp.io_bf16 &&
+                      kp.out_ld == kp.cout;
+    return hold ? dout->hold : ws;
+}
 
 static inline long cdiv(long a, long b) { return (a + b - 1) / b; }
 
@@ -119,7 +163,8 @@
 constexpr long kFillBlocksBf16 = 256;
 
 [[maybe_unused]] static int select_and_launch(const TileChoice *cands, int ncand, ConvKParams &kp, int cin_total, float *final_out,
-                             float *ws, size_t ws_floats, hipStream_t st, const ProfInfo &pi, long kFill = kFillBlocks) {
+                             float *ws, size_t ws_floats, hipStream_t st, const ProfInfo &pi, long kFill = kFillBlocks, SplitkOut *dout = nullptr,
+                             const pws_conv_args *a = nullptr, const SplitkSrc *din = nullptr) {
     const TileChoice *best = nullptr;
     long best_blocks = -1;
     double best_score = -1.0;
@@ -137,6 +182,15 @@
         if (blocks * useful > best_score) best = &c, best_blocks = blocks, best_score = blocks * useful;
     }
     const TileChoice &c = *best;
+    if (kp.dsrc_ksplit > 1 && !c.defer) {
+        if (!a || !din) {
+            set_error("select_and_launch: deferred split-K source without its descriptor");
+            return PWS_EINVAL;
+        }
+        const int rc = splitk_resolve(a, *din, st);
+        if (rc != PWS_OK) return rc;
+        kp.src_ptr[kp.dsrc] = a->src[kp.dsrc].ptr, kp.dsrc_ksplit = 0;
+    }
     kp.tiles_x = (int)cdiv(kp.LW, c.tw), kp.tiles_y = (int)cdiv(kp.LH, c.th);
     kp.ntiles = (unsigned)(kp.tiles_x * kp.tiles_y * cdiv(kp.N, c.tn));
     const int total_chunks = cin_total / c.ck;
@@ -153,14 +207,23 @@
     kp.chunks_per_split = (int)cdiv(total_chunks, kp.ksplit);
     kp.ksplit = (int)cdiv(total_chunks, kp.chunks_per_split);
     kp.split_stride = out_floats;
-    kp.out = kp.ksplit > 1 ? ws : final_out;
-    ProfScope prof(c.kid, pi.flops, pi.bytes, st);
-    int rc = c.launch(kp, st, pi);
+    float *part = splitk_partial_dst(kp, kp.ksplit, out_floats, ws, dout);
+    kp.out = kp.ksplit > 1 ? part : final_out;
+    if (!dout) {
+        ProfScope prof(c.kid, pi.flops, pi.bytes, st);
+        int rc = c.launch(kp, st, pi);
+        if (rc != PWS_OK || kp.ksplit == 1) return rc;
+        kp.out = final_out;
+        return launch_splitk_reduce(kp, ws, out_floats / 4, st);
+    }
+    int rc;
+    {
+        ProfScope prof(c.kid, pi.flops, pi.bytes, st);
+        rc = c.launch(kp, st, pi);
+    }
     if (rc != PWS_OK || kp.ksplit == 1) return rc;
-    const size_t total4 = out_floats / 4;
-    kp.out = final_out;
-    return launch_splitk_reduce(kp, ws, total4, st);
-}
-
-
-}
+    return splitk_finish(kp, final_out, part, out_floats, st, dout);
+}
+
+
+}
diff --git a/pwstablenet_amd/csrc/conv_mfma.hip b/pwstablenet_amd/csrc/conv_mfma.hip
--- a/pwstablenet_amd/csrc/conv_mfma.hip
+++ b/pwstablenet_amd/csrc/conv_mfma.hip
@@ -23,7 +23,14 @@
     static constexpr int ITEMS_IN = (PIX * C4 + THREADS - 1) / THREADS;
     static constexpr int ITEMS_W = (TAPS * CK * (BN / 4) + THREADS - 1) / THREADS;
     static constexpr int ITEMS_NCHW = (PIX * CK + THREADS - 1) / THREADS;
+    static constexpr bool DEFER = false;
 };
+template <class C>
+struct Deferred : C {
+    static constexpr bool DEFER = true;
+};
+template <class C>
+constexpr bool kHasDeferred = !C::NCHW && C::BM == 64 && C::CK == 16 && ((C::KS == 3 && C::STRIDE == 2 && C::SUBPIX == 0) || C::SUBPIX == 1);
 
 template <class C>
 __global__ void __launch_bounds__(C::THREADS, 2) conv_mfma_kernel(const ConvKParams p) {
@@ -101,9 +108,21 @@
         } else {
             const float *sp = p.src_ptr[s] + c0;
             const size_t ld = p.src_ld[s];
-#pragma unroll
-            for (int it = 0; it < C::ITEMS_IN; ++it)
-                r_in[it] = *reinterpret_cast<const float4 *>(sp + (size_t)g_pix[it] * ld + g_c4[it]);
+            bool deferred = false;
+            if constexpr (C::DEFER) deferred = s == p.dsrc;
+            if (deferred) {
+                if constexpr (C::DEFER) {
+                    unsigned off[C::ITEMS_IN];
+                    int ch[C::ITEMS_IN];
+#pragma unroll
+                    for (int it = 0; it < C::ITEMS_IN; ++it) off[it] = (unsigned)g_pix[it] * (unsigned)ld + (unsigned)g_c4[it], ch[it] = c0 + g_c4[it];
+                    splitk_deferred_load<C::ITEMS_IN, 2>(r_in, sp, off, ch, C::ITEMS_IN, p.dsrc_ksplit, p.dsrc_stride, p.dsrc_bias, p.dsrc_act);
+                }
+            } else {
+#pragma unroll
+                for (int it = 0; it < C::ITEMS_IN; ++it)
+                    r_in[it] = *reinterpret_cast<const float4 *>(sp + (size_t)g_pix[it] * ld + g_c4[it]);
+            }
         }
         const float *wp = w_cls + (size_t)wrow * p.cout;
 #pragma unroll
@@ -246,8 +265,35 @@
     return check_launch("splitk_reduce_kernel");
 }
 
+int splitk_finish(ConvKParams &kp, float *final_out, const float *ws, size_t out_floats, hipStream_t st, SplitkOut *dout) {
+    if (dout && dout->hold && ws == dout->hold) {
+        dout->ksplit = kp.ksplit, dout->split_stride = kp.split_stride;
+        return PWS_OK;
+    }
+    kp.out = final_out;
+    ProfScope prof(KID_SPLITK_REDUCE, (double)out_floats * kp.ksplit, 4.0 * out_floats * (kp.ksplit + 1), st);
+    return launch_splitk_reduce(kp, ws, out_floats / 4, st);
+}
+
+int splitk_resolve(const pws_conv_args *a, const SplitkSrc &d, hipStream_t st) {
+    ConvKParams kp{};
+    const pws_src &sr = a->src[d.src];
+    kp.cout = sr.channels, kp.out_ld = sr.ld, kp.bias = d.bias, kp.act = d.act, kp.out = const_cast<float *>(sr.ptr);
+    kp.ksplit = d.ksplit, kp.split_stride = d.split_stride;
+    const size_t out_floats = (size_t)a->n * a->h * a->w * sr.channels;
+    ProfScope prof(KID_SPLITK_REDUCE, (double)out_floats * kp.ksplit, 4.0 * out_floats * (kp.ksplit + 1), st);
+    return launch_splitk_reduce(kp, d.partial, out_floats / 4, st);
+}
+
 template <class C, int KID>
 static int launch_cfg(ConvKParams &kp, hipStream_t st, const ProfInfo &pi) {
+    if constexpr (!C::DEFER && kHasDeferred<C>) {
+        if (kp.dsrc_ksplit > 1) return launch_cfg<Deferred<C>, KID>(kp, st, pi);
+    }
+    if (!C::DEFER && kp.dsrc_ksplit > 1) {
+        set_error("conv_mfma_kernel: this tile has no deferred split-K read");
+        return PWS_EINVAL;
+    }
     static PerDeviceFlag attr_set_dev;
     bool &attr_set = attr_set_dev.cur();
     if (!attr_set) {
@@ -266,7 +312,7 @@
 
 template <class C, int KID>
 static constexpr TileChoice choice() {
-    return TileChoice{C::TH, C::TW, C::TN, C::CK, C::BN, KID, &launch_cfg<C, KID>};
+    return TileChoice{C::TH, C::TW, C::TN, C::CK, C::BN, KID, &launch_cfg<C, KID>, kHasDeferred<C>};
 }
 
 using K3S1_T256 = ConvCfg<3, 1, 1, 0, 16, 16, 1, 16, 4, 1, 2, 2>;
@@ -323,9 +369,9 @@
 int conv_ringf_try(int kind, const ConvKParams &kp, hipStream_t st, const ProfInfo &pi);
 int conv_first_try(const ConvKParams &kp, hipStream_t st, const ProfInfo &pi);
 int wino5_first_try(const ConvKParams &kp, const float *u, hipStream_t st, const ProfInfo &pi);
-int conv_skinny_try(int kind, ConvKParams &kp, float *final_out, float *ws, size_t ws_floats, hipStream_t st, const ProfInfo &pi);
-
-int conv2d_fwd_impl(const pws_conv_args *a, hipStream_t st) {
+int conv_skinny_try(int kind, ConvKParams &kp, float *final_out, float *ws, size_t ws_floats, hipStream_t st, const ProfInfo &pi, SplitkOut *dout);
+
+int conv2d_fwd_impl(const pws_conv_args *a, hipStream_t st, const SplitkSrc *din, SplitkOut *dout) {
     PWS_REQUIRE(a != nullptr, "pws_conv2d_fwd: args is NULL");
     PWS_REQUIRE(a->n >= 0 && a->h > 0 && a->w > 0, "pws_conv2d_fwd: bad n/h/w %d/%d/%d", a->n, a->h, a->w);
     PWS_REQUIRE(a->nsrc >= 1 && a->nsrc <= 4, "pws_conv2d_fwd: nsrc %d not in 1..4", a->nsrc);
@@ -365,6 +411,25 @@
     float *ws = static_cast<float *>(a->ws);
     const size_t ws_floats = a->ws_bytes / sizeof(float);
     const bool bf16 = a->math == PWS_MATH_BF16 && a->w_bf16 && !nchw;
+    if (dout) dout->ksplit = 1;
+    if (bf16 || nchw || a->store == PWS_STORE_BF16) dout = nullptr;
+    SplitkSrc dsrc_desc{};
+    if (din && din->src >= 0 && din->ksplit > 1) {
+        PWS_REQUIRE(din->src < a->nsrc && din->partial && !nchw, "pws_conv2d_fwd: bad deferred split-K source");
+        const pws_src &sr = a->src[din->src];
+        const bool reach = !bf16 && a->store != PWS_STORE_BF16 && sr.ld == sr.channels && (size_t)a->n * a->h * a->w * sr.channels < (1u << 31) &&
+                           ((a->kind == PWS_CONV_K3S2 && a->w <= 16) || (a->kind == PWS_CONVT_K4S2 && a->w <= 8));
+        if (reach) {
+            dsrc_desc = *din;
+            kp.src_ptr[din->src] = din->partial;
+            kp.dsrc = din->src, kp.dsrc_ksplit = din->ksplit, kp.dsrc_stride = din->split_stride, kp.dsrc_bias = din->bias, kp.dsrc_act = din->act;
+            dout = nullptr;
+        } else {
+            const int rc = splitk_resolve(a, *din, st);
+            if (rc != PWS_OK) return rc;
+        }
+    }
+    const SplitkSrc *dpend = kp.dsrc_ksplit > 1 ? &dsrc_desc : nullptr;
     if (a->store == PWS_STORE_BF16) {
         PWS_REQUIRE(bf16, "pws_conv2d_fwd: bf16 storage needs math == PWS_MATH_BF16, w_bf16 and NHWC sources");
         PWS_REQUIRE(a->out_ld % 2 == 0 && a->cout % 2 == 0 && (reinterpret_cast<size_t>(a->out) & 3) == 0,
@@ -410,10 +475,10 @@
             kp.out = a->out;
             int rc = ledger_direct(8) ? 1 : conv_ringf_try(a->kind, kp, st, pi);
             if (rc != 1) return rc;
-            rc = ledger_direct(16) ? 1 : conv_skinny_try(a->kind, kp, a->out, ws, ws_floats, st, pi);
-            if (rc != 1) return rc;
-        }
-        return select_and_launch(kK3S1, 5, kp, kp.cin_pad, a->out, ws, ws_floats, st, pi);
+            rc = ledger_direct(16) ? 1 : conv_skinny_try(a->kind, kp, a->out, ws, ws_floats, st, pi, dout);
+            if (rc != 1) return rc;
+        }
+        return select_and_launch(kK3S1, 5, kp, kp.cin_pad, a->out, ws, ws_floats, st, pi, kFillBlocks, dout);
     }
     case PWS_CONV_K3S2:
         kp.OH = kp.LH = (a->h + 2 - 3) / 2 + 1, kp.OW = kp.LW = (a->w + 2 - 3) / 2 + 1;
@@ -425,10 +490,10 @@
             kp.out = a->out;
             int rc = ledger_direct(8) ? 1 : conv_ringf_try(a->kind, kp, st, info(9, (double)a->n * kp.OH * kp.OW));
             if (rc != 1) return rc;
-            rc = ledger_direct(16) ? 1 : conv_skinny_try(a->kind, kp, a->out, ws, ws_floats, st, info(9, (double)a->n * kp.OH * kp.OW));
-            if (rc != 1) return rc;
-        }
-        return select_and_launch(kK3S2, 5, kp, kp.cin_pad, a->out, ws, ws_floats, st, info(9, (double)a->n * kp.OH * kp.OW));
+            rc = ledger_direct(16) ? 1 : conv_skinny_try(a->kind, kp, a->out, ws, ws_floats, st, info(9, (double)a->n * kp.OH * kp.OW), dout);
+            if (rc != 1) return rc;
+        }
+        return select_and_launch(kK3S2, 5, kp, kp.cin_pad, a->out, ws, ws_floats, st, info(9, (double)a->n * kp.OH * kp.OW), kFillBlocks, dout, a, dpend);
     case PWS_CONV_K5S1:
         kp.OH = kp.LH = a->h, kp.OW = kp.LW = a->w;
         if (bf16) {
@@ -464,10 +529,10 @@
             kp.out = a->out;
             int rc = ledger_direct(8) ? 1 : conv_ringf_try(a->kind, kp, st, pi);
             if (rc != 1) return rc;
-            rc = ledger_direct(16) ? 1 : conv_skinny_try(a->kind, kp, a->out, ws, ws_floats, st, pi);
-            if (rc != 1) return rc;
-        }
-        return select_and_launch(kCT4, 5, kp, kp.cin_pad, a->out, ws, ws_floats, st, pi);
+            rc = ledger_direct(16) ? 1 : conv_skinny_try(a->kind, kp, a->out, ws, ws_floats, st, pi, dout);
+            if (rc != 1) return rc;
+        }
+        return select_and_launch(kCT4, 5, kp, kp.cin_pad, a->out, ws, ws_floats, st, pi, kFillBlocks, dout, a, dpend);
     }
     default:
         set_error("pws_conv2d_fwd: kind %d is not a runnable conv kind", a->kind);
diff --git a/pwstablenet_amd/csrc/conv_skinny.hip b/pwstablenet_amd/csrc/conv_skinny.hip
--- a/pwstablenet_amd/csrc/conv_skinny.hip
+++ b/pwstablenet_amd/csrc/conv_skinny.hip
@@ -23,6 +23,9 @@
     int ksplit, cps, nchunks;
     int M;
     unsigned ncob;
+    int dsrc, dsrc_ksplit, dsrc_act;
+    size_t dsrc_stride;
+    const float *dsrc_bias;
 };
 
 constexpr unsigned kSkOob = 0x7ffffff0u;
@@ -37,7 +40,7 @@
     return i == 0 ? a[0] : (i == 1 ? a[1] : (i == 2 ? a[2] : a[3]));
 }
 
-template <int MT_W, int NT_W, int WM>
+template <int MT_W, int NT_W, int WM, bool DEFER = false>
 __global__ void __launch_bounds__(256) conv_skinny_kernel(const SkParams p) {
     extern __shared__ __attribute__((aligned(16))) unsigned char lds[];
     constexpr int WN = 4 / WM;
@@ -97,15 +100,44 @@
         const float *sp = sksel4(p.src_ptr, s) + c0 + kq * 4;
         const int ld = sksel4(p.src_ld, s);
         const int kw = p.mode == SK_CT4 ? 2 : 3;
-#pragma unroll
-        for (int t = 0; t < MAXT; ++t) {
-            if (t < ntaps) {
-                const int dy = t / kw, dx = t - dy * kw;
-#pragma unroll
-                for (int i = 0; i < MT_W; ++i) {
-                    const int iy = piy[i] + dy, ix = pix_[i] + dx;
-                    const bool ok = pok[i] && iy >= 0 && iy < p.H && ix >= 0 && ix < p.W;
-                    a[t][i] = ok ? *reinterpret_cast<const f32x4 *>(sp + ((size_t)(pn[i] * p.H + iy) * p.W + ix) * ld) : (f32x4){0.f, 0.f, 0.f, 0.f};
+        bool deferred = false;
+        if constexpr (DEFER) deferred = s == p.dsrc;
+        if (deferred) {
+            if constexpr (DEFER) {
+                f32x4(&v)[MAXT * MT_W] = reinterpret_cast<f32x4(&)[MAXT * MT_W]>(a);
+                unsigned off[MAXT * MT_W];
+                int ch[MAXT * MT_W];
+                unsigned okm = 0;
+#pragma unroll
+                for (int t = 0; t < MAXT; ++t) {
+                    const int dy = t / kw, dx = t - dy * kw;
+#pragma unroll
+                    for (int i = 0; i < MT_W; ++i) {
+                        const int iy = piy[i] + dy, ix = pix_[i] + dx;
+                        const bool ok = t < ntaps && pok[i] && iy >= 0 && iy < p.H && ix >= 0 && ix < p.W;
+                        off[t * MT_W + i] = ok ? (unsigned)((pn[i] * p.H + iy) * p.W + ix) * (unsigned)ld : 0u;
+                        ch[t * MT_W + i] = c0 + kq * 4;
+                        okm |= ok ? 1u << (t * MT_W + i) : 0u;
+                    }
+                }
+                splitk_deferred_load<MAXT * MT_W, MT_W == 1 ? 2 : 1>(v, sp, off, ch, ntaps * MT_W, p.dsrc_ksplit, p.dsrc_stride, p.dsrc_bias, p.dsrc_act);
+#pragma unroll
+                for (int t = 0; t < MAXT; ++t)
+#pragma unroll
+                    for (int i = 0; i < MT_W; ++i)
+                        if (t < ntaps) a[t][i] = (okm >> (t * MT_W + i)) & 1u ? v[t * MT_W + i] : (f32x4){0.f, 0.f, 0.f, 0.f};
+            }
+        } else {
+#pragma unroll
+            for (int t = 0; t < MAXT; ++t) {
+                if (t < ntaps) {
+                    const int dy = t / kw, dx = t - dy * kw;
+#pragma unroll
+                    for (int i = 0; i < MT_W; ++i) {
+                        const int iy = piy[i] + dy, ix = pix_[i] + dx;
+                        const bool ok = pok[i] && iy >= 0 && iy < p.H && ix >= 0 && ix < p.W;
+                        a[t][i] = ok ? *reinterpret_cast<const f32x4 *>(sp + ((size_t)(pn[i] * p.H + iy) * p.W + ix) * ld) : (f32x4){0.f, 0.f, 0.f, 0.f};
+                    }
                 }
             }
         }
@@ -174,12 +206,15 @@
     }
 }
 
-template <int MT_W, int NT_W, int WM>
+template <int MT_W, int NT_W, int WM, bool DEFER = false>
 static int skinny_launch(const SkParams &p, unsigned grid, int lds_bytes, hipStream_t st) {
+    if constexpr (!DEFER) {
+        if (p.dsrc_ksplit > 1) return skinny_launch<MT_W, NT_W, WM, true>(p, grid, lds_bytes, st);
+    }
     static PerDeviceFlag attr_set_dev;
     bool &attr_set = attr_set_dev.cur();
     if (!attr_set) {
-        hipError_t e = hipFuncSetAttribute(reinterpret_cast<const void *>(&conv_skinny_kernel<MT_W, NT_W, WM>), hipFuncAttributeMaxDynamicSharedMemorySize,
+        hipError_t e = hipFuncSetAttribute(reinterpret_cast<const void *>(&conv_skinny_kernel<MT_W, NT_W, WM, DEFER>), hipFuncAttributeMaxDynamicSharedMemorySize,
                                            160 * 1024);
         if (e != hipSuccess) {
             set_error("hipFuncSetAttribute(conv_skinny_kernel): %s", hipGetErrorString(e));
@@ -187,11 +222,11 @@
         }
         attr_set = true;
     }
-    hipLaunchKernelGGL((conv_skinny_kernel<MT_W, NT_W, WM>), dim3(grid), dim3(256), lds_bytes, st, p);
+    hipLaunchKernelGGL((conv_skinny_kernel<MT_W, NT_W, WM, DEFER>), dim3(grid), dim3(256), lds_bytes, st, p);
     return check_launch("conv_skinny_kernel");
 }
 
-int conv_skinny_try(int kind, ConvKParams &kp, float *final_out, float *ws, size_t ws_floats, hipStream_t st, const ProfInfo &pi) {
+int conv_skinny_try(int kind, ConvKParams &kp, float *final_out, float *ws, size_t ws_floats, hipStream_t st, const ProfInfo &pi, SplitkOut *dout) {
     if (kp.io_bf16 || kp.ndst != 0 || exp_is(EXP_SKINNY_OFF)) return 1;
     int mode;
     if (kind == PWS_CONV_K3S1 || kind == PWS_CONVT_K3S1) mode = SK_K3S1;
@@ -214,6 +249,7 @@
     p.nsrc = kp.nsrc, p.N = kp.N, p.H = kp.H, p.W = kp.W, p.LH = kp.LH, p.LW = kp.LW, p.OH = kp.OH, p.OW = kp.OW, p.mode = mode;
     p.cin_pad = kp.cin_pad, p.cout = kp.cout, p.w = kp.w, p.w_bytes = (unsigned)w_bytes, p.bias = kp.bias, p.act = kp.act, p.out_ld = kp.out_ld;
     p.M = (int)M, p.ncob = (unsigned)((kp.cout + 63) / 64);
+    p.dsrc = kp.dsrc, p.dsrc_ksplit = kp.dsrc_ksplit, p.dsrc_act = kp.dsrc_act, p.dsrc_stride = kp.dsrc_stride, p.dsrc_bias = kp.dsrc_bias;
     p.nchunks = cin / 16;
     const int maxc = 36 / ntaps;
     const long blocks1 = (long)p.ncob * ncls;
@@ -230,18 +266,31 @@
     p.ksplit = (int)cdiv(p.nchunks, p.cps);
     if (p.cps > maxc) return 1;
     p.split_stride = out_floats;
-    p.out = p.ksplit > 1 ? ws : final_out;
+    float *part = splitk_partial_dst(kp, p.ksplit, out_floats, ws, dout);
+    p.out = p.ksplit > 1 ? part : final_out;
     const unsigned grid = (unsigned)(blocks1 * p.ksplit);
     const int lds_bytes = p.cps * ntaps * 4096;
     if (exp_is(EXP_SKINNY_SKIP)) return PWS_OK;
-    ProfScope prof(KID_CONV_SKINNY, pi.flops, pi.bytes, st);
+    auto launch = [&]() {
+        if (M <= 16) return skinny_launch<1, 1, 1>(p, grid, lds_bytes, st);
+        if (M <= 32) return skinny_launch<1, 2, 2>(p, grid, lds_bytes, st);
+        return skinny_launch<2, 4, 4>(p, grid, lds_bytes, st);
+    };
+    if (!dout) {
+        ProfScope prof(KID_CONV_SKINNY, pi.flops, pi.bytes, st);
+        const int rc = launch();
+        if (rc != PWS_OK || p.ksplit == 1) return rc;
+        kp.ksplit = p.ksplit, kp.split_stride = out_floats, kp.out = final_out;
+        return launch_splitk_reduce(kp, ws, out_floats / 4, st);
+    }
     int rc;
-    if (M <= 16) rc = skinny_launch<1, 1, 1>(p, grid, lds_bytes, st);
-    else if (M <= 32) rc = skinny_launch<1, 2, 2>(p, grid, lds_bytes, st);
-    else rc = skinny_launch<2, 4, 4>(p, grid, lds_bytes, st);
+    {
+        ProfScope prof(KID_CONV_SKINNY, pi.flops, pi.bytes, st);
+        rc = launch();
+    }
     if (rc != PWS_OK || p.ksplit == 1) return rc;
-    kp.ksplit = p.ksplit, kp.split_stride = out_floats, kp.out = final_out;
-    return launch_splitk_reduce(kp, ws, out_floats / 4, st);
-}
-
-}
+    kp.ksplit = p.ksplit, kp.split_stride = out_floats;
+    return splitk_finish(kp, final_out, part, out_floats, st, dout);
+}
+
+}
diff --git a/pwstablenet_amd/csrc/experiments.h b/pwstablenet_amd/csrc/experiments.h
--- a/pwstablenet_amd/csrc/experiments.h
+++ b/pwstablenet_amd/csrc/experiments.h
@@ -29,6 +29,7 @@
     EXP_SKINNY16_OFF = 71,
     EXP_SKINNY16_4096 = 72,
     EXP_SKINNY_SKIP = 73,
+    EXP_SPLITK_DEFER_OFF = 75,
     EXP_WGRAD_RING_OFF = 80,
     EXP_WGRAD_RING_FORCE = 81,
     EXP_HEAD_VALU = 90,
diff --git a/pwstablenet_amd/csrc/netg.cpp b/pwstablenet_amd/csrc/netg.cpp
--- a/pwstablenet_amd/csrc/netg.cpp
+++ b/pwstablenet_amd/csrc/netg.cpp
@@ -360,11 +360,21 @@
         }
         return o;
     }
-    Tn conv_groups(int layer, const Tn &x, int act, int ngroups, const Groups &dst, int g0) {
-        return run_conv(layer, x, act, group(dst, g0), ngroups, nullptr, 0);
-    }
-
-    Tn run_conv(int layer, const Tn &x, int act, const Tn &o, int ngroups, const float *nchw_src, int nchw_c) {
+    Tn conv_groups(int layer, const Tn &x, int act, int ngroups, const Groups &dst, int g0, bool sole_reader_next = false) {
+        return run_conv(layer, x, act, group(dst, g0), ngroups, nullptr, 0, sole_reader_next);
+    }
+
+    static bool splitk_defer_layer(int layer) {
+        switch (layer) {
+        case L_DB1_CS + 2 * 5:
+            return true;
+        default:
+            return false;
+        }
+    }
+    bool splitk_chain() const { return math_ == PWS_MATH_FP32 && !io16_ && !bn_on_ && !training_ && hold_[0] && hold_[1]; }
+
+    Tn run_conv(int layer, const Tn &x, int act, const Tn &o, int ngroups, const float *nchw_src, int nchw_c, bool sole_reader_next = false) {
         const Layer &l = L_[layer];
         const int oh = o.h, ow = o.w;
         Op op{OP_CONV, layer, act, 0, nchw_c > 0, x, o};
@@ -395,9 +405,27 @@
         }
         a.store = store();
         a.out_sign = o.seg[0].sign, a.out_sign_ld = l.cout / 8;
+        SplitkSrc din{};
+        if (pend_.ksplit > 1) {
+            for (int i = 0; i < a.nsrc && nchw_c == 0; ++i)
+                if (a.src[i].ptr == pend_dense_ && pend_q_ == q_) din = pend_, din.src = i;
+            pend_ = SplitkSrc{};
+            if (din.src < 0) {
+                set_error("pws_netg_forward: layer %d does not read the deferred split-K output in front of it", layer);
+                rc_ = PWS_EINVAL;
+                return o;
+            }
+        }
+        SplitkOut dout{};
+        const bool ask = sole_reader_next && splitk_chain();
+        if (ask && splitk_defer_layer(layer) && !exp_is(EXP_SPLITK_DEFER_OFF)) dout.hold = hold_[q_], dout.hold_floats = hold_bytes_ / sizeof(float);
         g_prof_tag = layer;
-        rc_ = pws_conv2d_fwd(&a, streams_[q_]);
+        rc_ = conv2d_fwd_impl(&a, streams_[q_], din.src >= 0 ? &din : nullptr, ask ? &dout : nullptr);
         g_prof_tag = -1;
+        if (rc_ == PWS_OK && dout.ksplit > 1) {
+            pend_.ksplit = dout.ksplit, pend_.split_stride = dout.split_stride, pend_.partial = dout.hold, pend_.bias = a.bias, pend_.act = a.act;
+            pend_dense_ = a.out, pend_q_ = q_;
+        }
         if (bn_on_ && rc_ == PWS_OK) {
             const int repeat = (layer == L_DB1_CS || layer == L_DB1_CS + 1) ? 2 : 1;
             rc_ = bn_forward(layer, op.aux[0], (size_t)n_ * oh * ow, act, o.seg[0].ptr, op.aux[1], repeat);
@@ -475,6 +503,10 @@
         splitk_ws2_ = alloc(splitk_big_ / sizeof(float));
         theta_ws_ = alloc(pws_theta_head_ws_floats(n_, 4 * ngf, 8 * ngf));
         theta_ws2_ = alloc(pws_theta_head_ws_floats(n_, 4 * ngf, 8 * ngf));
+        if (!training) {
+            hold_bytes_ = splitk_bytes_ / 2;
+            hold_[0] = alloc(hold_bytes_ / sizeof(float)), hold_[1] = alloc(hold_bytes_ / sizeof(float));
+        }
         if (!splitk_ws_ || !splitk_ws2_) splitk_bytes_ = 0, splitk_big_ = 0;
         for (int s = 0; s < 3; ++s) h_saved_[s] = training ? alloc((size_t)n_ * 8 * ngf) : nullptr;
         x_nhwc_ = alloc((size_t)n_ * 256 * 256 * 32);
@@ -487,6 +519,11 @@
 
   private:
     float *splitk_ws_ = nullptr, *splitk_ws2_ = nullptr, *theta_ws_ = nullptr, *theta_ws2_ = nullptr;
+    float *hold_[2] = {nullptr, nullptr};
+    size_t hold_bytes_ = 0;
+    SplitkSrc pend_{};
+    const float *pend_dense_ = nullptr;
+    int pend_q_ = 0;
     float *h_saved_[3] = {nullptr, nullptr, nullptr};
     float *x_nhwc_ = nullptr;
     float *theta_x32_[2] = {nullptr, nullptr};
@@ -561,7 +598,7 @@
     }
     for (int k = 4; k <= 8; ++k) {
         const int db = k - 1;
-        E.conv_groups(L_DB1_CS + 2 * (db - 1), enc(k - 1, 1), PWS_ACT_LRELU, 2, Ck[k], 0);
+        E.conv_groups(L_DB1_CS + 2 * (db - 1), enc(k - 1, 1), PWS_ACT_LRELU, 2, Ck[k], 0, true);
         E.conv_groups(L_DB1_CS + 2 * (db - 1) + 1, Exec::cat(enc(k - 1, 2), E.group(Ck[k], 0)), PWS_ACT_LRELU, 2, Ek[k], 1);
     }
     E.use(0);
@@ -575,7 +612,7 @@
         E.field(x111, 0, th1, ac, resid, grids);
     }
     auto merged_level = [&](int l) {
-        E.conv_groups(L_UB7_MP + 2 * (7 - l) + 1, dec(l + 1, 1), PWS_ACT_RELU, 2, Gl[l], 0);
+        E.conv_groups(L_UB7_MP + 2 * (7 - l) + 1, dec(l + 1, 1), PWS_ACT_RELU, 2, Gl[l], 0, true);
         E.conv_groups(L_UB7_MP + 2 * (7 - l), Exec::cat(E.group(Gl[l], 0), dec(l + 1, 2)), PWS_ACT_RELU, 2, Vl[l], 1);
     };
     E.use(1);
diff --git a/pwstablenet_amd/hipabi.py b/pwstablenet_amd/hipabi.py
--- a/pwstablenet_amd/hipabi.py
+++ b/pwstablenet_amd/hipabi.py
@@ -43,6 +43,7 @@
     SKINNY16_OFF = 71
     SKINNY16_4096 = 72
     SKINNY_SKIP = 73
+    SPLITK_DEFER_OFF = 75
     WGRAD_RING_OFF = 80
     WGRAD_RING_FORCE = 81
     HEAD_VALU = 90
```

Result: no change. 2020 (-0.1%).
